# ZKTLabs/zkt-plonk

Hardware: AMD Instinct MI355X
Metric: proofs/sec (withdraw, n=2^20) (higher is better)
Workload: dtype u32 limbs (256-bit Montgomery); 1 GPU; full prove, WithdrawCircuit INPUTS=8 HEIGHT=64 Poseidon x5 (1019498 gates, 538 Poseidon gadgets), bn254, n=2^20, TABLE_SIZE=1024, 12 public inputs; parallelism=proofs sharded across 1 GPU(s), chained=True, distinct_witnesses=2, witness_on_device=True, table_cached=True, proof_bytes=802

## Files before the change

### include/zkt_plonk.h

```cpp
#ifndef ZKT_PLONK_H
#define ZKT_PLONK_H

#include <stddef.h>
#include <stdint.h>

#ifdef __cplusplus
extern "C" {
#endif

typedef struct zkt_ctx zkt_ctx;

enum {
    ZKT_CURVE_BN254 = 0,
    ZKT_CURVE_BLS12_381 = 1
};

enum {
    ZKT_OK = 0,
    ZKT_ERR_INVALID_ARGUMENT = 1,
    ZKT_ERR_INVALID_DOMAIN_SIZE = 2,
    ZKT_ERR_HIP = 3,
    ZKT_ERR_NO_DEVICE = 4,
    ZKT_ERR_TOO_MANY_COEFFICIENTS = 5,
    ZKT_ERR_ZERO_DENOMINATOR = 6,
// ... 23 lines not shown
    int (*all_gather_async)(void* user, const void* d_send, void* d_recv, size_t bytes, void* hip_stream);
} zkt_comm_vtable;
#define ZKT_QUOTIENT_CHUNKS 4
int zkt_ctx_set_comm(zkt_ctx* ctx, const zkt_comm_vtable* comm);
int zkt_shard_range(size_t total, int rank, int world, size_t* lo, size_t* hi);
int zkt_comm_stats(zkt_ctx* ctx, uint64_t* calls, uint64_t* bytes_sent);
int zkt_comm_selftest(const zkt_comm_vtable* comm, const void* send, void* recv, size_t bytes);

int zkt_dev_alloc(zkt_ctx* ctx, size_t bytes, void** dptr);
int zkt_dev_free(zkt_ctx* ctx, void* dptr);
int zkt_dev_upload(zkt_ctx* ctx, void* dptr, const void* host, size_t bytes);
int zkt_dev_download(zkt_ctx* ctx, void* host, const void* dptr, size_t bytes);

int zkt_ntt(zkt_ctx* ctx, int log_n, int inverse, int coset, const uint64_t* in, size_t in_len, uint64_t* out);
int zkt_ntt_dev(zkt_ctx* ctx, int log_n, int inverse, int coset, const void* d_in, size_t in_len, void* d_out);
int zkt_ntt_class(zkt_ctx* ctx, int log_n, int log_big, int cls, const uint64_t* in, size_t in_len, uint64_t* out);
int zkt_domain_group_gen(zkt_ctx* ctx, int log_n, uint64_t* out4);

int zkt_srs_load(zkt_ctx* ctx, const uint64_t* g1_xy_mont, size_t count);
int zkt_srs_load_dev(zkt_ctx* ctx, const void* d_g1_xy_mont, size_t count);
int zkt_srs_generate(zkt_ctx* ctx, const uint64_t* tau_canonical4, size_t count);
int zkt_srs_download(zkt_ctx* ctx, size_t offset, size_t count, uint64_t* out_xy_mont);
int zkt_srs_generate_g2(int curve_id, const uint64_t* tau_canonical4, uint64_t* out_h, uint64_t* out_beta_h);
int zkt_srs_load_slice(zkt_ctx* ctx, const uint64_t* g1_xy_mont_slice, size_t offset, size_t count, size_t total);
int zkt_srs_generate_slice(zkt_ctx* ctx, const uint64_t* tau_canonical4, size_t offset, size_t count, size_t total);
int zkt_msm_g1(zkt_ctx* ctx, const uint64_t* scalars, size_t len, size_t base_offset, int scalars_montgomery,
               uint64_t* out_xy_mont, int* out_is_infinity);
int zkt_msm_g1_dev(zkt_ctx* ctx, const void* d_scalars, size_t len, size_t base_offset, int scalars_montgomery,
                   void* out_xy_mont_host);
int zkt_msm_enqueue_dev(zkt_ctx* ctx, const void* d_scalars, size_t len, size_t base_offset, int scalars_montgomery);
int zkt_msm_info(zkt_ctx* ctx, int* window_bits, int* windows, size_t* srs_count);

#define ZKT_MSM_BASES_MAX ((size_t)1 << 22)
int zkt_msm_g1_bases(zkt_ctx* ctx, const uint64_t* bases_xy_mont, const uint64_t* scalars, size_t n,
                     int scalars_montgomery, uint64_t* out_xy_mont, int* out_is_infinity);
int zkt_msm_g1_bases_dev(zkt_ctx* ctx, const void* d_bases_xy_mont, const void* d_scalars, size_t n,
                         int scalars_montgomery, uint64_t* out_xy_mont_host, int* out_is_infinity);
int zkt_msm_bases_info(zkt_ctx* ctx, size_t n, int scalars_montgomery, int* window_bits, int* windows);

#define ZKT_KZG_BATCH_MAX 32
int zkt_kzg_commit_batch(zkt_ctx* ctx, const uint64_t* const* coeffs, const size_t* lens, int k,
                         int scalars_montgomery, uint64_t* out_xy_mont, int* out_is_infinity);
int zkt_kzg_commit_batch_dev(zkt_ctx* ctx, const void* const* d_coeffs, const size_t* lens, int k,
                             int scalars_montgomery, uint64_t* out_xy_mont, int* out_is_infinity);
int zkt_kzg_open(zkt_ctx* ctx, const uint64_t* const* coeffs, const size_t* lens, int k,
                 const uint64_t* challenges_mont, const uint64_t* point_mont,
                 uint64_t* out_w_xy_mont, int* out_w_is_infinity, uint64_t* out_evals_mont);
int zkt_kzg_open_dev(zkt_ctx* ctx, const void* const* d_coeffs, const size_t* lens, int k,
                     const uint64_t* challenges_mont, const uint64_t* point_mont,
                     uint64_t* out_w_xy_mont, int* out_w_is_infinity, uint64_t* out_evals_mont);

int zkt_ctx_set_lagrange(zkt_ctx* ctx, int on);
int zkt_ctx_set_wire_elimination(zkt_ctx* ctx, int mode);
int zkt_lagrange_info(zkt_ctx* ctx, int* log_n, size_t* bases);
int zkt_commit_evals_dev(zkt_ctx* ctx, const void* d_evals, const uint64_t* blinders, int k, int path, uint64_t* out_xy_mont,
                         int* out_is_infinity);

enum {
    ZKT_TRANSCRIPT_MERLIN = 0,
    ZKT_TRANSCRIPT_ETHEREUM = 1
};
typedef struct zkt_transcript zkt_transcript;
zkt_transcript* zkt_transcript_new(int kind, const char* label);
void zkt_transcript_free(zkt_transcript* t);
void zkt_transcript_append_u64(zkt_transcript* t, const char* label, uint64_t v);
void zkt_transcript_append_scalars(zkt_transcript* t, const char* label, const uint8_t* le32, size_t count, int single);
void zkt_transcript_append_commitment(zkt_transcript* t, const char* label, const uint8_t* x_le, const uint8_t* y_le,
                                      size_t fq_bytes, int is_infinity);
void zkt_transcript_challenge_scalar(zkt_transcript* t, const char* label, int fr_bits, uint8_t out_le32[32]);
void zkt_transcript_seed(zkt_transcript* t, uint64_t circuit_size, const uint8_t* xy_le, const uint8_t* is_infinity,
                         size_t fq_bytes);
int zkt_transcript_append_message(zkt_transcript* t, const char* label, const uint8_t* msg, size_t len);
int zkt_transcript_challenge_bytes(zkt_transcript* t, const char* label, uint8_t* out, size_t len);

typedef struct {
    void* user;
    void (*append_u64)(void* user, const char* label, uint64_t v);
    void (*append_scalars)(void* user, const char* label, const uint64_t* fr_mont, size_t count, int single);
    void (*append_commitment)(void* user, const char* label, const uint64_t* g1_xy_mont, int is_infinity);
    void (*challenge_scalar)(void* user, const char* label, uint64_t* fr_mont_out4);
} zkt_transcript_vtable;

int zkt_circuit_load(zkt_ctx* ctx, int log_n, const uint64_t* const* pk_polys, const size_t* pk_lens);

int zkt_circuit_setup(zkt_ctx* ctx, int log_n, const uint64_t* const* evals, const size_t* eval_lens, int evals_on_device,
                      uint64_t* out_commitments, int* out_is_infinity);

int zkt_circuit_sigma_dev(zkt_ctx* ctx, int log_n, const uint32_t* d_w_l, const uint32_t* d_w_r, const uint32_t* d_w_o,
                          size_t n_rows, size_t n_vars, void* const* d_sigma);
int zkt_circuit_setup_wiring(zkt_ctx* ctx, int log_n, const uint64_t* const* evals, const size_t* eval_lens,
                             int evals_on_device, const uint32_t* w_l, const uint32_t* w_r, const uint32_t* w_o,
                             size_t n_rows, size_t n_vars, int wiring_on_device,
                             uint64_t* out_commitments, int* out_is_infinity);

typedef struct {
    const uint64_t* a_evals;
    const uint64_t* b_evals;
    const uint64_t* c_evals;
    size_t n_rows;
    const uint64_t* table;
    size_t table_len;
    const size_t* pi_pos;
    const uint64_t* pi_vals;
    size_t n_pi;
    const uint64_t* blinders;
    int wires_on_device;
// ... 107 lines not shown
int zkt_verify_prepare(int curve_id, const zkt_verify_inputs* in, zkt_transcript* transcript, uint64_t* out_pairs,
                       int* out_is_infinity);

int zkt_pairing_product_is_one(int curve_id, const uint64_t* g1_xy_mont, const uint64_t* g2_xy_mont, size_t n, int* is_one);
int zkt_verify(int curve_id, const zkt_verify_inputs* in, zkt_transcript* transcript, const uint64_t* h_g2_mont,
               const uint64_t* beta_h_g2_mont, int* accepted);

int zkt_verify_batch(int curve_id, const zkt_verify_inputs* ins, zkt_transcript* const* transcripts, size_t count,
                     const uint64_t* h_g2_mont, const uint64_t* beta_h_g2_mont, int* accepted);

#define ZKT_G1_DECOMPRESS_MAX ((size_t)1 << 22)
enum {
    ZKT_G1_VALID = 0,
    ZKT_G1_IDENTITY = 1,
    ZKT_G1_NOT_CANONICAL = 2,
    ZKT_G1_BOTH_FLAGS = 3,
    ZKT_G1_NOT_ON_CURVE = 4,
    ZKT_G1_NOT_IN_SUBGROUP = 5
};
int zkt_g1_decompress(zkt_ctx* ctx, const uint8_t* compressed, size_t n, uint64_t* out_xy_mont, uint8_t* out_status);
int zkt_g1_decompress_dev(zkt_ctx* ctx, const void* d_compressed, size_t n, void* d_out_xy_mont, void* d_out_status);

#define ZKT_VERIFY_BATCH_DEV_MAX (ZKT_MSM_BASES_MAX / 24)
int zkt_verify_batch_prepare_dev(zkt_ctx* ctx, const zkt_verify_inputs* ins, zkt_transcript* const* transcripts, size_t count,
                                 const uint64_t* h_g2_mont, const uint64_t* beta_h_g2_mont, uint64_t* out_ab,
                                 int* out_ab_is_infinity, uint64_t* out_rho);
int zkt_verify_batch_dev(zkt_ctx* ctx, const zkt_verify_inputs* ins, zkt_transcript* const* transcripts, size_t count,
                         const uint64_t* h_g2_mont, const uint64_t* beta_h_g2_mont, int* accepted);

int zkt_g1_msm_host(int curve_id, const uint64_t* points_xy_mont, const uint64_t* scalars, size_t n, int scalars_montgomery,
                    uint64_t* out_xy_mont, int* out_is_infinity);

int zkt_keyfile_committer_key(const char* path, int curve_id, size_t max_powers, uint64_t* out_xy_mont, size_t* n_powers);
int zkt_keyfile_prover_key(const char* path, int curve_id, uint64_t* const* out_polys, size_t* lens10);
int zkt_keyfile_verifier_key(const char* path, int curve_id, uint64_t* n, uint64_t* pi_roots_mont, size_t pi_cap, size_t* n_pi,
                             uint64_t* commitments_xy_mont, int* is_infinity10);
#define ZKT_EPK_VECTORS 17
int zkt_keyfile_extended_prover_key(const char* path, int curve_id, int which, uint64_t* out_mont, size_t cap, size_t* lens17);
int zkt_circuit_check_epk_file(zkt_ctx* ctx, const char* epk_path, int* first_mismatch_vector, size_t* mismatch_at);
int zkt_srs_load_file(zkt_ctx* ctx, const char* ck_path, size_t max_powers);
int zkt_circuit_load_file(zkt_ctx* ctx, const char* pk_path, int log_n);

int zkt_debug_params(zkt_ctx* ctx, int which, uint32_t* out, size_t out_words);
int zkt_host_field_op(int curve_id, int which, int op, const uint32_t* a, const uint32_t* b, uint32_t* out);
int zkt_g1_sum_host(int curve_id, const uint64_t* points_xy_mont, size_t count, uint64_t* out_xy_mont, int* out_is_infinity);
int zkt_debug_fr_mul(zkt_ctx* ctx, const uint64_t* a, const uint64_t* b, size_t n, uint64_t* out);
int zkt_debug_ntt_batch(zkt_ctx* ctx, int log_n, int inverse, int coset, int nb, const void* const* d_in, const size_t* in_len,
                        void* const* d_out);
int zkt_debug_ntt_split(zkt_ctx* ctx, int npass, const int* log_r);
int zkt_debug_merkle_tree_split(zkt_merkle_tree* tree, int wide_min_parents);
int zkt_debug_pairing_selftest(int curve_id);
int zkt_debug_quotient(zkt_ctx* ctx, const uint64_t* challenges, const uint64_t* const* wit, const uint64_t* pi_pos,
                       const uint64_t* pi_vals, size_t n_pi, uint64_t* out);
int zkt_debug_grand_products(zkt_ctx* ctx, const uint64_t* challenges, const uint64_t* const* vectors, uint64_t* out_z1,
                             uint64_t* out_z2);
int zkt_debug_combine_split(zkt_ctx* ctx, const uint64_t* table, size_t table_len, const uint64_t* f, int fresh,
                            uint64_t* h1_out, uint64_t* h2_out);
int zkt_debug_commit_wires_dev(zkt_ctx* ctx, const void* d_variables, size_t n_vars, const uint32_t* d_w_l, const uint32_t* d_w_r,
                               const uint32_t* d_w_o, size_t n_rows, const uint64_t* blinders, int route, uint64_t* out_xy_mont,
                               int* out_is_infinity, int* out_route);
int zkt_debug_commit_wires_pi_dev(zkt_ctx* ctx, const void* d_variables, size_t n_vars, const uint32_t* d_w_l, const uint32_t* d_w_r,
                                  const uint32_t* d_w_o, size_t n_rows, const uint64_t* blinders, int route, const size_t* pi_pos,
                                  size_t n_pi, uint64_t* out_xy_mont, int* out_is_infinity, int* out_route);
int zkt_debug_wire_elimination(int curve, const uint64_t* const* selectors, const uint32_t* w_l, const uint32_t* w_r, const uint32_t* w_o,
                               size_t n_rows, size_t n_vars, const size_t* pi_pos, size_t n_pi, int K, uint8_t* out_kind,
                               uint32_t* out_free, size_t* out_n_free, uint32_t* out_term_v, uint32_t* out_term_f,
                               uint64_t* out_term_coef, size_t* out_n_terms, uint64_t* out_kappa);
int zkt_debug_open_witness(zkt_ctx* ctx, const uint64_t* coeffs, size_t len, const uint64_t* z4, uint64_t* out);
int zkt_debug_eval_lincomb(zkt_ctx* ctx, const uint64_t* const* polys, const size_t* lens, int k, const uint64_t* points,
                           const uint64_t* scalars, uint64_t* out_evals, uint64_t* out_lincomb, size_t out_len);

enum zkt_fx_op {
    ZKT_FX_UNPACK = 0, ZKT_FX_UNPACK_SHIFT = 1, ZKT_FX_PACK = 2, ZKT_FX_FROM_ARK = 3, ZKT_FX_TO_ARK = 4,
    ZKT_FX_NORMALIZE = 5, ZKT_FX_ADD = 6, ZKT_FX_DBL = 7, ZKT_FX_SUB_1 = 8, ZKT_FX_SUB_2 = 9, ZKT_FX_SUB_4 = 10,
    ZKT_FX_SUB_8 = 11, ZKT_FX_SUB2_6 = 12, ZKT_FX_ADD_LAZY = 13, ZKT_FX_SUB_LAZY_3 = 14, ZKT_FX_SUB_LAZY_4 = 15,
    ZKT_FX_SUB_LAZY_5 = 16, ZKT_FX_SUB_LAZY_9 = 17, ZKT_FX_SUB_LAZY_WIDE_8_30 = 18, ZKT_FX_MUL = 19, ZKT_FX_MUL_INL = 20,
    ZKT_FX_SQR = 21, ZKT_FX_SQR_INL = 22, ZKT_FX_MUL2_INL = 23, ZKT_FX_MUL_SHOUP = 24 ,
    ZKT_FX_MUL_LOW = 25, ZKT_FX_REDUCE_SMALL = 26, ZKT_FX_REDUCE_LAZY = 27 ,
    ZKT_FX_COND_SUB_P = 28, ZKT_FX_CANON = 29, ZKT_FX_IS_ZERO_CANON = 30, ZKT_FX_IS_ZERO_LT2P = 31, ZKT_FX_OP_COUNT = 32
};
enum zkt_xyzz_op {
    ZKT_XYZZ_ADD_MIXED = 0, ZKT_XYZZ_ADD_MIXED_INL = 1, ZKT_XYZZ_ADD = 2, ZKT_XYZZ_ADD_INL = 3, ZKT_XYZZ_DOUBLE = 4,
    ZKT_XYZZ_DOUBLE_AFFINE = 5, ZKT_XYZZ_OP_COUNT = 6
};
int zkt_debug_fx_layout(int curve_id, int which, int* limbs, int* limb_bits, int* sh);
int zkt_host_fx_op(int curve_id, int which, int op, const uint32_t* in, size_t n, uint32_t* out);
int zkt_debug_fx_op(zkt_ctx* ctx, int which, int op, const uint32_t* in, size_t n, uint32_t* out);
int zkt_host_xyzz_op(int curve_id, int op, const uint32_t* in, size_t n, uint32_t* out);
int zkt_debug_xyzz_op(zkt_ctx* ctx, int op, const uint32_t* in, size_t n, uint32_t* out);

#ifdef __cplusplus
}
#endif
#endif
```

### shim/src/ffi.rs

```rust
use std::os::raw::{c_char, c_int, c_void};

#[repr(C)]
pub struct ZktCtx {
    _private: [u8; 0],
}

#[repr(C)]
pub struct ZktTranscriptVtable {
    pub user: *mut c_void,
    pub append_u64: extern "C" fn(*mut c_void, *const c_char, u64),
    pub append_scalars: extern "C" fn(*mut c_void, *const c_char, *const u64, usize, c_int),
    pub append_commitment: extern "C" fn(*mut c_void, *const c_char, *const u64, c_int),
    pub challenge_scalar: extern "C" fn(*mut c_void, *const c_char, *mut u64),
}

#[repr(C)]
pub struct ZktCommVtable {
    pub user: *mut c_void,
    pub rank: c_int,
    pub world: c_int,
    pub device_buffers: c_int,
    pub all_gather: extern "C" fn(*mut c_void, *const c_void, *mut c_void, usize, c_int, *mut c_void) -> c_int,
    pub all_gather_async: Option<extern "C" fn(*mut c_void, *const c_void, *mut c_void, usize, *mut c_void) -> c_int>,
}
// ... 17 lines not shown
    pub w_r: *const u32,
    pub w_o: *const u32,
}

#[repr(C)]
pub struct ZktWitnessReport {
    pub satisfied: c_int,
    pub checked: c_int,
    pub n_arithmetic: u64,
    pub first_arithmetic: u64,
    pub residual: [u64; 4],
    pub n_lookup: u64,
    pub first_lookup: u64,
    pub n_wiring: u64,
    pub first_wiring_row: u64,
    pub first_wiring_column: c_int,
}

pub const ZKT_CHECK_WIRING: c_int = 1;
pub const ZKT_CHECK_NONE: u64 = u64::MAX;
pub const ZKT_VARIABLE_ZERO: u32 = 0xFFFF_FFFF;
pub const ZKT_CURVE_BN254: c_int = 0;
pub const ZKT_CURVE_BLS12_381: c_int = 1;
pub const ZKT_KZG_BATCH_MAX: usize = 32;

extern "C" {
    pub fn zkt_ctx_create(curve_id: c_int, device_id: c_int, out: *mut *mut ZktCtx) -> c_int;
    pub fn zkt_ctx_destroy(ctx: *mut ZktCtx);
    pub fn zkt_last_error(ctx: *const ZktCtx) -> *const c_char;
    pub fn zkt_ctx_set_comm(ctx: *mut ZktCtx, comm: *const ZktCommVtable) -> c_int;
    pub fn zkt_shard_range(total: usize, rank: c_int, world: c_int, lo: *mut usize, hi: *mut usize) -> c_int;
    pub fn zkt_ntt(ctx: *mut ZktCtx, log_n: c_int, inverse: c_int, coset: c_int, input: *const u64, in_len: usize,
                   out: *mut u64) -> c_int;
    pub fn zkt_srs_load(ctx: *mut ZktCtx, g1_xy_mont: *const u64, count: usize) -> c_int;
    pub fn zkt_srs_load_slice(ctx: *mut ZktCtx, g1_xy_mont: *const u64, offset: usize, count: usize, total: usize) -> c_int;
    pub fn zkt_srs_load_file(ctx: *mut ZktCtx, ck_path: *const c_char, max_powers: usize) -> c_int;
    pub fn zkt_msm_g1(ctx: *mut ZktCtx, scalars: *const u64, len: usize, base_offset: usize, scalars_montgomery: c_int,
                      out_xy_mont: *mut u64, out_is_infinity: *mut c_int) -> c_int;
    pub fn zkt_ctx_fork(ctx: *mut ZktCtx, out: *mut *mut ZktCtx) -> c_int;
    pub fn zkt_kzg_commit_batch(ctx: *mut ZktCtx, coeffs: *const *const u64, lens: *const usize, k: c_int,
                                scalars_montgomery: c_int, out_xy_mont: *mut u64, out_is_infinity: *mut c_int) -> c_int;
    pub fn zkt_kzg_commit_batch_dev(ctx: *mut ZktCtx, d_coeffs: *const *const c_void, lens: *const usize, k: c_int,
                                    scalars_montgomery: c_int, out_xy_mont: *mut u64, out_is_infinity: *mut c_int) -> c_int;
    pub fn zkt_kzg_open(ctx: *mut ZktCtx, coeffs: *const *const u64, lens: *const usize, k: c_int, challenges_mont: *const u64,
                        point_mont: *const u64, out_w_xy_mont: *mut u64, out_w_is_infinity: *mut c_int,
                        out_evals_mont: *mut u64) -> c_int;
    pub fn zkt_kzg_open_dev(ctx: *mut ZktCtx, d_coeffs: *const *const c_void, lens: *const usize, k: c_int,
                            challenges_mont: *const u64, point_mont: *const u64, out_w_xy_mont: *mut u64,
                            out_w_is_infinity: *mut c_int, out_evals_mont: *mut u64) -> c_int;
    pub fn zkt_commit_evals_dev(ctx: *mut ZktCtx, d_evals: *const c_void, blinders: *const u64, k: c_int, path: c_int,
                                out_xy_mont: *mut u64, out_is_infinity: *mut c_int) -> c_int;
    pub fn zkt_ctx_set_lagrange(ctx: *mut ZktCtx, on: c_int) -> c_int;
    pub fn zkt_ctx_set_wire_elimination(ctx: *mut ZktCtx, mode: c_int) -> c_int;
    pub fn zkt_lagrange_info(ctx: *mut ZktCtx, log_n: *mut c_int, bases: *mut usize) -> c_int;
    pub fn zkt_circuit_load(ctx: *mut ZktCtx, log_n: c_int, pk_polys: *const *const u64, pk_lens: *const usize) -> c_int;
    pub fn zkt_circuit_load_file(ctx: *mut ZktCtx, pk_path: *const c_char, log_n: c_int) -> c_int;
    pub fn zkt_keyfile_extended_prover_key(path: *const c_char, curve_id: c_int, which: c_int, out_mont: *mut u64, cap: usize,
                                           lens17: *mut usize) -> c_int;
    pub fn zkt_circuit_check_epk_file(ctx: *mut ZktCtx, epk_path: *const c_char, first_mismatch_vector: *mut c_int,
                                      mismatch_at: *mut usize) -> c_int;
    pub fn zkt_circuit_setup(ctx: *mut ZktCtx, log_n: c_int, evals: *const *const u64, eval_lens: *const usize,
                             evals_on_device: c_int, out_commitments: *mut u64, out_is_infinity: *mut c_int) -> c_int;
    pub fn zkt_circuit_sigma_dev(ctx: *mut ZktCtx, log_n: c_int, d_w_l: *const u32, d_w_r: *const u32, d_w_o: *const u32,
                                 n_rows: usize, n_vars: usize, d_sigma: *const *mut c_void) -> c_int;
    pub fn zkt_circuit_setup_wiring(ctx: *mut ZktCtx, log_n: c_int, evals: *const *const u64, eval_lens: *const usize,
                                    evals_on_device: c_int, w_l: *const u32, w_r: *const u32, w_o: *const u32, n_rows: usize,
                                    n_vars: usize, wiring_on_device: c_int, out_commitments: *mut u64,
                                    out_is_infinity: *mut c_int) -> c_int;
    pub fn zkt_prove_with(ctx: *mut ZktCtx, inputs: *const ZktProveInputs, transcript: *const ZktTranscriptVtable,
                          proof_out: *mut u8, proof_cap: usize, proof_len: *mut usize) -> c_int;
    pub fn zkt_prove_set_next(ctx: *mut ZktCtx, next: *const ZktProveInputs) -> c_int;
    pub fn zkt_circuit_check_witness(ctx: *mut ZktCtx, inputs: *const ZktProveInputs, flags: c_int,
                                     out: *mut ZktWitnessReport) -> c_int;
    pub fn zkt_g1_msm_host(curve_id: c_int, points_xy_mont: *const u64, scalars: *const u64, n: usize, scalars_montgomery: c_int,
                           out_xy_mont: *mut u64, out_is_infinity: *mut c_int) -> c_int;
    pub fn zkt_msm_g1_bases(ctx: *mut ZktCtx, bases_xy_mont: *const u64, scalars: *const u64, n: usize,
                            scalars_montgomery: c_int, out_xy_mont: *mut u64, out_is_infinity: *mut c_int) -> c_int;
    pub fn zkt_msm_g1_bases_dev(ctx: *mut ZktCtx, d_bases_xy_mont: *const c_void, d_scalars: *const c_void, n: usize,
                                scalars_montgomery: c_int, out_xy_mont_host: *mut u64, out_is_infinity: *mut c_int) -> c_int;
    pub fn zkt_verify(curve_id: c_int, inputs: *const ZktVerifyInputs, transcript: *mut c_void, h_g2_mont: *const u64,
                      beta_h_g2_mont: *const u64, accepted: *mut c_int) -> c_int;
    pub fn zkt_verify_batch(curve_id: c_int, inputs: *const ZktVerifyInputs, transcripts: *const *mut c_void, count: usize,
                            h_g2_mont: *const u64, beta_h_g2_mont: *const u64, accepted: *mut c_int) -> c_int;
    pub fn zkt_verify_batch_prepare_dev(ctx: *mut ZktCtx, inputs: *const ZktVerifyInputs, transcripts: *const *mut c_void, count: usize,
                                        h_g2_mont: *const u64, beta_h_g2_mont: *const u64, out_ab: *mut u64,
                                        out_ab_is_infinity: *mut c_int, out_rho: *mut u64) -> c_int;
    pub fn zkt_verify_batch_dev(ctx: *mut ZktCtx, inputs: *const ZktVerifyInputs, transcripts: *const *mut c_void, count: usize,
                                h_g2_mont: *const u64, beta_h_g2_mont: *const u64, accepted: *mut c_int) -> c_int;
    pub fn zkt_g1_decompress(ctx: *mut ZktCtx, compressed: *const u8, n: usize, out_xy_mont: *mut u64, out_status: *mut u8) -> c_int;
    pub fn zkt_g1_decompress_dev(ctx: *mut ZktCtx, d_compressed: *const c_void, n: usize, d_out_xy_mont: *mut c_void,
                                 d_out_status: *mut c_void) -> c_int;
    pub fn zkt_poseidon_load(ctx: *mut ZktCtx, params: *const ZktPoseidonParams, out: *mut *mut c_void) -> c_int;
    pub fn zkt_poseidon_free(ctx: *mut ZktCtx, params: *mut c_void);
    pub fn zkt_poseidon_hash_batch_dev(ctx: *mut ZktCtx, params: *const c_void, d_inputs: *const c_void, batch: usize,
                                       arity: c_int, d_out_hashes: *mut c_void, d_out_states: *mut c_void) -> c_int;
    pub fn zkt_poseidon_gadget_vars_per_hash(params: *const c_void) -> usize;
    pub fn zkt_poseidon_gadget_witness_dev(ctx: *mut ZktCtx, params: *const c_void, args: *const ZktPoseidonGadgetArgs) -> c_int;
    pub fn zkt_poseidon_gadget_check(ctx: *mut ZktCtx, params: *const c_void) -> c_int;
    pub fn zkt_merkle_path_vars_per_level(params: *const c_void) -> usize;
    pub fn zkt_poseidon_merkle_path_witness_dev(ctx: *mut ZktCtx, params: *const c_void, args: *const ZktMerklePathArgs) -> c_int;
    pub fn zkt_poseidon_merkle_path_validate(ctx: *mut ZktCtx, params: *const c_void, args: *const ZktMerklePathArgs) -> c_int;
    pub fn zkt_merkle_tree_create(ctx: *mut ZktCtx, params: *const c_void, height: c_int, capacity: usize, out: *mut *mut c_void) -> c_int;
    pub fn zkt_merkle_tree_free(ctx: *mut ZktCtx, tree: *mut c_void);
    pub fn zkt_merkle_tree_append_dev(ctx: *mut ZktCtx, tree: *mut c_void, d_leaves: *const c_void, m: usize, first_index: *mut u64) -> c_int;
    pub fn zkt_merkle_tree_append(ctx: *mut ZktCtx, tree: *mut c_void, leaves: *const u64, m: usize, first_index: *mut u64) -> c_int;
    pub fn zkt_merkle_tree_root(ctx: *mut ZktCtx, tree: *mut c_void, out4: *mut u64) -> c_int;
// ... 73 lines not shown
```

### zkt-plonk_amd/_lib.py

```python
from __future__ import annotations

import ctypes
import os
import re
from typing import Optional

import numpy as np

_HERE = os.path.dirname(os.path.abspath(__file__))
_LIB = os.environ.get("ZKT_LIB_PATH") or os.path.join(_HERE, "libzkt_plonk_hip.so")
_HEADER = os.path.join(_HERE, "..", "include", "zkt_plonk.h")

MSM_BASES_MAX = 1 << 22
G1_DECOMPRESS_MAX = 1 << 22
VERIFY_BATCH_DEV_MAX = MSM_BASES_MAX // 24
KZG_BATCH_MAX = 32
CURVE_BN254 = 0
CURVE_BLS12_381 = 1
_CURVES = {"bn254": 0, "bls12_381": 1, "bls12-381": 1, 0: 0, 1: 1}

_lib = None


class ZktError(RuntimeError):
# ... 462 lines not shown
def host_fx_op(curve, which: int, op: int, records) -> np.ndarray:
    L_ = fx_layout(curve, which)[0]
    rec = _records(records, 4 * L_)
    out = np.zeros_like(rec)
    rc = lib().zkt_host_fx_op(curve_id(curve), which, op, _u32p(rec), rec.shape[0], _u32p(out))
    if rc:
        raise ZktError(rc, "zkt_host_fx_op")
    return out


def host_xyzz_op(curve, op: int, records) -> np.ndarray:
    w = 4 * fx_layout(curve, 1)[0] + 1
    rec = _records(records, 2 * w)
    out = np.zeros((rec.shape[0], w), dtype=np.uint32)
    rc = lib().zkt_host_xyzz_op(curve_id(curve), op, _u32p(rec), rec.shape[0], _u32p(out))
    if rc:
        raise ZktError(rc, "zkt_host_xyzz_op")
    return out


def srs_generate_g2(curve, tau: int):
    L = lib()
    cid = curve_id(curve)
    words = 8 if cid == CURVE_BN254 else 12
    t = np.array([(int(tau) >> (64 * i)) & 0xFFFFFFFFFFFFFFFF for i in range(4)], dtype=np.uint64)
    h = np.zeros(2 * words, dtype=np.uint64)
    bh = np.zeros(2 * words, dtype=np.uint64)
    P64 = ctypes.POINTER(ctypes.c_uint64)
    L.zkt_srs_generate_g2.argtypes = [ctypes.c_int, P64, P64, P64]
    rc = L.zkt_srs_generate_g2(cid, u64p(t), u64p(h), u64p(bh))
    if rc:
        raise ZktError(rc, "zkt_srs_generate_g2")
    return h, bh


def g1_msm_host(curve, points, scalars, montgomery: bool = True) -> tuple:
    L = lib()
    cid = curve_id(curve)
    words = 8 if cid == CURVE_BN254 else 12
    pts = np.ascontiguousarray(points, dtype=np.uint64).reshape(-1, words)
    sc = np.ascontiguousarray(scalars, dtype=np.uint64).reshape(-1, 4)
    assert pts.shape[0] == sc.shape[0]
    out = np.zeros(words, dtype=np.uint64)
    inf = ctypes.c_int(0)
    P64 = ctypes.POINTER(ctypes.c_uint64)
    L.zkt_g1_msm_host.argtypes = [ctypes.c_int, P64, P64, ctypes.c_size_t, ctypes.c_int, P64, ctypes.POINTER(ctypes.c_int)]
    rc = L.zkt_g1_msm_host(cid, u64p(pts) if pts.size else None, u64p(sc) if sc.size else None, pts.shape[0], int(montgomery),
                           u64p(out), ctypes.byref(inf))
    if rc:
        raise ZktError(rc, "zkt_g1_msm_host")
    return out, bool(inf.value)


def wire_elimination(curve, selectors, w_l, w_r, w_o, n_vars: int, pi_pos=(), K: int = 16):
    L = lib()
    sel = [np.ascontiguousarray(q, dtype=np.uint64).reshape(-1, 4) for q in selectors]
    w = [np.ascontiguousarray(x, dtype=np.uint32) for x in (w_l, w_r, w_o)]
    n_rows = len(w[0])
    assert len(sel) == 5 and all(q.shape[0] == n_rows for q in sel) and all(len(x) == n_rows for x in w)
    pi = (ctypes.c_size_t * max(len(pi_pos), 1))(*[int(x) for x in pi_pos])
    cap = max(K * n_vars, 1)
    kind = np.zeros(max(n_vars, 1), dtype=np.uint8)
    free = np.zeros(max(n_vars, 1), dtype=np.uint32)
    tv, tf = np.zeros(cap, dtype=np.uint32), np.zeros(cap, dtype=np.uint32)
    tc = np.zeros((cap, 4), dtype=np.uint64)
    kappa = np.zeros((max(n_vars, 1), 4), dtype=np.uint64)
    n_free, n_terms = ctypes.c_size_t(0), ctypes.c_size_t(0)
    P64, P32 = ctypes.POINTER(ctypes.c_uint64), ctypes.POINTER(ctypes.c_uint32)
    sp = (P64 * 5)(*[u64p(q) for q in sel])
    L.zkt_debug_wire_elimination.argtypes = [ctypes.c_int, ctypes.POINTER(P64), P32, P32, P32, ctypes.c_size_t, ctypes.c_size_t,
                                             ctypes.POINTER(ctypes.c_size_t), ctypes.c_size_t, ctypes.c_int,
                                             ctypes.POINTER(ctypes.c_uint8), P32, ctypes.POINTER(ctypes.c_size_t), P32, P32, P64,
                                             ctypes.POINTER(ctypes.c_size_t), P64]
    rc = L.zkt_debug_wire_elimination(curve_id(curve), sp, _u32p(w[0]), _u32p(w[1]), _u32p(w[2]), n_rows, n_vars, pi, len(pi_pos),
                                      int(K), kind.ctypes.data_as(ctypes.POINTER(ctypes.c_uint8)), _u32p(free), ctypes.byref(n_free),
                                      _u32p(tv), _u32p(tf), u64p(tc), ctypes.byref(n_terms), u64p(kappa))
    if rc:
        raise ZktError(rc, "zkt_debug_wire_elimination")
    nt = n_terms.value
    return kind[:n_vars], free[:n_free.value].copy(), tv[:nt].copy(), tf[:nt].copy(), tc[:nt].copy(), kappa[:n_vars]


class Transcript:

    def __init__(self, kind: str = "merlin", label: str = "ZKT Plonk", fr_bits: int = 254, fq_bytes: int = 32):
        self._L = lib()
        self._h = ctypes.c_void_p(self._L.zkt_transcript_new(0 if kind == "merlin" else 1, label.encode()))
        self.fr_bits = fr_bits
        self.fq_bytes = fq_bytes

    def __del__(self):
        if getattr(self, "_h", None):
            self._L.zkt_transcript_free(self._h)
            self._h = None

    @property
    def handle(self):
        return self._h

    def append_u64(self, label: str, v: int):
        self._L.zkt_transcript_append_u64(self._h, label.encode(), v)

    def append_scalar(self, label: str, v: int):
        self._L.zkt_transcript_append_scalars(self._h, label.encode(), int(v).to_bytes(32, "little"), 1, 1)

    def append_scalars(self, label: str, vals):
# ... 702 lines not shown
            self._L.zkt_debug_commit_wires_pi_dev.argtypes = [ctypes.c_void_p, ctypes.c_void_p, ctypes.c_size_t, ctypes.c_void_p,
                                                              ctypes.c_void_p, ctypes.c_void_p, ctypes.c_size_t,
                                                              ctypes.POINTER(ctypes.c_uint64), ctypes.c_int,
                                                              ctypes.POINTER(ctypes.c_size_t), ctypes.c_size_t,
                                                              ctypes.POINTER(ctypes.c_uint64), ctypes.POINTER(ctypes.c_int),
                                                              ctypes.POINTER(ctypes.c_int)]
            self.check(self._L.zkt_debug_commit_wires_pi_dev(self._h, ctypes.c_void_p(d_variables), n_vars, ctypes.c_void_p(d_w_l),
                                                             ctypes.c_void_p(d_w_r), ctypes.c_void_p(d_w_o), n_rows, u64p(bl),
                                                             int(route), pi, len(pos), u64p(out), inf, took))
            return out, [bool(x) for x in inf], [int(x) for x in took]
        self._L.zkt_debug_commit_wires_dev.argtypes = [ctypes.c_void_p, ctypes.c_void_p, ctypes.c_size_t, ctypes.c_void_p,
                                                       ctypes.c_void_p, ctypes.c_void_p, ctypes.c_size_t,
                                                       ctypes.POINTER(ctypes.c_uint64), ctypes.c_int,
                                                       ctypes.POINTER(ctypes.c_uint64), ctypes.POINTER(ctypes.c_int),
                                                       ctypes.POINTER(ctypes.c_int)]
        self.check(self._L.zkt_debug_commit_wires_dev(self._h, ctypes.c_void_p(d_variables), n_vars, ctypes.c_void_p(d_w_l),
                                                      ctypes.c_void_p(d_w_r), ctypes.c_void_p(d_w_o), n_rows, u64p(bl), int(route),
                                                      u64p(out), inf, took))
        return out, [bool(x) for x in inf], [int(x) for x in took]

    def check_epk_file(self, path: str):
        self._L.zkt_circuit_check_epk_file.argtypes = [ctypes.c_void_p, ctypes.c_char_p, ctypes.POINTER(ctypes.c_int),
                                                       ctypes.POINTER(ctypes.c_size_t)]
        vec, at = ctypes.c_int(0), ctypes.c_size_t(0)
        self.check(self._L.zkt_circuit_check_epk_file(self._h, path.encode(), ctypes.byref(vec), ctypes.byref(at)))
        if vec.value < 0:
            return None
        return vec.value, (-1 if at.value == ctypes.c_size_t(-1).value else at.value)

    def debug_eval_lincomb(self, polys, points, scalars, out_len: int):
        keep = [np.ascontiguousarray(p_, dtype=np.uint64).reshape(-1, 4) for p_ in polys]
        k = len(keep)
        P64 = ctypes.POINTER(ctypes.c_uint64)
        ptrs = (P64 * k)(*[u64p(a) for a in keep])
        lens = (ctypes.c_size_t * k)(*[a.shape[0] for a in keep])
        pts = np.ascontiguousarray(points, dtype=np.uint64).reshape(k, 4)
        scs = np.ascontiguousarray(scalars, dtype=np.uint64).reshape(k, 4)
        ev = np.empty((k, 4), dtype=np.uint64)
        lc = np.empty((out_len, 4), dtype=np.uint64)
        self._L.zkt_debug_eval_lincomb.argtypes = [ctypes.c_void_p, ctypes.POINTER(P64), ctypes.POINTER(ctypes.c_size_t), ctypes.c_int,
                                                   P64, P64, P64, P64, ctypes.c_size_t]
        self.check(self._L.zkt_debug_eval_lincomb(self._h, ptrs, lens, k, u64p(pts), u64p(scs), u64p(ev), u64p(lc), out_len))
        return ev, lc

    def debug_open_witness(self, coeffs, z) -> np.ndarray:
        p_ = np.ascontiguousarray(coeffs, dtype=np.uint64).reshape(-1, 4)
        zz = np.ascontiguousarray(z, dtype=np.uint64).reshape(4)
        out = np.empty((p_.shape[0] - 1, 4), dtype=np.uint64)
        self._L.zkt_debug_open_witness.argtypes = [ctypes.c_void_p, ctypes.POINTER(ctypes.c_uint64), ctypes.c_size_t,
                                                   ctypes.POINTER(ctypes.c_uint64), ctypes.POINTER(ctypes.c_uint64)]
        self.check(self._L.zkt_debug_open_witness(self._h, u64p(p_), p_.shape[0], u64p(zz), u64p(out)))
        return out

    def debug_quotient(self, n: int, challenges, wit, pi_pos=(), pi_vals=None) -> np.ndarray:
        ch = np.ascontiguousarray(challenges, dtype=np.uint64).reshape(5, 4)
        keep = [None if w is None else np.ascontiguousarray(w, dtype=np.uint64).reshape(4 * n, 4) for w in wit]
        assert len(keep) == 9
        ptrs = (ctypes.c_void_p * 9)(*[None if w is None else w.ctypes.data for w in keep])
        pos = np.ascontiguousarray(list(pi_pos), dtype=np.uint64)
        vals = np.ascontiguousarray(pi_vals if len(pos) else np.zeros((0, 4)), dtype=np.uint64).reshape(-1, 4)
        out = np.empty((4 * n, 4), dtype=np.uint64)
        self.check(self._L.zkt_debug_quotient(self._h, u64p(ch), ptrs, u64p(pos) if len(pos) else None,
                                              u64p(vals) if len(pos) else None, len(pos), u64p(out)))
        return out
```

### zkt-plonk_amd/csrc/capi.hip

```cpp
#include "ctx.hpp"

#include <cstdlib>
#include "hostinv.hpp"
#include "ec.hpp"
#include "hostec.hpp"
#include "fx_test.hpp"
#include "msm.hpp"

#include <cstring>

namespace zkt {

const char* exp_env(const char* name) {
#ifdef ZKT_EXPERIMENTS
    return getenv(name);
#else
    (void)name;
    return nullptr;
#endif
}

int set_err(zkt_ctx* c, int code, const std::string& msg) {
    if (c) c->err = msg;
    return code;
// ... 150 lines not shown
template <class P>
static int dump_params(uint32_t* out, size_t words) {
    const int N = P::N;
    if (words < (size_t)(3 * N + 1)) return -1;
    for (int i = 0; i < N; ++i) out[i] = P::mod(i);
    out[N] = P::INV;
    for (int i = 0; i < N; ++i) out[N + 1 + i] = P::one(i);
    for (int i = 0; i < N; ++i) out[2 * N + 1 + i] = P::r2(i);
    return N;
}

}

using namespace zkt;

extern "C" {

const char* zkt_version(void) { return "zkt-plonk_amd 0.1 (gfx950)"; }

int zkt_ctx_create(int curve_id, int device_id, zkt_ctx** out) {
    if (!out) return ZKT_ERR_INVALID_ARGUMENT;
    *out = nullptr;
    if (curve_id != ZKT_CURVE_BN254 && curve_id != ZKT_CURVE_BLS12_381) return ZKT_ERR_INVALID_ARGUMENT;
    int count = 0;
    if (hipGetDeviceCount(&count) != hipSuccess || count <= 0 || device_id < 0 || device_id >= count)
        return ZKT_ERR_NO_DEVICE;
    if (hipSetDevice(device_id) != hipSuccess) return ZKT_ERR_NO_DEVICE;
    zkt_ctx* c = new zkt_ctx();
    c->batch_off = exp_env("ZKT_MSM_NO_BATCH") != nullptr;
    c->aux_off = exp_env("ZKT_NO_AUX") != nullptr;
    c->curve = curve_id;
    c->device = device_id;
    if (hipStreamCreateWithFlags(&c->stream, hipStreamNonBlocking) != hipSuccess) {
        delete c;
        return ZKT_ERR_HIP;
    }
    c->own_stream = true;
    *out = c;
    return ZKT_OK;
}

int zkt_ctx_fork(zkt_ctx* parent, zkt_ctx** out) {
    if (!parent || !out) return ZKT_ERR_INVALID_ARGUMENT;
    *out = nullptr;
    if (parent->sharded()) return set_err(parent, ZKT_ERR_INVALID_ARGUMENT, "zkt_ctx_fork: not for a context with a communicator");
    if (parent->zombie) return set_err(parent, ZKT_ERR_INVALID_ARGUMENT, "zkt_ctx_fork: the context has been destroyed");
    zkt_ctx* root = parent->parent ? parent->parent : parent;
    zkt_ctx* c = nullptr;
    int rc = zkt_ctx_create(parent->curve, parent->device, &c);
    if (rc) return rc;
    (void)hipStreamSynchronize(parent->stream);
    c->lagrange_off = parent->lagrange_off;
    c->wire_elim_mode = parent->wire_elim_mode;
    c->batch_off = parent->batch_off;
    c->aux_off = parent->aux_off;
    c->ntt_plans = parent->ntt_plans;
    c->parent = root;
    root->forks.fetch_add(1);
    if ((rc = msm_fork(c, parent)) || (rc = circuit_fork(c, parent))) {
        parent->err = c->err;
        zkt_ctx_destroy(c);
        return rc;
    }
    *out = c;
    return ZKT_OK;
}

void zkt_ctx_destroy(zkt_ctx* c) {
    if (!c) return;
    (void)hipSetDevice(c->device);
    (void)hipStreamSynchronize(c->stream);
    if (c->forks.load() > 0) {
        c->zombie = true;
        return;
    }
    zkt_ctx* const owner = c->parent;
    circuit_release(c);
    msm_release(c);
    prof_resolve(c);
    for (hipEvent_t e : c->event_pool) (void)hipEventDestroy(e);
    c->event_pool.clear();
    c->ntt_plans.clear();
    c->msm.reset();
    c->msmb.reset();
    c->kzg.reset();
    c->circuit.reset();
    if (c->comm.pinned) (void)hipHostFree(c->comm.pinned);
    for (void* p : c->owned) (void)hipFree(p);
    c->owned.clear();
    if (c->own_stream && c->stream) (void)hipStreamDestroy(c->stream);
    delete c;
    if (owner && owner->forks.fetch_sub(1) == 1 && owner->zombie) {
        owner->zombie = false;
        zkt_ctx_destroy(owner);
    }
}

int zkt_ctx_set_comm(zkt_ctx* c, const zkt_comm_vtable* comm) {
    if (!c) return ZKT_ERR_INVALID_ARGUMENT;
    if (int rf = refuse_if_forked(c, "zkt_ctx_set_comm")) return rf;
    if (c->parent && comm && comm->world > 1) return set_err(c, ZKT_ERR_INVALID_ARGUMENT, "a forked context cannot take a communicator");
    if (comm && comm->world > 1) {
        const int w = comm->world;
        if ((w != 2 && w != 4 && w != 8) || comm->rank < 0 || comm->rank >= w || !comm->all_gather)
            return set_err(c, ZKT_ERR_INVALID_ARGUMENT, "communicator: world must be 1, 2, 4 or 8 with a valid rank and callback");
    }
// ... 372 lines not shown
```

### zkt-plonk_amd/csrc/ctx.hpp

```cpp
#pragma once
#include <hip/hip_runtime.h>
#include <stdint.h>
#include <stddef.h>
#include <map>
#include <string>
#include <tuple>
#include <vector>
#include <memory>
#include <atomic>

#include "../../include/zkt_plonk.h"
#include "fp.hpp"
#include "fx.hpp"
#include "ntt.hpp"

namespace zkt {

struct MsmState;
struct MsmBasesState;
struct KzgState;
struct CircuitState;

}

struct zkt_ctx {
    int curve = 0;
    int device = 0;
    hipStream_t stream = nullptr;
    bool own_stream = false;
    std::string err;

    std::map<std::tuple<int, int, int, int>, std::shared_ptr<void>> ntt_plans;
    int ntt_split_npass = 0;
    int ntt_split_log_r[3] = {0, 0, 0};
    void* ntt_scratch = nullptr;
    size_t ntt_scratch_bytes = 0;
    void* io_a = nullptr;
    size_t io_a_bytes = 0;
    void* io_b = nullptr;
    size_t io_b_bytes = 0;
    void* check_scratch = nullptr;
    size_t check_scratch_bytes = 0;
    void* verify_scratch = nullptr;
    size_t verify_scratch_bytes = 0;

    int prof_on = 0;
    struct ProfSlot {
        std::vector<std::pair<hipEvent_t, hipEvent_t>> pending;
        double total_ms = 0.0;
        uint64_t calls = 0;
        uint64_t launches = 0;
    };
    std::map<std::string, ProfSlot> prof;
    std::vector<hipEvent_t> event_pool;

    struct Comm {
        zkt_comm_vtable vt{};
        void* pinned = nullptr;
        size_t pinned_bytes = 0;
        uint64_t calls = 0, bytes = 0;
    } comm;
    bool sharded() const { return comm.vt.world > 1; }

    std::shared_ptr<zkt::MsmState> msm;
    std::shared_ptr<zkt::MsmBasesState> msmb;
    std::shared_ptr<zkt::KzgState> kzg;
    uint64_t msm_epoch = 0;
    uint64_t srs_generation = 0;
    zkt_ctx* parent = nullptr;
    std::atomic<int> forks{0};
    bool zombie = false;
    bool aux_off = false;
    bool batch_off = false;
    bool lagrange_off = false;
    int wire_elim_mode = 1;
    std::shared_ptr<zkt::CircuitState> circuit;
    std::vector<void*> owned;
};

namespace zkt {

const char* exp_env(const char* name);

int set_err(zkt_ctx* c, int code, const std::string& msg);
int refuse_if_forked(zkt_ctx* c, const char* what);
int hip_fail(zkt_ctx* c, hipError_t e, const char* what);

#define ZKT_HIP(c, call)                                        \
    do {                                                        \
        hipError_t _e = (call);                                 \
        if (_e != hipSuccess) return zkt::hip_fail((c), _e, #call); \
    } while (0)

struct ProfScope {
    zkt_ctx* c;
    zkt_ctx::ProfSlot* slot = nullptr;
    hipEvent_t e0 = nullptr, e1 = nullptr;
    hipStream_t stream = nullptr;
    uint64_t count = 1;
    ProfScope(zkt_ctx* ctx, const char* name, hipStream_t on_stream = nullptr, uint64_t units = 1);
    ~ProfScope();
};

int comm_all_gather_host(zkt_ctx* c, const void* send, void* recv, size_t bytes);
int comm_all_gather_dev(zkt_ctx* c, const void* d_send, void* d_recv, size_t bytes);
bool comm_async_available(const zkt_ctx* c);
int comm_all_gather_async(zkt_ctx* c, const void* d_send, void* d_recv, size_t bytes, hipStream_t st);

int ensure_buffer(zkt_ctx* c, void** p, size_t* cur, size_t bytes);
struct DevBuf {
    void* p = nullptr;
    size_t bytes = 0;
};
inline int grow(zkt_ctx* c, DevBuf& b, size_t bytes) { return ensure_buffer(c, &b.p, &b.bytes, bytes); }
int dev_alloc(zkt_ctx* c, void** p, size_t bytes);
void dev_free(zkt_ctx* c, void* p);

template <class P>
Fe<P> root_of_unity(int log_n);
int ntt_run(zkt_ctx* c, int log_n, int inverse, int coset, const void* d_in, size_t in_len, void* d_out);
int ntt_run_batch(zkt_ctx* c, int log_n, int inverse, int coset, int nb, const void* const* d_in, const size_t* in_len,
                  void* const* d_out);
int ntt_class_code(int log_big, int cls);
int ntt_force_split(zkt_ctx* c, int npass, const int* log_r);
int ntt_run_class(zkt_ctx* c, int log_n, int log_big, int cls, const void* d_in, size_t in_len, void* d_out, void* d_fold);

void circuit_release(zkt_ctx* c);
int circuit_fork(zkt_ctx* child, const zkt_ctx* parent);

}
```

### zkt-plonk_amd/csrc/ntt.hip

```cpp
#include "ctx.hpp"
#include "hostinv.hpp"
#include <cstdlib>

namespace zkt {

constexpr int TILE_LOG = 10;
constexpr int TILE = 1 << TILE_LOG;
constexpr int NTT_THREADS = 256;
constexpr int EPT = TILE / NTT_THREADS;

template <class P>
ZKT_D Fx<P> tile_get(const uint4* lo, const uint4* hi, const uint32_t* top, int64_t idx) {
    static_assert(FxP<P>::L == 9, "scalar fields use nine limbs");
    const uint4 a = lo[idx], b = hi[idx];
    Fx<P> r;
    r.l[0] = a.x; r.l[1] = a.y; r.l[2] = a.z; r.l[3] = a.w;
    r.l[4] = b.x; r.l[5] = b.y; r.l[6] = b.z; r.l[7] = b.w;
    r.l[8] = top[idx];
    return r;
}
template <class P>
ZKT_D void tile_put(uint4* lo, uint4* hi, uint32_t* top, int64_t idx, const Fx<P>& x) {
    lo[idx] = make_uint4(x.l[0], x.l[1], x.l[2], x.l[3]);
    hi[idx] = make_uint4(x.l[4], x.l[5], x.l[6], x.l[7]);
    top[idx] = x.l[8];
}

ZKT_D uint32_t bitrev32(uint32_t x, int bits) { return __brev(x) >> (32 - bits); }

constexpr int NTT_W_PACKED = 0, NTT_W_LIMBS = 1, NTT_W_SHOUP = 2;
template <class P, int MODE>
struct WTile {
    const uint4* lo;
    const uint4* hi;
    const uint32_t* top;
    const uint4* qlo;
    const uint4* qhi;
    const uint32_t* qtop;
    ZKT_D Fx<P> mul(int e, const Fx<P>& d) const {
        if constexpr (MODE == NTT_W_SHOUP) {
            return fx_mul_shoup<P>(d, tile_get<P>(lo, hi, top, e), tile_get<P>(qlo, qhi, qtop, e));
        } else if constexpr (MODE == NTT_W_LIMBS) {
            return fx_mul_inl<P>(tile_get<P>(lo, hi, top, e), d);
        } else {
            Fe<P> w;
            const uint4 a = lo[e], b = hi[e];
            w.v[0] = a.x; w.v[1] = a.y; w.v[2] = a.z; w.v[3] = a.w;
            w.v[4] = b.x; w.v[5] = b.y; w.v[6] = b.z; w.v[7] = b.w;
            return fx_mul_inl<P>(fx_unpack<P>(w), d);
        }
    }
};

template <class P, int G, bool LASTSTEP, class W>
ZKT_D void dif_group(Fx<P>* x, const W& w, int off, int sub, int L) {
// ... 116 lines not shown
        } else {
            const Fe<P> w = fe_load<P>(w_inner + i);
            lds_w_lo[i] = make_uint4(w.v[0], w.v[1], w.v[2], w.v[3]);
            lds_w_hi[i] = make_uint4(w.v[4], w.v[5], w.v[6], w.v[7]);
        }
    }
    const uint4* gq = reinterpret_cast<const uint4*>(reinterpret_cast<const char*>(a.w_inner_s) + (R / 2) * 36 + ((R / 2) * 36 % 16 ? 16 - (R / 2) * 36 % 16 : 0));
    const WT lds_w{lds_w_lo, lds_w_hi, lds_w_top, gq, gq + R / 2, reinterpret_cast<const uint32_t*>(gq + R)};

    const uint64_t tile = blockIdx.x;
    uint64_t in_base, out_base, tw_base;
    uint64_t ld_r, ld_c, st_k;
    if constexpr (!LAST) {
        const uint32_t log_s = a.log_s;
        const uint64_t tiles_per_hi = (uint64_t)1 << (log_s - LOG_T);
        const uint64_t hi = tile >> (log_s - LOG_T);
        const uint64_t lo0 = (tile & (tiles_per_hi - 1)) << LOG_T;
        in_base = (hi << (LOG_R + log_s)) + lo0;
        out_base = in_base;
        ld_r = (uint64_t)1 << log_s;
        ld_c = 1;
        st_k = ld_r;
        tw_base = hi << LOG_R;
    } else {
        const uint32_t log_r1 = a.log_r1, log_mid = a.log_mid;
        const uint64_t k1_tiles = (uint64_t)1 << (log_r1 - LOG_T);
        const uint64_t mid = tile >> (log_r1 - LOG_T);
        const uint64_t k10 = (tile & (k1_tiles - 1)) << LOG_T;
        in_base = (k10 << (log_mid + LOG_R)) + (mid << LOG_R);
        ld_r = 1;
        ld_c = (uint64_t)1 << (log_mid + LOG_R);
        out_base = k10 + (mid << log_r1);
        st_k = (uint64_t)1 << (a.log_n - LOG_R);
        tw_base = (k10 + (mid << log_r1)) << LOG_R;
    }

#pragma unroll 2
    for (int e = 0; e < EPT; ++e) {
        int flat = e * NTT_THREADS + tid;
        int r, c;
        if constexpr (!LAST) {
            c = flat & (T - 1);
            r = flat >> LOG_T;
        } else {
            r = flat & (R - 1);
            c = flat >> LOG_R;
        }
        uint64_t g = in_base + (uint64_t)r * ld_r + (uint64_t)c * ld_c;
        Fx<P> x;
        if (a.in_raw) {
            const uint4* rlo = reinterpret_cast<const uint4*>(in_p);
            x = tile_get<P>(rlo, rlo + a.raw_n, reinterpret_cast<const uint32_t*>(rlo + 2 * a.raw_n), (int64_t)g);
        } else {
            x = (g < in_len) ? fx_unpack<P>(fe_load<P>(in + g)) : fx_zero<P>();
        }
        if (in_row && (a.in_raw || g < in_len)) x = fx_mul<P>(x, fx_unpack<P>(fe_load<P>(in_row + r)));
        if (tw) {
            uint64_t ti = LAST ? (tw_base + ((uint64_t)c << LOG_R) + r) : (tw_base + r);
            x = fx_mul<P>(x, fx_unpack<P>(fe_load<P>(tw + ti)));
        }
        tile_put<P>(lds_lo, lds_hi, lds_top, r * T + c, x);
    }
    __syncthreads();

    dif_all<P, LOG_R>(lds_lo, lds_hi, lds_top, lds_w, tid);
    __syncthreads();

#pragma unroll 2
    for (int e = 0; e < EPT; ++e) {
        int flat = e * NTT_THREADS + tid;
        int c = flat & (T - 1);
        int k = flat >> LOG_T;
        int rho = (int)bitrev32((uint32_t)k, LOG_R);
        Fx<P> x = tile_get<P>(lds_lo, lds_hi, lds_top, rho * T + c);
        if (out_row) x = fx_mul<P>(x, fx_unpack<P>(fe_load<P>(out_row + k)));
        else if (!a.out_raw) x = fx_cond_sub_p<P>(x);
        const uint64_t at = out_base + (uint64_t)k * st_k + c;
        if (a.out_raw) {
            uint4* rlo = reinterpret_cast<uint4*>(out_p);
            tile_put<P>(rlo, rlo + a.raw_n, reinterpret_cast<uint32_t*>(rlo + 2 * a.raw_n), (int64_t)at, x);
        } else {
            fe_store<P>(out + at, fx_pack<P>(fx_cond_sub_p<P>(x)));
        }
    }
}

template <class P>
__global__ void k_table_to_fx(Fe<P>* t, uint64_t n) {
    uint64_t i = (uint64_t)blockIdx.x * blockDim.x + threadIdx.x;
    if (i >= n) return;
    fe_store<P>(t + i, fx_pack<P>(fx_cond_sub_p<P>(fx_from_ark<P>(fe_load<P>(t + i)))));
}

template <class P>
__global__ void k_table_to_shoup(const Fe<P>* t, void* out, uint64_t n, Fx<P> npinv) {
    uint64_t i = (uint64_t)blockIdx.x * blockDim.x + threadIdx.x;
    if (i >= n) return;
    const Fe<P> x = fe_load<P>(t + i);
    const Fx<P> w = fx_unpack<P>(fe_from_mont<P>(x));
    const Fx<P> what = fx_cond_sub_p<P>(fx_from_ark<P>(x));
    const Fx<P> wq = fx_mul_low<P>(what, npinv);
    const uint64_t plane = n * 36, second = (plane + 15) & ~(uint64_t)15;
    uint4* wl = reinterpret_cast<uint4*>(out);
    tile_put<P>(wl, wl + n, reinterpret_cast<uint32_t*>(wl + 2 * n), (int64_t)i, w);
    uint4* ql = reinterpret_cast<uint4*>(reinterpret_cast<char*>(out) + second);
    tile_put<P>(ql, ql + n, reinterpret_cast<uint32_t*>(ql + 2 * n), (int64_t)i, wq);
}

template <class P>
__global__ __launch_bounds__(NTT_THREADS) void k_ntt_small(const Fe<P>* in, uint64_t in_len, Fe<P>* out, int log_n,
                                                           const Fe<P>* w, const Fe<P>* in_scale,
                                                           const Fe<P>* out_scale) {
    __shared__ Fe<P> buf[TILE];
    const int n = 1 << log_n;
    const int tid = threadIdx.x;
    for (int i = tid; i < n; i += NTT_THREADS) {
        Fe<P> x = ((uint64_t)i < in_len) ? fe_load<P>(in + i) : fe_zero<P>();
        if (in_scale) x = fe_mul<P>(x, fe_load<P>(in_scale + i));
        buf[i] = x;
    }
    __syncthreads();
    for (int s = 0; s < log_n; ++s) {
        const int m = n >> s, half = m >> 1;
        for (int idx = tid; idx < n / 2; idx += NTT_THREADS) {
            int blk = idx / half, j = idx % half;
            int i0 = blk * m + j, i1 = i0 + half;
            Fe<P> u = buf[i0], v = buf[i1];
            buf[i0] = fe_add<P>(u, v);
            buf[i1] = fe_mul<P>(fe_sub<P>(u, v), fe_load<P>(w + ((size_t)j << s)));
        }
        __syncthreads();
    }
    for (int k = tid; k < n; k += NTT_THREADS) {
        Fe<P> x = buf[log_n ? bitrev32((uint32_t)k, log_n) : 0];
        if (out_scale) x = fe_mul<P>(x, fe_load<P>(out_scale + k));
        fe_store<P>(out + k, x);
    }
}

template <class P>
__global__ void k_gen_pow(Fe<P>* out, uint64_t n, Fe<P> base, Fe<P> scale) {
    uint64_t i = (uint64_t)blockIdx.x * blockDim.x + threadIdx.x;
    if (i >= n) return;
    fe_store<P>(out + i, fe_mul<P>(scale, fe_pow_u64<P>(base, i)));
}
template <class P>
__global__ void k_gen_tw2d(Fe<P>* out, uint64_t rows, uint32_t log_cols, Fe<P> w, Fe<P> row_base, Fe<P> col_base,
                           Fe<P> scale, int use_row, int use_col) {
    uint64_t i = (uint64_t)blockIdx.x * blockDim.x + threadIdx.x;
    if (i >= (rows << log_cols)) return;
    uint64_t K = i >> log_cols, m = i & (((uint64_t)1 << log_cols) - 1);
    Fe<P> x = fe_mul<P>(scale, fe_pow_u64<P>(w, m * K));
    if (use_row) x = fe_mul<P>(x, fe_pow_u64<P>(row_base, K));
    if (use_col) x = fe_mul<P>(x, fe_pow_u64<P>(col_base, m));
    fe_store<P>(out + i, x);
}

template <class P>
static Fe<P> host_pow_limbs(const Fe<P>& a, const uint32_t* e, int nlimbs) {
    Fe<P> r = fe_one<P>();
    bool started = false;
    for (int i = nlimbs * 32 - 1; i >= 0; --i) {
        if (started) r = fe_sqr<P>(r);
        if ((e[i / 32] >> (i % 32)) & 1u) {
            r = fe_mul<P>(r, a);
            started = true;
        }
    }
    return r;
}
// ... 209 lines not shown
                               (const Fe<P>*)pl.w_inner[i], pl.w_inner_s[i], cnt, npinv);
            ZKT_HIP(c, hipGetLastError());
        }
    }
    for (int i = 0; i < p; ++i)
        if ((rc = table_to_fx<P>(c, pl.w_inner[i], (uint64_t)1 << (pl.log_r[i] - 1)))) return rc;
    if ((rc = table_to_fx<P>(c, pl.in_row, (uint64_t)1 << pl.log_r[0]))) return rc;
    {
        int acc2 = 0;
        for (int i = 1; i < p; ++i) {
            acc2 += pl.log_r[i - 1];
            if ((rc = table_to_fx<P>(c, pl.tw[i], (uint64_t)1 << (acc2 + pl.log_r[i])))) return rc;
        }
    }
    if ((rc = table_to_fx<P>(c, pl.out_row, (uint64_t)1 << pl.log_r[p - 1]))) return rc;
    return 0;
}

static int ntt_mode_for(int log_r) {
    int mont_from = 10;
    if (const char* e = exp_env("ZKT_NTT_MONT_FROM")) mont_from = atoi(e);
    if (log_r < mont_from) return NTT_W_SHOUP;
    return log_r <= 7 ? NTT_W_LIMBS : NTT_W_PACKED;
}

template <class P, bool LAST, int LOG_R>
static void launch_pass_r(zkt_ctx* c, const dim3& grid, const NttPassArgs& a) {
    const int mode = ntt_mode_for(LOG_R);
    if (mode == NTT_W_SHOUP) {
        hipLaunchKernelGGL((k_ntt_pass<P, LOG_R, LAST, NTT_W_SHOUP>), grid, dim3(NTT_THREADS), 0, c->stream, a);
        return;
    }
#if defined(ZKT_EXPERIMENTS)
    hipLaunchKernelGGL((k_ntt_pass<P, LOG_R, LAST, (LOG_R <= 7 ? NTT_W_LIMBS : NTT_W_PACKED)>), grid, dim3(NTT_THREADS), 0, c->stream, a);
#else
    hipLaunchKernelGGL((k_ntt_pass<P, LOG_R, LAST, NTT_W_SHOUP>), grid, dim3(NTT_THREADS), 0, c->stream, a);
#endif
}

template <class P, bool LAST>
static void launch_pass(zkt_ctx* c, int log_r, unsigned blocks, unsigned nb, const NttPassArgs& a) {
    const dim3 grid(blocks, nb);
    switch (log_r) {
        case 5: launch_pass_r<P, LAST, 5>(c, grid, a); break;
        case 6: launch_pass_r<P, LAST, 6>(c, grid, a); break;
        case 7: launch_pass_r<P, LAST, 7>(c, grid, a); break;
        case 8: launch_pass_r<P, LAST, 8>(c, grid, a); break;
        default: launch_pass_r<P, LAST, 9>(c, grid, a); break;
    }
}

template <class P>
static int ntt_run_batch_t(zkt_ctx* c, int log_n, int inverse, int coset, int nb, const void* const* d_in, const size_t* in_len,
                           void* const* d_out) {
    if (nb < 1 || nb > NTT_MAX_BATCH) return set_err(c, ZKT_ERR_INVALID_ARGUMENT, "transform batch out of range");
    if (log_n < 0 || log_n > P::TWO_ADICITY)
        return set_err(c, ZKT_ERR_INVALID_DOMAIN_SIZE,
                       "InvalidEvalDomainSize: log_size_of_group " + std::to_string(log_n) + " exceeds adicity " +
                           std::to_string(P::TWO_ADICITY));
    if (log_n > 27) return set_err(c, ZKT_ERR_INVALID_DOMAIN_SIZE, "domains above 2^27 are not supported");
    const uint64_t N = (uint64_t)1 << log_n;
    for (int y = 0; y < nb; ++y)
        if (in_len[y] > N) return set_err(c, ZKT_ERR_INVALID_DOMAIN_SIZE, "more coefficients than the domain size");
    const bool forced = c->ntt_split_npass && log_n > TILE_LOG;
    if (forced && c->ntt_split_log_r[0] + c->ntt_split_log_r[1] + c->ntt_split_log_r[2] != log_n)
        return set_err(c, ZKT_ERR_INVALID_ARGUMENT, "the forced split (zkt_debug_ntt_split) does not multiply to this domain size");
    auto key = std::make_tuple(log_n, inverse ? 1 : 0, coset, forced ? ntt_split_code(c) : 0);
    auto it = c->ntt_plans.find(key);
    if (it == c->ntt_plans.end()) {
        auto holder = std::make_shared<NttPlan<P>>();
        int rc = build_plan<P>(c, log_n, inverse ? 1 : 0, coset, forced, *holder);
        if (rc) return rc;
        it = c->ntt_plans.emplace(key, std::static_pointer_cast<void>(holder)).first;
    }
    const NttPlan<P>& pl = *static_cast<const NttPlan<P>*>(it->second.get());
    const std::string prof_name = "ntt_" + std::to_string(log_n);
    ProfScope prof_all(c, prof_name.c_str(), nullptr, nb);
    if (pl.npass == 0) {
        for (int y = 0; y < nb; ++y)
            hipLaunchKernelGGL(k_ntt_small<P>, dim3(1), dim3(NTT_THREADS), 0, c->stream, (const Fe<P>*)d_in[y],
                               (uint64_t)in_len[y], (Fe<P>*)d_out[y], log_n, (const Fe<P>*)pl.small_w,
                               (const Fe<P>*)pl.small_in, (const Fe<P>*)pl.small_out);
        ZKT_HIP(c, hipGetLastError());
        return 0;
    }
    int rc = ensure_buffer(c, &c->ntt_scratch, &c->ntt_scratch_bytes, N * 36 * (size_t)nb);
    if (rc) return rc;
    const int p = pl.npass;
    const unsigned blocks = (unsigned)(N >> TILE_LOG);
    int acc = 0;
    for (int i = 0; i < p; ++i) {
        NttPassArgs a{};
        const bool last = (i == p - 1);
        for (int y = 0; y < NTT_MAX_BATCH; ++y) {
            const int yy = y < nb ? y : 0;
            a.in[y] = (i == 0) ? d_in[yy] : c->ntt_scratch;
            a.out[y] = last ? d_out[yy] : c->ntt_scratch;
            a.in_len[y] = (i == 0) ? (uint64_t)in_len[yy] : N;
        }
        a.w_inner = pl.w_inner[i];
        a.w_inner_s = pl.w_inner_s[i];
        a.in_row = (i == 0) ? pl.in_row : nullptr;
        a.tw = pl.tw[i];
        a.out_row = last ? pl.out_row : nullptr;
        a.log_n = (uint32_t)log_n;
        a.in_raw = (i == 0) ? 0u : 1u;
        a.out_raw = last ? 0u : 1u;
        a.raw_n = N;
        acc += pl.log_r[i];
        if (!last) {
            a.log_s = (uint32_t)(log_n - acc);
            launch_pass<P, false>(c, pl.log_r[i], blocks, (unsigned)nb, a);
        } else {
            a.log_r1 = (uint32_t)pl.log_r[0];
            a.log_mid = (uint32_t)(log_n - pl.log_r[0] - pl.log_r[i]);
            launch_pass<P, true>(c, pl.log_r[i], blocks, (unsigned)nb, a);
        }
        ZKT_HIP(c, hipGetLastError());
    }
    return 0;
}

template <class P>
static int ntt_run_t(zkt_ctx* c, int log_n, int inverse, int coset, const void* d_in, size_t in_len, void* d_out) {
    return ntt_run_batch_t<P>(c, log_n, inverse, coset, 1, &d_in, &in_len, &d_out);
}

int ntt_run_batch(zkt_ctx* c, int log_n, int inverse, int coset, int nb, const void* const* d_in, const size_t* in_len,
                  void* const* d_out) {
    if (c->curve == ZKT_CURVE_BN254) return ntt_run_batch_t<Bn254Fr>(c, log_n, inverse, coset, nb, d_in, in_len, d_out);
    return ntt_run_batch_t<Bls381Fr>(c, log_n, inverse, coset, nb, d_in, in_len, d_out);
}

int ntt_run(zkt_ctx* c, int log_n, int inverse, int coset, const void* d_in, size_t in_len, void* d_out) {
    if (c->curve == ZKT_CURVE_BN254) return ntt_run_t<Bn254Fr>(c, log_n, inverse, coset, d_in, in_len, d_out);
    return ntt_run_t<Bls381Fr>(c, log_n, inverse, coset, d_in, in_len, d_out);
}

template <class P>
__global__ void k_fold(const Fe<P>* in, uint64_t in_len, Fe<P>* out, uint64_t N, Fe<P> cN) {
    uint64_t i = (uint64_t)blockIdx.x * blockDim.x + threadIdx.x;
    if (i >= N) return;
    Fe<P> acc = (i < in_len) ? fe_load<P>(in + i) : fe_zero<P>();
    Fe<P> pw = cN;
    for (uint64_t at = i + N; at < in_len; at += N) {
        acc = fe_add<P>(acc, fe_mul<P>(pw, fe_load<P>(in + at)));
        pw = fe_mul<P>(pw, cN);
    }
    fe_store<P>(out + i, acc);
}

template <class P>
static int ntt_run_class_t(zkt_ctx* c, int log_n, int log_big, int cls, const void* d_in, size_t in_len, void* d_out,
                           void* d_fold) {
    const uint64_t N = (uint64_t)1 << log_n;
    if (log_big < log_n || log_big > P::TWO_ADICITY || cls < 0 || cls >= (1 << (log_big - log_n)) || cls > 255)
        return set_err(c, ZKT_ERR_INVALID_DOMAIN_SIZE, "class transform: bad (log_n, log_big, class)");
    const int code = (log_big == log_n) ? 1 : ntt_class_code(log_big, cls);
    if (in_len > N) {
        if (!d_fold) return set_err(c, ZKT_ERR_INVALID_ARGUMENT, "class transform: fold scratch missing");
        const Fe<P> cN = fe_pow_u64<P>(coset_shift<P>(code), N);
        hipLaunchKernelGGL(k_fold<P>, dim3((unsigned)((N + 255) / 256)), dim3(256), 0, c->stream, (const Fe<P>*)d_in,
                           (uint64_t)in_len, (Fe<P>*)d_fold, N, cN);
        ZKT_HIP(c, hipGetLastError());
        d_in = d_fold;
        in_len = N;
    }
    return ntt_run_t<P>(c, log_n, 0, code, d_in, in_len, d_out);
}

int ntt_run_class(zkt_ctx* c, int log_n, int log_big, int cls, const void* d_in, size_t in_len, void* d_out, void* d_fold) {
    if (c->curve == ZKT_CURVE_BN254) return ntt_run_class_t<Bn254Fr>(c, log_n, log_big, cls, d_in, in_len, d_out, d_fold);
    return ntt_run_class_t<Bls381Fr>(c, log_n, log_big, cls, d_in, in_len, d_out, d_fold);
}

}
```

### zkt-plonk_amd/csrc/ntt.hpp

```cpp
#pragma once
#include <hip/hip_runtime.h>
#include <stdint.h>
#include <stddef.h>

namespace zkt {

constexpr int NTT_MAX_BATCH = 4;

struct NttPassArgs {
    const void* in[NTT_MAX_BATCH];
    void* out[NTT_MAX_BATCH];
    const void* w_inner;
    const void* w_inner_s;
    const void* in_row;
    const void* tw;
    const void* out_row;
    uint64_t in_len[NTT_MAX_BATCH];
    uint32_t log_n;
    uint32_t log_s;
    uint32_t log_r1;
    uint32_t log_mid;
    uint32_t in_raw, out_raw;
    uint64_t raw_n;
};

template <class P>
struct NttPlan {
    int log_n = -1;
    int inverse = 0, coset = 0;
    int npass = 0;
    int log_r[3] = {0, 0, 0};
    void* w_inner[3] = {nullptr, nullptr, nullptr};
    void* w_inner_s[3] = {nullptr, nullptr, nullptr};
    void* in_row = nullptr;
    void* tw[3] = {nullptr, nullptr, nullptr};
    void* out_row = nullptr;
    void* small_w = nullptr;
    void* small_in = nullptr;
    void* small_out = nullptr;
    size_t table_bytes = 0;
};

}
```

### zkt-plonk_amd/csrc/poly.hip

```cpp
#include "poly.hpp"
#include "hostinv.hpp"

namespace zkt {

template <class P>
ZKT_D Fe<P> arg_fe(const uint32_t* w) {
    Fe<P> r;
#pragma unroll
    for (int i = 0; i < 8; ++i) r.v[i] = w[i];
    return r;
}

template <class P>
__global__ void k_mul_vec(const Fe<P>* a, const Fe<P>* b, Fe<P>* o, size_t n) {
    size_t i = (size_t)blockIdx.x * blockDim.x + threadIdx.x;
    if (i < n) fe_store<P>(o + i, fe_mul<P>(fe_load<P>(a + i), fe_load<P>(b + i)));
}

template <class P>
__global__ void k_trim_len(const Fe<P>* p, size_t lo, size_t n, uint32_t* len, int skip_if_set, Fe<P>* zero_at,
                           int zero_count) {
    if (zero_at && blockIdx.x == 0 && (int)threadIdx.x < zero_count) fe_store<P>(zero_at + threadIdx.x, fe_zero<P>());
    if (skip_if_set && *len != 0) return;
    size_t i = lo + (size_t)blockIdx.x * blockDim.x + threadIdx.x;
// ... 813 lines not shown
    const uint64_t j = i / piece, o = i - j * piece;
    fe_store<P>(out + t, fe_load<P>(in + ((j << log_g) + cls) * piece + o));
}
template <class P> static int interleave_t(zkt_ctx* c, const void* in, void* out, size_t n4, uint32_t G, uint32_t chunks) {
    uint32_t lg = 0;
    while ((1u << lg) < G) ++lg;
    const uint64_t m = n4 >> lg;
    if (chunks == 0 || m % chunks) return set_err(c, ZKT_ERR_INVALID_ARGUMENT, "interleave: pieces must divide the class");
    hipLaunchKernelGGL(k_interleave<P>, dim3(nblocks(n4)), dim3(256), 0, c->stream, (const Fe<P>*)in, (Fe<P>*)out, (uint64_t)n4, lg,
                       m / chunks);
    ZKT_HIP(c, hipGetLastError());
    return ZKT_OK;
}
int quotient_interleave(zkt_ctx* c, const void* in, void* out, size_t n4, uint32_t G, uint32_t chunks) {
    ZKT_DISPATCH(c, interleave_t, in, out, n4, G, chunks);
}

template <class P>
__global__ void k_quot_split(const Fe<P>* q, size_t chunk, size_t cap, Fe<P>* lo, Fe<P>* mid, Fe<P>* hi) {
    const size_t i = (size_t)blockIdx.x * blockDim.x + threadIdx.x;
    if (i >= cap) return;
    const bool in = i < chunk;
    const Fe<P> z = fe_zero<P>();
    fe_store<P>(lo + i, in ? fe_load<P>(q + i) : z);
    fe_store<P>(mid + i, in ? fe_load<P>(q + chunk + i) : z);
    fe_store<P>(hi + i, in ? fe_load<P>(q + 2 * chunk + i) : z);
}

template <class P> static int quot_split_t(zkt_ctx* c, const void* q, size_t n, const void* b0b1, void* lo, void* mid, void* hi, uint32_t* d_status) {
    const Fe<P>* Q = (const Fe<P>*)q;
    const size_t cap = n + 8, chunk = n + 2;
    hipLaunchKernelGGL(k_quot_split<P>, dim3(nblocks(cap)), dim3(256), 0, c->stream, Q, chunk, cap, (Fe<P>*)lo, (Fe<P>*)mid,
                       (Fe<P>*)hi);
    ZKT_HIP(c, hipGetLastError());
    uint32_t* lens = d_status + 4;
    int rc;
    if ((rc = trim_len_t<P>(c, lo, chunk, lens + 0))) return rc;
    if ((rc = trim_len_t<P>(c, mid, chunk, lens + 1))) return rc;
    if ((rc = trim_len_t<P>(c, hi, chunk, lens + 2))) return rc;
    {
        const size_t lo = 3 * chunk, hi = 4 * n;
        hipLaunchKernelGGL(k_trim_len<P>, dim3(nblocks(hi - lo)), dim3(256), 0, c->stream, (const Fe<P>*)q, lo, hi, lens + 3, 0,
                           (Fe<P>*)nullptr, 0);
        ZKT_HIP(c, hipGetLastError());
    }
    hipLaunchKernelGGL(k_quot_blind<P>, dim3(1), dim3(64), 0, c->stream, (Fe<P>*)lo, (Fe<P>*)mid, (Fe<P>*)hi, lens, (const Fe<P>*)b0b1, (uint32_t)n, d_status);
    ZKT_HIP(c, hipGetLastError());
    return ZKT_OK;
}
int quotient_split_blind(zkt_ctx* c, const void* q, size_t n, const void* d_b0b1, void* q_lo, void* q_mid, void* q_hi, uint32_t* d_status) {
    ZKT_DISPATCH(c, quot_split_t, q, n, d_b0b1, q_lo, q_mid, q_hi, d_status);
}

int open_elems(size_t len) { return ow_elems(len); }
size_t open_blocks(size_t len) { return ow_blocks(len); }
template <class P> static int open_pow_tables_t(zkt_ctx* c, const uint32_t* z, const uint32_t* zinv, void* d_powers, size_t len) {
    hipLaunchKernelGGL(k_pow_tables<P>, dim3(1), dim3(OW_THREADS), 0, c->stream, host_fe<P>(z), host_fe<P>(zinv), (Fe<P>*)d_powers,
                       (int)ow_blocks(len), ow_elems(len));
    ZKT_HIP(c, hipGetLastError());
    return ZKT_OK;
}
int open_pow_tables(zkt_ctx* c, const uint32_t z[8], const uint32_t z_inv[8], void* d_powers, size_t len) {
    ZKT_DISPATCH(c, open_pow_tables_t, z, z_inv, d_powers, len);
}
template <class P> static int open_divide_t(zkt_ctx* c, const void* t, size_t len, void* tb, void* scan_tmp, void* out, const void* d_powers) {
    if (len == 0) return ZKT_OK;
    const Fe<P>* pw = (const Fe<P>*)d_powers;
    const int E = ow_elems(len);
    const unsigned blocks = (unsigned)ow_blocks(len);
    int rc = scan_t<P, OpAdd>(c, (const Fe<P>*)t, (Fe<P>*)tb, len, true, (Fe<P>*)scan_tmp);
    if (rc) return rc;
    hipLaunchKernelGGL(k_mul_pow<P>, dim3(blocks), dim3(256), 0, c->stream, (const Fe<P>*)tb + 1, (Fe<P>*)out, len - 1, len,
                       pw + EV_PW, pw + 2 * EV_PW + blocks, E, 1);
    ZKT_HIP(c, hipGetLastError());
    return ZKT_OK;
}
int open_divide(zkt_ctx* c, const void* t, size_t len, void* d_tmp, void* d_scan_tmp, void* out, const void* d_powers) {
    ZKT_DISPATCH(c, open_divide_t, t, len, d_tmp, d_scan_tmp, out, d_powers);
}

template <class P> static int open_witness_t(zkt_ctx* c, const void* p, size_t len, const uint32_t* z, const uint32_t* zinv, void* ta, void* tb, void* scan_tmp, void* out, void* d_powers) {
    if (len == 0) return ZKT_OK;
    Fe<P>* pw = (Fe<P>*)d_powers;
    const int E = ow_elems(len);
    const unsigned blocks = (unsigned)ow_blocks(len);
    int rc = open_pow_tables_t<P>(c, z, zinv, d_powers, len);
    if (rc) return rc;
    hipLaunchKernelGGL(k_mul_pow<P>, dim3(blocks), dim3(256), 0, c->stream, (const Fe<P>*)p, (Fe<P>*)ta, len, len,
                       (const Fe<P>*)pw, (const Fe<P>*)pw + 2 * EV_PW, E, 0);
    ZKT_HIP(c, hipGetLastError());
    return open_divide_t<P>(c, ta, len, tb, scan_tmp, out, d_powers);
}
int open_witness(zkt_ctx* c, const void* p, size_t len, const uint32_t z[8], const uint32_t z_inv[8], void* d_tmp_a, void* d_tmp_b, void* d_scan_tmp, void* out, void* d_powers) {
    ZKT_DISPATCH(c, open_witness_t, p, len, z, z_inv, d_tmp_a, d_tmp_b, d_scan_tmp, out, d_powers);
}

template <class P> static int sum_rows_t(zkt_ctx* c, const void* partials, int nblk, int rows, void* out) {
    hipLaunchKernelGGL(k_eval_final<P>, dim3(rows), dim3(256), 0, c->stream, (const Fe<P>*)partials, nblk, (Fe<P>*)out);
    ZKT_HIP(c, hipGetLastError());
    return ZKT_OK;
}
int poly_sum_rows(zkt_ctx* c, const void* d_partials, int nblk, int rows, void* d_out) {
    ZKT_DISPATCH(c, sum_rows_t, d_partials, nblk, rows, d_out);
}

template <class P> static int gen_powers_t(zkt_ctx* c, void* out, size_t n, const uint32_t* base, const uint32_t* scale) {
// ... 35 lines not shown
```

### zkt-plonk_amd/csrc/poly.hpp

```cpp
#pragma once
#include "ctx.hpp"

namespace zkt {

constexpr int LC_MAX_TERMS = 16;
struct LinCombArgs {
    const void* poly[LC_MAX_TERMS];
    uint64_t len[LC_MAX_TERMS];
    uint32_t scalar[LC_MAX_TERMS][8];
    int nterms;
};

constexpr int EVAL_MAX = 16;
struct EvalArgs {
    const void* poly[EVAL_MAX];
    uint64_t len[EVAL_MAX];
    uint32_t point[EVAL_MAX][8];
    int count;
};

struct QuotientArgs {
    const void *a, *b, *c, *pi, *z1, *z2, *t, *h1, *h2;
    const void *q_m, *q_l, *q_r, *q_o, *q_c, *q_lookup, *q_table, *sigma1, *sigma2, *sigma3, *x, *l1;
    void* out;
    uint32_t alpha[8], beta[8], gamma[8], delta[8], epsilon[8];
    uint32_t zh_inv[4][8];
    uint64_t n4;
    const uint32_t* pi_tab;
    uint32_t n_pi_direct;
    uint32_t G, cls, next_off;
    const void *z1_next, *z2_next, *t_next, *h1_next;
    uint64_t first, count;
};
constexpr int QUOTIENT_PI_DIRECT_MAX = 16;

struct ZTermsArgs {
    const void *a, *b, *c, *s1, *s2, *s3, *roots;
    const void *f, *t, *h1, *h2;
    void *num, *den;
    uint32_t beta[8], gamma[8], delta[8], epsilon[8];
    uint64_t n;
};

int poly_mul_vec(zkt_ctx* c, const void* a, const void* b, void* out, size_t n);
int poly_set_zero(zkt_ctx* c, void* p, size_t n_elems);
int poly_trim_len(zkt_ctx* c, const void* p, size_t n, uint32_t* d_len, void* zero_at = nullptr, int zero_count = 0);
int poly_copy_pad(zkt_ctx* c, const void* d_in, size_t len, void* out, size_t n);
int poly_gather_pad(zkt_ctx* c, const void* d_values, size_t n_vars, const uint32_t* d_idx, size_t rows, void* out, size_t n,
                    uint32_t* d_status);
int poly_add_blinders(zkt_ctx* c, void* p, const uint32_t* d_len, const void* d_blinders, int k, size_t cap);
int poly_lincomb(zkt_ctx* c, const LinCombArgs& a, void* out, size_t n);
int lagrange_scalars(zkt_ctx* c, const void* ev, size_t n, const uint32_t* d_len, const void* d_blinders, int k, const void* d_roots,
                     void* out);
int poly_eval_many(zkt_ctx* c, const EvalArgs& a, void* d_partials, void* d_results, void* d_powers);
int z1_terms(zkt_ctx* c, const ZTermsArgs& a);
int z2_terms(zkt_ctx* c, const ZTermsArgs& a);
int scan_mul(zkt_ctx* c, const void* in, void* out, size_t n, bool reverse, void* d_tmp );
int scan_add(zkt_ctx* c, const void* in, void* out, size_t n, bool reverse, void* d_tmp);
int z_combine(zkt_ctx* c, const void* pn, const void* sd, const uint32_t inv_total[8], void* out, size_t n);
int quotient_pointwise(zkt_ctx* c, const QuotientArgs& a);
int to_hat_form(zkt_ctx* c, void* v, size_t n, int k32);
int quotient_interleave(zkt_ctx* c, const void* in, void* out, size_t n4, uint32_t G, uint32_t chunks = 1);
int quotient_split_blind(zkt_ctx* c, const void* q, size_t n, const void* d_b0b1, void* q_lo, void* q_mid, void* q_hi,
                         uint32_t* d_status);
int open_witness(zkt_ctx* c, const void* p, size_t len, const uint32_t z[8], const uint32_t z_inv[8], void* d_tmp_a, void* d_tmp_b,
                 void* d_scan_tmp, void* out, void* d_powers );
size_t open_witness_powers(size_t maxlen);
constexpr int OPEN_PW_ROW = 257;
int open_elems(size_t len);
size_t open_blocks(size_t len);
int open_pow_tables(zkt_ctx* c, const uint32_t z[8], const uint32_t z_inv[8], void* d_powers, size_t len);
int open_divide(zkt_ctx* c, const void* t, size_t len, void* d_tmp, void* d_scan_tmp, void* out, const void* d_powers);
int poly_sum_rows(zkt_ctx* c, const void* d_partials, int nblk, int rows, void* d_out);
int sigma_build(zkt_ctx* c, int log_n, const uint32_t* d_w_l, const uint32_t* d_w_r, const uint32_t* d_w_o, size_t n_rows, size_t n_vars,
                void* const* d_sigma);
size_t sigma_scratch_bytes(int log_n, size_t n_rows);
int sigma_enqueue(zkt_ctx* c, int log_n, const uint32_t* d_w_l, const uint32_t* d_w_r, const uint32_t* d_w_o, size_t n_rows, size_t n_vars,
                  void* const* d_sigma, void* d_scratch, uint32_t* d_flag);
struct WitnessCheckKeys {
    int log_n;
    const void* pk[5];
    const void* q_lookup_ev;
    const void* sigma_ev[3];
};
int selector_evals_enqueue(zkt_ctx* c, int log_n, const void* const* pk, void* const* outs);
int witness_check(zkt_ctx* c, const WitnessCheckKeys& keys, const zkt_prove_inputs& in, int flags, zkt_witness_report* out);
int gen_powers(zkt_ctx* c, void* out, size_t n, const uint32_t base[8], const uint32_t scale[8]);
int lookup_count(zkt_ctx* c, const void* f, size_t n, const void* d_sorted_keys, const uint32_t* d_perm, uint32_t nkeys,
                 uint32_t* d_counts, uint32_t* d_status);
int lookup_starts(zkt_ctx* c, const uint32_t* d_base_counts, uint32_t* d_hits, uint32_t nkeys, size_t n, uint32_t* d_even,
                  uint32_t* d_odd, uint32_t* d_status);
int lookup_expand(zkt_ctx* c, const void* d_keys_insertion, const uint32_t* d_starts, uint32_t nkeys, void* out, size_t n);

}
```

### zkt-plonk_amd/csrc/prover.hip

```cpp
#include "ctx.hpp"
#include "hostinv.hpp"
#include <chrono>
#include <cstdio>
#include <cstdlib>
#include "ec.hpp"
#include "keyfile.hpp"
#include "msm.hpp"
#include "poly.hpp"
#include "transcript.hpp"

#include <algorithm>
#include <functional>
#include <cstring>
#include <memory>
#include <optional>
#include <vector>

namespace zkt {

enum { PK_QM = 0, PK_QL, PK_QR, PK_QO, PK_QC, PK_S1, PK_S2, PK_S3, PK_QLOOKUP, PK_QTABLE, PK_COUNT };
enum { CS_QM = 0, CS_QL, CS_QR, CS_QO, CS_QC, CS_QLOOKUP, CS_QTABLE, CS_S1, CS_S2, CS_S3, CS_X, CS_L1, CS_COUNT };
enum { W_A = 0, W_B, W_C, W_PI, W_Z1, W_Z2, W_T, W_H1, W_H2, W_COUNT };

struct CircuitState {
    int log_n = 0;
    size_t n = 0;
    int G = 1, cls = 0, log_m = 0;
    size_t m = 0;
    void* wnext[4] = {};
    void* fold = nullptr;
    void* qgather = nullptr;
    bool have[16] = {};
    void* pk[PK_COUNT] = {};
    size_t pk_len[PK_COUNT] = {};
    void* coset[CS_COUNT] = {};
    void* sigma_ev[3] = {};
    void* q_lookup_ev = nullptr;
    void* roots = nullptr;
    uint32_t zh_inv[4][8] = {};
    void* ev[8] = {};
    void* sc[4] = {};
    void* scan_tmp = nullptr;
    void* poly[13] = {};
    void* wcos[W_COUNT] = {};
    void* qev = nullptr;
    void* lag_scalars = nullptr;
    void* lag_scalars_q[3] = {};
    void* small = nullptr;
    uint32_t* status = nullptr;
    uint32_t* lk_u32 = nullptr;
    uint32_t lk_nkeys = 0;
    std::vector<uint32_t> lk_host_keys, lk_host_sorted, lk_host_counts, lk_host_order;
    bool has_next = false, prefetch_same_table = false;
    int prefetch_stage = 0;
    uint64_t prefetch_epoch = 0;
    zkt_prove_inputs next_in{}, prefetch_in{};
    void* poly_alt[3] = {};
    uint32_t* status_alt = nullptr;
    void* lk_keys = nullptr;
    size_t lk_cap = 0;
    void* pinned = nullptr;
    hipStream_t comm_stream = nullptr;
    hipEvent_t ev_piece[ZKT_QUOTIENT_CHUNKS] = {}, ev_gathered = nullptr;
    hipStream_t aux_stream = nullptr;
    hipEvent_t ev_aux_go = nullptr, ev_aux_done = nullptr;
    void* aux_scan_tmp = nullptr;
    void* aux_pw = nullptr;
    hipStream_t copy_stream = nullptr;
    hipEvent_t ev_copy[4] = {};
    void* pinned_pi = nullptr;
    uint32_t* pi_tab = nullptr;
    void* eval_pw = nullptr;
    std::vector<uint64_t> cached_table;
    bool t_cached = false, t_coset_valid = false;
    uint64_t t_srs_generation = 0;
    uint64_t t_commit_xy[12] = {};
    bool keys_borrowed = false;
    bool wire_route[3] = {};
    bool wire_dense_only = false;
    int wire_elim_force = -1;
};

template <class P>
struct HostF {
    using F = Fe<P>;
    static F from_words(const uint64_t* w) {
        F r;
        memcpy(r.v, w, 32);
        return r;
    }
    static void to_le_bytes(const F& mont, uint8_t out[32]) {
        F c = fe_from_mont<P>(mont);
        memcpy(out, c.v, 32);
    }
    static F from_le_bytes(const uint8_t in[32]) {
        F c;
        memcpy(c.v, in, 32);
        return fe_to_mont<P>(c);
    }
    static F pow_u64(F a, uint64_t e) { return fe_pow_u64<P>(a, e); }
};

template <class Q>
static void fq_to_le(const Fe<Q>& mont, uint8_t* out) {
    Fe<Q> c = fe_from_mont<Q>(mont);
    memcpy(out, c.v, Q::N * 4);
}

template <class Q>
static void serialize_point(const Affine<Q>& p, std::vector<uint8_t>& out) {
    const size_t nb = Q::N * 4;
    std::vector<uint8_t> b(nb, 0);
    if (aff_is_inf<Q>(p)) {
        b[nb - 1] |= 0x40;
    } else {
        fq_to_le<Q>(p.x, b.data());
        Fe<Q> y = fe_from_mont<Q>(p.y);
        Fe<Q> ny = fe_from_mont<Q>(fe_neg<Q>(p.y));
        bool greater = false;
        for (int i = Q::N - 1; i >= 0; --i) {
            if (y.v[i] != ny.v[i]) {
                greater = y.v[i] > ny.v[i];
                break;
            }
        }
        if (greater) b[nb - 1] |= 0x80;
    }
    out.insert(out.end(), b.begin(), b.end());
}

constexpr int WIRE_ELIM_MIN_LOG_N = 17;

template <class C>
struct Prover {
    using R = typename C::Fr;
    using Q = typename C::Fq;
    using F = Fe<R>;
    using H = HostF<R>;

    zkt_ctx* c;
    CircuitState& S;
    HostTranscript& tr;
    Prover(zkt_ctx* ctx, CircuitState& st, HostTranscript& t) : c(ctx), S(st), tr(t) {
        trace_on = exp_env("ZKT_HOST_TRACE") != nullptr;
    }
    bool copy_fenced = false;
    bool trace_on = false;
    std::vector<std::pair<const char*, std::chrono::steady_clock::time_point>> marks;
    void mark(const char* what) {
        if (trace_on) marks.emplace_back(what, std::chrono::steady_clock::now());
    }
    void dump_marks() {
        if (!trace_on || marks.empty()) return;
        for (size_t i = 1; i < marks.size(); ++i)
            fprintf(stderr, "[zkt host] %-28s %8.1f us\n", marks[i].first,
                    std::chrono::duration<double, std::micro>(marks[i].second - marks[i - 1].second).count());
        marks.clear();
    }

    void tr_commit(const char* label, const Affine<Q>& p) {
        uint8_t x[64], y[64];
        bool inf = aff_is_inf<Q>(p);
        if (!inf) {
            fq_to_le<Q>(p.x, x);
            fq_to_le<Q>(p.y, y);
        }
        tr.append_commitment(label, x, y, Q::N * 4, inf);
    }
    void tr_scalar(const char* label, const F& v) {
        uint8_t b[32];
        H::to_le_bytes(v, b);
        tr.append_scalars(label, b, 1, 32, true);
    }
    F tr_challenge(const char* label) {
        uint8_t b[32];
        tr.challenge_scalar(label, R::BITS, b);
        return H::from_le_bytes(b);
    }
    static void put(uint32_t dst[8], const F& v) { memcpy(dst, v.v, 32); }

    std::optional<ProfScope> idle;
    void wait_begin() {
        if (c->prof_on && !idle) idle.emplace(c, "host_wait");
    }
// ... 179 lines not shown
            size_t zero_idx = table_len;
            for (size_t i = 0; i < table_len; ++i)
                if (fe_is_zero<R>(keys[i])) {
                    zero_idx = i;
                    break;
                }
            if (n > table_len) {
                if (zero_idx == table_len) {
                    keys.push_back(fe_zero<R>());
                    counts.push_back(0);
                }
                counts[zero_idx] += (uint32_t)(n - table_len);
            }
            const uint32_t nk = (uint32_t)keys.size();
            if (nk + 2 > S.lk_cap) return set_err(c, ZKT_ERR_INVALID_ARGUMENT, "lookup table larger than the circuit bound");
            order.resize(nk);
            for (uint32_t i = 0; i < nk; ++i) order[i] = i;
            auto less = [&](uint32_t a, uint32_t b) {
                for (int i = R::N - 1; i >= 0; --i) {
                    if (keys[a].v[i] != keys[b].v[i]) return keys[a].v[i] < keys[b].v[i];
                }
                return false;
            };
            std::sort(order.begin(), order.end(), less);
            for (uint32_t i = 1; i < nk; ++i)
                if (!less(order[i - 1], order[i]))
                    return set_err(c, ZKT_ERR_INVALID_ARGUMENT, "lookup table holds a repeated value");
            sorted.resize(nk);
            for (uint32_t i = 0; i < nk; ++i) sorted[i] = keys[order[i]];
            ZKT_HIP(c, hipMemcpyAsync(d_keys, keys.data(), nk * 32, hipMemcpyHostToDevice, c->stream));
            ZKT_HIP(c, hipMemcpyAsync(d_sorted, sorted.data(), nk * 32, hipMemcpyHostToDevice, c->stream));
            ZKT_HIP(c, hipMemcpyAsync(d_perm, order.data(), nk * 4, hipMemcpyHostToDevice, c->stream));
            ZKT_HIP(c, hipMemcpyAsync(d_base, counts.data(), nk * 4, hipMemcpyHostToDevice, c->stream));
            ZKT_HIP(c, hipMemsetAsync(d_hits, 0, (size_t)nk * 4, c->stream));
            S.lk_nkeys = nk;
        }
        const uint32_t nk = S.lk_nkeys;
        int rc;
        if ((rc = lookup_count(c, S.ev[4], n, d_sorted, d_perm, nk, d_hits, S.status))) return rc;
        if ((rc = lookup_starts(c, d_base, d_hits, nk, n, d_even, d_odd, S.status))) return rc;
        if ((rc = lookup_expand(c, d_keys, d_even, nk, S.ev[5], n))) return rc;
        if ((rc = lookup_expand(c, d_keys, d_odd, nk, S.ev[6], n))) return rc;
        return ZKT_OK;
    }

    static bool same_inputs(const zkt_prove_inputs& a, const zkt_prove_inputs& b) {
        return a.a_evals == b.a_evals && a.b_evals == b.b_evals && a.c_evals == b.c_evals && a.n_rows == b.n_rows &&
               a.table == b.table && a.table_len == b.table_len && a.pi_pos == b.pi_pos && a.pi_vals == b.pi_vals &&
               a.n_pi == b.n_pi && a.blinders == b.blinders && a.wires_on_device == b.wires_on_device &&
               a.variables == b.variables && a.n_vars == b.n_vars && a.w_l == b.w_l && a.w_r == b.w_r && a.w_o == b.w_o;
    }
    int to_coset(int k) {
        static const int coset_src[W_COUNT] = {0, 1, 2, 8, 6, 7, 3, 4, 5};
        if (S.G == 1) return ntt_run(c, S.log_n + 2, 0, 1, S.poly[coset_src[k]], S.n + 8, S.wcos[k]);
        int rc = ntt_run_class(c, S.log_m, S.log_n + 2, S.cls, S.poly[coset_src[k]], S.n + 8, S.wcos[k], S.fold);
        if (rc || S.G < 8) return rc;
        static const int next_of[W_COUNT] = {-1, -1, -1, -1, 0, 1, 2, 3, -1};
        if (next_of[k] < 0) return ZKT_OK;
        return ntt_run_class(c, S.log_m, S.log_n + 2, (S.cls + 4) & 7, S.poly[coset_src[k]], S.n + 8, S.wnext[next_of[k]], S.fold);
    }

    int to_coset_many(std::initializer_list<int> ks) {
        static const int coset_src[W_COUNT] = {0, 1, 2, 8, 6, 7, 3, 4, 5};
        int rc;
        if (S.G != 1 || ks.size() > (size_t)NTT_MAX_BATCH) {
            for (int k : ks) if ((rc = to_coset(k))) return rc;
            return ZKT_OK;
        }
        const void* ins[NTT_MAX_BATCH];
        void* outs[NTT_MAX_BATCH];
        size_t lens[NTT_MAX_BATCH];
        int nb = 0;
        for (int k : ks) {
            ins[nb] = S.poly[coset_src[k]];
            outs[nb] = S.wcos[k];
            lens[nb] = S.n + 8;
            ++nb;
        }
        return nb ? ntt_run_batch(c, S.log_n + 2, 0, 1, nb, ins, lens, outs) : ZKT_OK;
    }

    void swap_work_sets() {
        for (int k = 0; k < 3; ++k) std::swap(S.poly[k], S.poly_alt[k]);
        std::swap(S.status, S.status_alt);
    }

    int enqueue_round_1(const zkt_prove_inputs& in) {
        const size_t n = S.n;
        int rc;
        ProfScope prof_round(c, "round1");
        if (in.n_rows > n) return set_err(c, ZKT_ERR_INVALID_ARGUMENT, "more rows than the circuit bound");
        if (in.table_len >= n) return set_err(c, ZKT_ERR_INVALID_ARGUMENT, "max table size is equal or larger than n");
        if (n < 8) return set_err(c, ZKT_ERR_INVALID_ARGUMENT, "circuit bound below 8");
        if (!in.blinders) return set_err(c, ZKT_ERR_INVALID_ARGUMENT, "null blinders");
        ZKT_HIP(c, hipMemsetAsync(S.status, 0, 64 * 4, c->stream));
        ZKT_HIP(c, hipMemcpyAsync(S.small, in.blinders, 19 * 32, hipMemcpyHostToDevice, c->stream));

        const uint64_t* wires[3] = {in.a_evals, in.b_evals, in.c_evals};
        const bool from_vars = in.a_evals == nullptr && in.variables != nullptr;
        const void* d_vars = in.variables;
        const uint32_t* d_idx[3] = {in.w_l, in.w_r, in.w_o};
        if (from_vars) {
            if (in.n_rows && (!in.w_l || !in.w_r || !in.w_o)) return set_err(c, ZKT_ERR_INVALID_ARGUMENT, "null wire index vector");
            if (in.n_vars > 0xFFFFFFFEull) return set_err(c, ZKT_ERR_INVALID_ARGUMENT, "too many variables");
            if (!in.wires_on_device) {
                if (in.n_vars > 4 * n || 3 * in.n_rows * 4 > (n + 8) * 32)
                    return set_err(c, ZKT_ERR_INVALID_ARGUMENT, "witness larger than the staging buffers");
                if (in.n_vars)
                    ZKT_HIP(c, hipMemcpyAsync(S.qev, in.variables, in.n_vars * 32, hipMemcpyHostToDevice, c->stream));
                d_vars = S.qev;
                for (int k = 0; k < 3; ++k) {
                    uint32_t* dst = (uint32_t*)S.poly[12] + (size_t)k * in.n_rows;
                    if (in.n_rows)
                        ZKT_HIP(c, hipMemcpyAsync(dst, d_idx[k], in.n_rows * 4, hipMemcpyHostToDevice, c->stream));
                    d_idx[k] = dst;
                }
            }
        }
        const bool host_wires = !from_vars && !in.wires_on_device;
        for (bool& r : S.wire_route) r = false;
        bool wire_tables = from_vars && in.wires_on_device && !c->sharded() && !c->lagrange_off && !S.wire_dense_only &&
                           lagrange_ready(c, S.log_n) && in.n_rows > 0;
        if (wire_tables) {
            const bool eliminate = S.wire_elim_force >= 0 ? S.wire_elim_force != 0
                                                          : c->wire_elim_mode == 2 || (c->wire_elim_mode == 1 && S.log_n >= WIRE_ELIM_MIN_LOG_N);
            WireElimKeys ek{};
            for (int k = 0; k < 5; ++k) ek.pk[k] = S.pk[PK_QM + k];
            ek.pi_pos = in.pi_pos;
            ek.n_pi = in.pi_pos ? in.n_pi : 0;
            if ((rc = wire_bases_prepare(c, S.log_n, d_idx, in.n_rows, in.n_vars, eliminate ? &ek : nullptr))) return rc;
            wire_tables = wire_bases_use(c, 0) || wire_bases_use(c, 1) || wire_bases_use(c, 2);
            if (wire_tables && (rc = wire_bases_digest(c, d_idx, in.n_rows))) return rc;
// ... 35 lines not shown
                    S.wire_route[k] = true;
                }
                rc = queueing() ? commit_push(sc, len, k, tbl) : tbl ? msm_begin(c, sc, len, 0, 1, k, tbl) : commit_begin(sc, len, k);
                if (rc) return rc;
            }
        }
        if ((rc = commit_flush())) return rc;
        return to_coset_many({W_A, W_B, W_C});
    }

    bool table_is_cached(const zkt_prove_inputs& in) const {
        return S.t_cached && S.t_srs_generation == c->srs_generation && S.cached_table.size() == 4 * in.table_len &&
               (in.table_len == 0 || memcmp(S.cached_table.data(), in.table, in.table_len * 32) == 0);
    }
    int enqueue_table(const zkt_prove_inputs& in, bool with_coset) {
        const size_t n = S.n;
        int rc;
        if (in.table_len >= n) return set_err(c, ZKT_ERR_INVALID_ARGUMENT, "max table size is equal or larger than n");
        S.t_cached = false;
        S.t_coset_valid = false;
        ZKT_HIP(c, hipMemsetAsync(S.ev[3], 0, n * 32, c->stream));
        if (in.table_len) ZKT_HIP(c, hipMemcpyAsync(S.ev[3], in.table, in.table_len * 32, hipMemcpyHostToDevice, c->stream));
        if ((rc = evals_to_blinded_poly(S.ev[3], S.poly[3], 0, 0, 3))) return rc;
        if ((rc = commit_evals_begin(S.ev[3], S.poly[3], 0, 0, 3, 3))) return rc;
        if (with_coset && (rc = to_coset(W_T))) return rc;
        return ZKT_OK;
    }

    int enqueue_round_2(const zkt_prove_inputs& in, bool* same_table_out, bool table_done = false) {
        const size_t n = S.n;
        int rc;
        ProfScope prof_round(c, "round2");
        const bool same_table = !table_done && table_is_cached(in);
        *same_table_out = same_table;
        if (!same_table && !table_done && (rc = enqueue_table(in, false))) return rc;
        if ((rc = poly_mul_vec(c, S.q_lookup_ev, S.ev[2], S.ev[4], n))) return rc;
        if ((rc = combine_split(in.table, in.table_len, !same_table))) return rc;
        {
            const PolyJob jobs[2] = {{S.ev[5], S.poly[4], 6, 3, 4}, {S.ev[6], S.poly[5], 9, 2, 5}};
            if ((rc = evals_to_blinded_polys(jobs, 2))) return rc;
        }
        if ((rc = commit_evals_begin(S.ev[5], S.poly[4], 6, 3, 4, 4))) return rc;
        if ((rc = commit_evals_begin(S.ev[6], S.poly[5], 9, 2, 5, 5))) return rc;
        if ((rc = commit_flush())) return rc;
        if (!S.t_coset_valid && !table_done) return to_coset_many({W_T, W_H1, W_H2});
        return to_coset_many({W_H1, W_H2});
    }

    int run(const zkt_prove_inputs& in, std::vector<uint8_t>& proof) {
        const size_t n = S.n;
        const int log_n = S.log_n;
        int rc;
        mark("start");
        bool same_table = false;
        if (S.prefetch_stage == 2 && S.prefetch_epoch == c->msm_epoch && same_inputs(S.prefetch_in, in)) {
            same_table = S.prefetch_same_table;
            swap_work_sets();
            S.prefetch_stage = 0;
        } else {
            S.prefetch_stage = 0;
            const bool table_first = !table_is_cached(in);
            if (table_first && in.a_evals && !in.wires_on_device) {
                ZKT_HIP(c, hipEventRecord(S.ev_copy[3], c->stream));
                ZKT_HIP(c, hipStreamWaitEvent(S.copy_stream, S.ev_copy[3], 0));
                copy_fenced = true;
            }
            if (table_first && (rc = enqueue_table(in, true))) return rc;
            if ((rc = enqueue_round_1(in))) return rc;
            if ((rc = enqueue_round_2(in, &same_table, table_first))) return rc;
        }

        {
            std::vector<uint8_t> b(in.n_pi * 32);
            for (size_t i = 0; i < in.n_pi; ++i) H::to_le_bytes(H::from_words(in.pi_vals + 4 * i), b.data() + 32 * i);
            tr.append_scalars("pi", b.data(), in.n_pi, 32, false);
        }
        Affine<Q> cm[11];
        mark("enqueue rounds 1+2");
        {
            static const int slots[6] = {0, 1, 2, 3, 4, 5};
            const bool skip[6] = {false, false, false, same_table, false, false};
            if ((rc = commit_collect(slots, skip, 6, cm))) return rc;
            if ((rc = collect_wires(cm))) return rc;
        }
        mark("wait commits of rounds 1+2");
        if (!same_table) {
            memcpy(S.t_commit_xy, cm[3].x.v, Q::N * 4);
            memcpy(S.t_commit_xy + Q::N / 2, cm[3].y.v, Q::N * 4);
            S.cached_table.assign(in.table, in.table + 4 * in.table_len);
            S.t_cached = true;
            S.t_srs_generation = c->srs_generation;
        } else {
            memcpy(cm[3].x.v, S.t_commit_xy, Q::N * 4);
            memcpy(cm[3].y.v, S.t_commit_xy + Q::N / 2, Q::N * 4);
        }
        static const char* L12[6] = {"a_commit", "b_commit", "c_commit", "t_commit", "h1_commit", "h2_commit"};
        for (int k = 0; k < 6; ++k) tr_commit(L12[k], cm[k]);
        mark("transcript rounds 1+2");

        const F beta = tr_challenge("beta"), gamma = tr_challenge("gamma"), delta = tr_challenge("delta"),
                epsilon = tr_challenge("epsilon");
        if (fe_eq<R>(beta, gamma) || fe_eq<R>(beta, delta) || fe_eq<R>(beta, epsilon) || fe_eq<R>(gamma, delta) ||
            fe_eq<R>(gamma, epsilon) || fe_eq<R>(delta, epsilon))
            return set_err(c, ZKT_ERR_EQUAL_CHALLENGES, "challenges must be different (prove.rs:202-207)");
        ZTermsArgs za{};
        za.a = S.ev[0]; za.b = S.ev[1]; za.c = S.ev[2];
        za.s1 = S.sigma_ev[0]; za.s2 = S.sigma_ev[1]; za.s3 = S.sigma_ev[2]; za.roots = S.roots;
        za.f = S.ev[4]; za.t = S.ev[3]; za.h1 = S.ev[5]; za.h2 = S.ev[6];
        za.num = S.sc[0]; za.den = S.sc[1]; za.n = n;
        put(za.beta, beta); put(za.gamma, gamma); put(za.delta, delta); put(za.epsilon, epsilon);
        F* pin = (F*)S.pinned;
        void* pn2 = S.wcos[W_Z1];
        void* sd2 = (char*)S.wcos[W_Z1] + n * 32;
        mark("challenges round 3");
        std::optional<ProfScope> prof_round;
        wait_end();
        prof_round.emplace(c, "round3");
        if ((rc = z1_terms(c, za))) return rc;
        if ((rc = scan_mul(c, S.sc[0], S.sc[2], n, false, S.scan_tmp))) return rc;
        if ((rc = scan_mul(c, S.sc[1], S.sc[3], n, true, S.scan_tmp))) return rc;
        if ((rc = z2_terms(c, za))) return rc;
        if ((rc = scan_mul(c, S.sc[0], pn2, n, false, S.scan_tmp))) return rc;
        if ((rc = scan_mul(c, S.sc[1], sd2, n, true, S.scan_tmp))) return rc;
        ZKT_HIP(c, hipMemcpyAsync(pin, S.sc[3], 32, hipMemcpyDeviceToHost, c->stream));
        ZKT_HIP(c, hipMemcpyAsync(pin + 1, sd2, 32, hipMemcpyDeviceToHost, c->stream));
        mark("enqueue grand products");
        if ((rc = check_status())) return rc;
        mark("wait grand products");
        if (fe_is_zero<R>(pin[0])) return set_err(c, ZKT_ERR_ZERO_DENOMINATOR, "zero denominator in the permutation grand product");
        if (fe_is_zero<R>(pin[1])) return set_err(c, ZKT_ERR_ZERO_DENOMINATOR, "zero denominator in the lookup grand product");
        {
            const F d1 = pin[0], d2 = pin[1];
            const F inv12 = fe_inv_host<R>(fe_mul<R>(d1, d2));
            const F inv1 = fe_mul<R>(inv12, d2), inv2 = fe_mul<R>(inv12, d1);
            wait_end();
            if ((rc = z_combine(c, S.sc[2], S.sc[3], inv1.v, S.ev[7], n))) return rc;
            if ((rc = z_combine(c, pn2, sd2, inv2.v, S.sc[0], n))) return rc;
            const PolyJob jobs[2] = {{S.ev[7], S.poly[6], 11, 3, 6}, {S.sc[0], S.poly[7], 14, 3, 7}};
            if ((rc = evals_to_blinded_polys(jobs, 2))) return rc;
        }
        {
            void* const z1p[1] = {S.poly[6]};
            const size_t z1l[1] = {n + 3};
            static const int z1s[1] = {0};
            if ((rc = commit_begin_many(z1p, z1l, z1s, 1))) return rc;
        }
        if ((rc = commit_evals_begin(S.sc[0], S.poly[7], 14, 3, 7, 1))) return rc;
        if ((rc = commit_flush())) return rc;
        if ((rc = to_coset_many({W_Z1, W_Z2}))) return rc;
        for (size_t i = 0; i < in.n_pi; ++i)
            if (in.pi_pos[i] >= n) return set_err(c, ZKT_ERR_INVALID_ARGUMENT, "public input position out of range");
        const bool pi_direct = in.n_pi <= (size_t)QUOTIENT_PI_DIRECT_MAX && S.G <= 4;
        if (pi_direct) {
            uint32_t* tab = (uint32_t*)S.pinned_pi;
            for (size_t i = 0; i < in.n_pi; ++i) {
                tab[10 * i] = (uint32_t)(4 * in.pi_pos[i] / (size_t)S.G);
                const Fx<R> v = fx_unpack<R>(H::from_words(in.pi_vals + 4 * i));
                for (int w = 0; w < 9; ++w) tab[10 * i + 1 + w] = v.l[w];
            }
            if (in.n_pi)
                ZKT_HIP(c, hipMemcpyAsync(S.pi_tab, tab, in.n_pi * 40, hipMemcpyHostToDevice, c->stream));
        } else {
            ZKT_HIP(c, hipMemsetAsync(S.ev[7], 0, n * 32, c->stream));
            for (size_t i = 0; i < in.n_pi; ++i)
                ZKT_HIP(c, hipMemcpyAsync((char*)S.ev[7] + in.pi_pos[i] * 32, in.pi_vals + 4 * i, 32, hipMemcpyHostToDevice, c->stream));
            if ((rc = evals_to_blinded_poly(S.ev[7], S.poly[8], 0, 0, 8))) return rc;
            if ((rc = to_coset(W_PI))) return rc;
        }
        {
            static const int slots[2] = {0, 1};
            if ((rc = commit_collect(slots, nullptr, 2, cm + 6))) return rc;
        }
        prof_round.reset();
        tr_commit("z1_commit", cm[6]);
        tr_commit("z2_commit", cm[7]);
        mark("round 3 finish + commits");

        const F alpha = tr_challenge("alpha");
        wait_end();
        prof_round.emplace(c, "round4");
        {
            S.t_coset_valid = S.t_cached;
            QuotientArgs q{};
            q.a = S.wcos[W_A]; q.b = S.wcos[W_B]; q.c = S.wcos[W_C]; q.pi = S.wcos[W_PI];
            q.z1 = S.wcos[W_Z1]; q.z2 = S.wcos[W_Z2]; q.t = S.wcos[W_T]; q.h1 = S.wcos[W_H1]; q.h2 = S.wcos[W_H2];
            q.q_m = S.coset[CS_QM]; q.q_l = S.coset[CS_QL]; q.q_r = S.coset[CS_QR]; q.q_o = S.coset[CS_QO];
            q.q_c = S.coset[CS_QC]; q.q_lookup = S.coset[CS_QLOOKUP]; q.q_table = S.coset[CS_QTABLE];
            q.sigma1 = S.coset[CS_S1]; q.sigma2 = S.coset[CS_S2]; q.sigma3 = S.coset[CS_S3];
            q.x = S.coset[CS_X]; q.l1 = S.coset[CS_L1];
            q.out = S.qev;
            put(q.alpha, alpha); put(q.beta, beta); put(q.gamma, gamma); put(q.delta, delta); put(q.epsilon, epsilon);
            memcpy(q.zh_inv, S.zh_inv, sizeof(q.zh_inv));
            q.n4 = S.m;
            q.pi_tab = pi_direct ? S.pi_tab : nullptr;
            q.n_pi_direct = pi_direct ? (uint32_t)in.n_pi : 0;
            if (S.G > 1) {
                q.G = (uint32_t)S.G;
                q.cls = (uint32_t)S.cls;
                q.next_off = S.G <= 4 ? 4u / (uint32_t)S.G : (uint32_t)((S.cls + 4) >> 3);
                q.z1_next = S.G == 8 ? S.wnext[0] : q.z1;
                q.z2_next = S.G == 8 ? S.wnext[1] : q.z2;
                q.t_next = S.G == 8 ? S.wnext[2] : q.t;
                q.h1_next = S.G == 8 ? S.wnext[3] : q.h1;
                const size_t pieces = ZKT_QUOTIENT_CHUNKS;
                if (comm_async_available(c) && S.comm_stream && S.m % pieces == 0 && S.m / pieces >= 1024) {
                    const size_t mp = S.m / pieces;
                    for (size_t j = 0; j < pieces; ++j) {
                        char* recv = (char*)S.qgather + j * (size_t)S.G * mp * 32;
                        char* mine = recv + (size_t)S.cls * mp * 32;
                        q.first = j * mp;
                        q.count = mp;
                        q.out = mine - q.first * 32;
                        if ((rc = quotient_pointwise(c, q))) return rc;
                        ZKT_HIP(c, hipEventRecord(S.ev_piece[j], c->stream));
                        ZKT_HIP(c, hipStreamWaitEvent(S.comm_stream, S.ev_piece[j], 0));
                        if ((rc = comm_all_gather_async(c, mine, recv, mp * 32, S.comm_stream))) return rc;
                    }
                    ZKT_HIP(c, hipEventRecord(S.ev_gathered, S.comm_stream));
                    ZKT_HIP(c, hipStreamWaitEvent(c->stream, S.ev_gathered, 0));
                    if ((rc = quotient_interleave(c, S.qgather, S.qev, 4 * n, (uint32_t)S.G, (uint32_t)pieces))) return rc;
                } else {
                    q.out = (char*)S.qgather + (size_t)S.cls * S.m * 32;
                    if ((rc = quotient_pointwise(c, q))) return rc;
                    if ((rc = comm_all_gather_dev(c, q.out, S.qgather, S.m * 32))) return rc;
                    if ((rc = quotient_interleave(c, S.qgather, S.qev, 4 * n, (uint32_t)S.G))) return rc;
                }
            } else if ((rc = quotient_pointwise(c, q))) {
                return rc;
            }
            if ((rc = ntt_run(c, log_n + 2, 1, 1, S.qev, 4 * n, S.qev))) return rc;
            if ((rc = quotient_split_blind(c, S.qev, n, (const char*)S.small + 17 * 32, S.poly[9], S.poly[10], S.poly[11], S.status)))
                return rc;
        }
        {
            void* const polys[3] = {S.poly[9], S.poly[10], S.poly[11]};
            const size_t lens[3] = {n + 3, n + 3, n + 3};
            static const int slots[3] = {8, 9, 10};
            if ((rc = commit_begin_many(polys, lens, slots, 3))) return rc;
            if ((rc = commit_flush())) return rc;
        }
        if (S.has_next) {
            S.has_next = false;
            swap_work_sets();
            const int r1 = enqueue_round_1(S.next_in);
            swap_work_sets();
            S.prefetch_stage = (r1 == ZKT_OK) ? 1 : 0;
        }
        {
            static const int slots[3] = {8, 9, 10};
            if ((rc = commit_collect(slots, nullptr, 3, cm + 8))) return rc;
        }
        prof_round.reset();
        tr_commit("q_lo_commit", cm[8]);
        tr_commit("q_mid_commit", cm[9]);
        tr_commit("q_hi_commit", cm[10]);
        mark("round 4");

        const F xi = tr_challenge("xi");
        wait_end();
        prof_round.emplace(c, "round5");
        F w;
        {
            Fe<R> g = root_of_unity<R>(log_n);
            w = g;
        }
        const F shifted = fe_mul<R>(xi, w);
        const size_t cap = n + 8;
        EvalArgs ea{};
        const void* ep[12] = {S.poly[0], S.poly[1], S.poly[2], S.pk[PK_S1], S.pk[PK_S2], S.poly[6],
                              S.pk[PK_QLOOKUP], S.poly[3], S.poly[3], S.poly[7], S.poly[4], S.poly[5]};
        const size_t el[12] = {cap, cap, cap, S.pk_len[PK_S1], S.pk_len[PK_S2], cap, S.pk_len[PK_QLOOKUP], cap, cap, cap, cap, cap};
        const bool sh[12] = {false, false, false, false, false, true, false, false, true, true, true, false};
        ea.count = 12;
        for (int k = 0; k < 12; ++k) {
            ea.poly[k] = ep[k];
            ea.len[k] = el[k];
            put(ea.point[k], sh[k] ? shifted : xi);
        }
        void* d_partials = (char*)S.small + 64 * 32;
        void* d_results = (char*)S.small + 32 * 32;
        if ((rc = poly_eval_many(c, ea, d_partials, d_results, S.eval_pw))) return rc;
        ZKT_HIP(c, hipMemcpyAsync(pin, d_results, 12 * 32, hipMemcpyDeviceToHost, c->stream));
        mark("enqueue evaluations");
// ... 11 lines not shown
        nn.v[1] = (uint32_t)((uint64_t)n >> 32);
        nn = fe_to_mont<R>(nn);
        const F l1den = fe_mul<R>(nn, fe_sub<R>(xi, one));
        if (fe_is_zero<R>(l1den)) return set_err(c, ZKT_ERR_ZERO_DENOMINATOR, "xi = 1");
        const F l1 = fe_mul<R>(zh, fe_inv_host<R>(l1den));
        const F a2 = fe_sqr<R>(alpha), a3 = fe_mul<R>(a2, alpha), a4 = fe_mul<R>(a3, alpha), a5 = fe_mul<R>(a4, alpha);
        const F k1 = fe_from_u32<R>(7), k2 = fe_from_u32<R>(13);
        const F bxi = fe_mul<R>(beta, xi);
        F s_z1 = fe_mul<R>(alpha, fe_add<R>(fe_add<R>(bxi, e_a), gamma));
        s_z1 = fe_mul<R>(s_z1, fe_add<R>(fe_add<R>(fe_mul<R>(bxi, k1), e_b), gamma));
        s_z1 = fe_mul<R>(s_z1, fe_add<R>(fe_add<R>(fe_mul<R>(bxi, k2), e_c), gamma));
        s_z1 = fe_add<R>(s_z1, fe_mul<R>(l1, a2));
        F s_s3 = fe_mul<R>(fe_neg<R>(alpha), beta);
        s_s3 = fe_mul<R>(s_s3, e_z1n);
        s_s3 = fe_mul<R>(s_s3, fe_add<R>(fe_add<R>(fe_mul<R>(beta, e_s1), e_a), gamma));
        s_s3 = fe_mul<R>(s_s3, fe_add<R>(fe_add<R>(fe_mul<R>(beta, e_s2), e_b), gamma));
        const F opd = fe_add<R>(delta, one), eopd = fe_mul<R>(epsilon, opd);
        F s_z2 = fe_mul<R>(a3, opd);
        s_z2 = fe_mul<R>(s_z2, fe_add<R>(epsilon, fe_mul<R>(e_ql, e_c)));
        s_z2 = fe_mul<R>(s_z2, fe_add<R>(fe_add<R>(eopd, e_t), fe_mul<R>(delta, e_tn)));
        s_z2 = fe_add<R>(s_z2, fe_mul<R>(a4, l1));
        F s_h1 = fe_mul<R>(fe_neg<R>(a3), e_z2n);
        s_h1 = fe_mul<R>(s_h1, fe_add<R>(fe_add<R>(eopd, e_h2), fe_mul<R>(delta, e_h1n)));
        const F s_qt = fe_mul<R>(a5, e_t);
        const F xn2 = fe_mul<R>(fe_mul<R>(fe_add<R>(zh, one), xi), xi);
        const F nzh = fe_neg<R>(zh);
        LinCombArgs lr{};
        auto term = [&](LinCombArgs& L, const void* p, size_t len, const F& s) {
            L.poly[L.nterms] = p;
            L.len[L.nterms] = len;
            put(L.scalar[L.nterms], s);
            ++L.nterms;
        };
        term(lr, S.pk[PK_QM], S.pk_len[PK_QM], fe_mul<R>(e_a, e_b));
        term(lr, S.pk[PK_QL], S.pk_len[PK_QL], e_a);
        term(lr, S.pk[PK_QR], S.pk_len[PK_QR], e_b);
        term(lr, S.pk[PK_QO], S.pk_len[PK_QO], e_c);
        term(lr, S.pk[PK_QC], S.pk_len[PK_QC], one);
        term(lr, S.poly[6], cap, s_z1);
        term(lr, S.pk[PK_S3], S.pk_len[PK_S3], s_s3);
        term(lr, S.poly[7], cap, s_z2);
        term(lr, S.poly[4], cap, s_h1);
        term(lr, S.pk[PK_QTABLE], S.pk_len[PK_QTABLE], s_qt);
        term(lr, S.poly[9], cap, nzh);
        term(lr, S.poly[10], cap, fe_mul<R>(nzh, xn2));
        term(lr, S.poly[11], cap, fe_mul<R>(nzh, fe_sqr<R>(xn2)));
        static const char* EL[12] = {"a_eval", "b_eval", "c_eval", "sigma1_eval", "sigma2_eval", "z1_next_eval",
                                     "q_lookup_eval", "t_eval", "t_next_eval", "z2_next_eval", "h1_next_eval", "h2_eval"};
        for (int k = 0; k < 12; ++k) tr_scalar(EL[k], ev[k]);
        const F eta = tr_challenge("eta");
        void* work = S.poly[12];
        wait_end();
        if ((rc = poly_lincomb(c, lr, work, cap))) return rc;
        auto witness = [&](const void* comb, const F& z, void* ta, void* tb, void* scan, void* out, void* pw) -> int {
            if (fe_is_zero<R>(z)) {
                ZKT_HIP(c, hipMemcpyAsync(out, (const char*)comb + 32, (cap - 1) * 32, hipMemcpyDeviceToDevice, c->stream));
                return ZKT_OK;
            }
            const F zi = fe_inv_host<R>(z);
            return open_witness(c, comb, cap, z.v, zi.v, ta, tb, scan, out, pw);
        };
        Affine<Q> aw, saw;
        {
            LinCombArgs lo{};
            F pw = one;
            term(lo, work, cap, pw);
            const void* ps[8] = {S.poly[0], S.poly[1], S.poly[2], S.pk[PK_S1], S.pk[PK_S2], S.pk[PK_QLOOKUP], S.poly[3], S.poly[5]};
            const size_t pl[8] = {cap, cap, cap, S.pk_len[PK_S1], S.pk_len[PK_S2], S.pk_len[PK_QLOOKUP], cap, cap};
            for (int k = 0; k < 8; ++k) {
                pw = fe_mul<R>(pw, eta);
                term(lo, ps[k], pl[k], pw);
            }
            void* comb = S.sc[0];
            if ((rc = poly_lincomb(c, lo, comb, cap))) return rc;
            if ((rc = witness(comb, xi, S.sc[1], S.sc[2], S.scan_tmp, S.sc[3], S.eval_pw))) return rc;
        }
        const bool aux = S.aux_stream != nullptr && !c->aux_off;
        void* comb2 = aux ? S.wcos[W_Z1] : S.sc[0];
        void* ta2 = aux ? (void*)((char*)S.wcos[W_Z1] + cap * 32) : S.sc[1];
        void* tb2 = aux ? (void*)((char*)S.wcos[W_Z1] + 2 * cap * 32) : S.sc[2];
        void* out2 = aux ? S.wcos[W_Z2] : S.sc[3];
        auto second_opening = [&]() -> int {
            LinCombArgs lo{};
            F pw = one;
            const void* ps[4] = {S.poly[6], S.poly[7], S.poly[3], S.poly[4]};
            for (int k = 0; k < 4; ++k) {
                term(lo, ps[k], cap, pw);
                pw = fe_mul<R>(pw, eta);
            }
            int r2;
            if ((r2 = poly_lincomb(c, lo, comb2, cap))) return r2;
            return witness(comb2, shifted, ta2, tb2, aux ? S.aux_scan_tmp : S.scan_tmp, out2, aux ? S.aux_pw : S.eval_pw);
        };
        if (aux) {
            ZKT_HIP(c, hipEventRecord(S.ev_aux_go, c->stream));
            ZKT_HIP(c, hipStreamWaitEvent(S.aux_stream, S.ev_aux_go, 0));
            hipStream_t main_stream = c->stream;
            c->stream = S.aux_stream;
            const int r2 = second_opening();
            c->stream = main_stream;
            if (r2) return r2;
            ZKT_HIP(c, hipEventRecord(S.ev_aux_done, S.aux_stream));
        }
        const bool both = aux && queueing();
        if (!both && (rc = commit_begin(S.sc[3], cap - 1, 6))) return rc;
        {
            if (aux) ZKT_HIP(c, hipStreamWaitEvent(c->stream, S.ev_aux_done, 0));
            else if ((rc = second_opening())) return rc;
            if (both) {
                void* const wp[2] = {S.sc[3], out2};
                const size_t wl[2] = {cap - 1, cap - 1};
                static const int ws[2] = {6, 7};
                if ((rc = commit_begin_many(wp, wl, ws, 2))) return rc;
            } else if ((rc = commit_begin(out2, cap - 1, 7))) {
                return rc;
            }
            if ((rc = commit_flush())) return rc;
            if (S.prefetch_stage == 1) {
                bool st = false;
                swap_work_sets();
                const int r2 = enqueue_round_2(S.next_in, &st);
                swap_work_sets();
                if (r2 == ZKT_OK) {
                    S.prefetch_stage = 2;
                    S.prefetch_in = S.next_in;
                    S.prefetch_same_table = st;
                    S.prefetch_epoch = c->msm_epoch;
                } else {
                    S.prefetch_stage = 0;
                }
            }
            {
                static const int slots[2] = {6, 7};
                Affine<Q> w2[2];
                if ((rc = commit_collect(slots, nullptr, 2, w2))) return rc;
                aw = w2[0];
                saw = w2[1];
            }
        }
        wait_end();
        prof_round.reset();

        proof.clear();
        for (int k = 0; k < 11; ++k) serialize_point<Q>(cm[k], proof);
        serialize_point<Q>(aw, proof);
        proof.push_back(0);
        serialize_point<Q>(saw, proof);
        proof.push_back(0);
        for (int k = 0; k < 12; ++k) {
            uint8_t b[32];
            H::to_le_bytes(ev[k], b);
            proof.insert(proof.end(), b, b + 32);
        }
        mark("round 5 finish");
        dump_marks();
        return ZKT_OK;
    }
};

void circuit_release(zkt_ctx* c) {
    if (!c->circuit) return;
    (void)hipStreamSynchronize(c->stream);
    CircuitState& S = *c->circuit;
    if (S.copy_stream) (void)hipStreamSynchronize(S.copy_stream);
    auto fr = [&](void* p) { dev_free(c, p); };
    if (!S.keys_borrowed) {
        for (void* p : S.pk) fr(p);
        for (void* p : S.coset) fr(p);
        for (void* p : S.sigma_ev) fr(p);
        fr(S.q_lookup_ev); fr(S.roots);
    }
    for (void* p : S.ev) fr(p);
    for (void* p : S.sc) fr(p);
    fr(S.scan_tmp);
    for (void* p : S.poly) fr(p);
    for (void* p : S.wcos) fr(p);
    for (void* p : S.wnext) fr(p);
    fr(S.fold); fr(S.qgather);
    for (void* p : S.poly_alt) fr(p);
    fr(S.status_alt);
    fr(S.aux_scan_tmp); fr(S.aux_pw);
    for (void* q : S.lag_scalars_q) fr(q);
    wire_bases_drop(c);
    if (S.aux_stream) {
        (void)hipStreamSynchronize(S.aux_stream);
        (void)hipStreamDestroy(S.aux_stream);
    }
    if (S.ev_aux_go) (void)hipEventDestroy(S.ev_aux_go);
    if (S.ev_aux_done) (void)hipEventDestroy(S.ev_aux_done);
    fr(S.qev); fr(S.small); fr(S.lag_scalars); fr(S.status); fr(S.lk_u32); fr(S.lk_keys); fr(S.pi_tab); fr(S.eval_pw);
    if (S.pinned) (void)hipHostFree(S.pinned);
    if (S.pinned_pi) (void)hipHostFree(S.pinned_pi);
    if (S.copy_stream) {
        (void)hipStreamSynchronize(S.copy_stream);
        (void)hipStreamDestroy(S.copy_stream);
    }
    for (auto e : S.ev_copy) if (e) (void)hipEventDestroy(e);
    if (S.comm_stream) {
        (void)hipStreamSynchronize(S.comm_stream);
        (void)hipStreamDestroy(S.comm_stream);
    }
    for (auto e : S.ev_piece) if (e) (void)hipEventDestroy(e);
    if (S.ev_gathered) (void)hipEventDestroy(S.ev_gathered);
    c->circuit.reset();
}

static int circuit_alloc_work(zkt_ctx* c, CircuitState& S) {
    const size_t n = S.n, m = S.m;
    int rc;
    auto alloc = [&](void** p, size_t elems) { return dev_alloc(c, p, elems * 32); };
    if ((rc = alloc(&S.qev, 4 * n))) return rc;
    if (S.G > 1) {
        if ((rc = alloc(&S.fold, m))) return rc;
        if ((rc = alloc(&S.qgather, 4 * n))) return rc;
        if (S.G == 8) for (auto& p : S.wnext) if ((rc = alloc(&p, m))) return rc;
    }
    for (auto& p : S.ev) if ((rc = alloc(&p, n + 8))) return rc;
    for (auto& p : S.sc) if ((rc = alloc(&p, n + 8))) return rc;
    if ((rc = alloc(&S.scan_tmp, 2 * ((n + 8) / 1024 + 4096)))) return rc;
    for (auto& p : S.poly) if ((rc = alloc(&p, n + 8))) return rc;
    for (int k = 0; k < W_COUNT; ++k)
        if ((rc = alloc(&S.wcos[k], k == W_Z1 ? std::max(m, 2 * n) : m))) return rc;
    const size_t eval_blocks = (n + 8 + 2047) / 2048 + 1;
    if ((rc = alloc(&S.small, 64 + 16 * eval_blocks))) return rc;
    if ((rc = alloc(&S.lag_scalars, n + 16))) return rc;
    for (auto& q : S.lag_scalars_q) if ((rc = alloc(&q, n + 16))) return rc;
    if ((rc = dev_alloc(c, (void**)&S.status, 64 * 4))) return rc;
    if ((rc = dev_alloc(c, (void**)&S.status_alt, 64 * 4))) return rc;
    for (auto& p : S.poly_alt) if ((rc = alloc(&p, n + 8))) return rc;
    S.lk_cap = n + 2;
    if ((rc = dev_alloc(c, (void**)&S.lk_u32, 5 * S.lk_cap * 4 + 16))) return rc;
    if ((rc = alloc(&S.lk_keys, 2 * S.lk_cap))) return rc;
    ZKT_HIP(c, hipHostMalloc(&S.pinned, 64 * 32));
    ZKT_HIP(c, hipStreamCreateWithFlags(&S.copy_stream, hipStreamNonBlocking));
    if (S.G > 1) {
        ZKT_HIP(c, hipStreamCreateWithFlags(&S.comm_stream, hipStreamNonBlocking));
        for (auto& e : S.ev_piece) ZKT_HIP(c, hipEventCreateWithFlags(&e, hipEventDisableTiming));
        ZKT_HIP(c, hipEventCreateWithFlags(&S.ev_gathered, hipEventDisableTiming));
    }
    for (auto& e : S.ev_copy) ZKT_HIP(c, hipEventCreateWithFlags(&e, hipEventDisableTiming));
    ZKT_HIP(c, hipHostMalloc(&S.pinned_pi, QUOTIENT_PI_DIRECT_MAX * 40));
    if ((rc = dev_alloc(c, (void**)&S.pi_tab, QUOTIENT_PI_DIRECT_MAX * 40))) return rc;
    if ((rc = alloc(&S.eval_pw, std::max((size_t)EVAL_MAX * (257 + eval_blocks), open_witness_powers(n + 8))))) return rc;
    if (S.G == 1) {
        if ((rc = alloc(&S.aux_scan_tmp, 2 * ((n + 8) / 1024 + 4096)))) return rc;
        if ((rc = alloc(&S.aux_pw, open_witness_powers(n + 8)))) return rc;
        ZKT_HIP(c, hipStreamCreateWithFlags(&S.aux_stream, hipStreamNonBlocking));
        ZKT_HIP(c, hipEventCreateWithFlags(&S.ev_aux_go, hipEventDisableTiming));
        ZKT_HIP(c, hipEventCreateWithFlags(&S.ev_aux_done, hipEventDisableTiming));
    }
    return ZKT_OK;
}

int circuit_fork(zkt_ctx* child, const zkt_ctx* parent) {
    circuit_release(child);
    if (!parent->circuit) return ZKT_OK;
    const CircuitState& P0 = *parent->circuit;
    auto st = std::make_shared<CircuitState>();
    CircuitState& S = *st;
    S.log_n = P0.log_n; S.n = P0.n; S.G = P0.G; S.cls = P0.cls; S.log_m = P0.log_m; S.m = P0.m;
    for (int k = 0; k < PK_COUNT; ++k) { S.pk[k] = P0.pk[k]; S.pk_len[k] = P0.pk_len[k]; }
    for (int k = 0; k < CS_COUNT; ++k) S.coset[k] = P0.coset[k];
    for (int k = 0; k < 3; ++k) S.sigma_ev[k] = P0.sigma_ev[k];
    S.q_lookup_ev = P0.q_lookup_ev;
    S.roots = P0.roots;
    memcpy(S.zh_inv, P0.zh_inv, sizeof(S.zh_inv));
    S.keys_borrowed = true;
    child->circuit = st;
    const int rc = circuit_alloc_work(child, S);
    if (rc) circuit_release(child);
    return rc;
}

template <class C>
static int circuit_load_t(zkt_ctx* c, int log_n, const uint64_t* const* polys, const size_t* lens, bool from_evals = false,
                          unsigned evals_dev_mask = 0) {
    using R = typename C::Fr;
    using F = Fe<R>;
    if (log_n < 3 || log_n + 2 > R::TWO_ADICITY || log_n + 2 > 27)
        return set_err(c, ZKT_ERR_INVALID_DOMAIN_SIZE, "InvalidEvalDomainSize: 4n domain unsupported");
    if (int rf = refuse_if_forked(c, "loading a circuit")) return rf;
    circuit_release(c);
    auto st = std::make_shared<CircuitState>();
    CircuitState& S = *st;
    S.log_n = log_n;
    const size_t n = (size_t)1 << log_n;
    S.n = n;
    S.G = c->sharded() ? c->comm.vt.world : 1;
    S.cls = c->sharded() ? c->comm.vt.rank : 0;
    S.log_m = log_n + 2 - (S.G == 8 ? 3 : S.G == 4 ? 2 : S.G == 2 ? 1 : 0);
    S.m = (size_t)1 << S.log_m;
    const size_t m = S.m;
    int rc;
    auto alloc = [&](void** p, size_t elems) { return dev_alloc(c, p, elems * 32); };
    if ((rc = circuit_alloc_work(c, S))) return rc;
    for (int k = 0; k < PK_COUNT; ++k) {
        if (lens[k] > n) return set_err(c, ZKT_ERR_INVALID_ARGUMENT, "prover-key polynomial longer than n");
        if ((rc = alloc(&S.pk[k], n))) return rc;
        if (from_evals) {
            const void* src = polys[k];
            const bool on_device = (evals_dev_mask >> k) & 1u;
            if (!on_device) {
                ZKT_HIP(c, hipMemsetAsync(S.qev, 0, n * 32, c->stream));
                if (lens[k]) ZKT_HIP(c, hipMemcpyAsync(S.qev, polys[k], lens[k] * 32, hipMemcpyHostToDevice, c->stream));
                src = S.qev;
            }
            if ((rc = ntt_run(c, log_n, 1, 0, src, on_device ? lens[k] : n, S.pk[k]))) return rc;
            S.pk_len[k] = n;
        } else {
            ZKT_HIP(c, hipMemsetAsync(S.pk[k], 0, n * 32, c->stream));
            if (lens[k]) ZKT_HIP(c, hipMemcpyAsync(S.pk[k], polys[k], lens[k] * 32, hipMemcpyHostToDevice, c->stream));
            S.pk_len[k] = lens[k];
        }
    }
    for (int k = 0; k < CS_COUNT; ++k) if ((rc = alloc(&S.coset[k], m))) return rc;
    for (int k = 0; k < 3; ++k) if ((rc = alloc(&S.sigma_ev[k], n))) return rc;
    if ((rc = alloc(&S.q_lookup_ev, n))) return rc;
    if ((rc = alloc(&S.roots, n))) return rc;

    const int pk_of_cs[10] = {PK_QM, PK_QL, PK_QR, PK_QO, PK_QC, PK_QLOOKUP, PK_QTABLE, PK_S1, PK_S2, PK_S3};
// ... 355 lines not shown
    if (!c->circuit) return set_err(c, ZKT_ERR_NOT_LOADED, "no circuit loaded (zkt_circuit_load)");
    if (!c->msm) return set_err(c, ZKT_ERR_NOT_LOADED, "no SRS loaded (zkt_srs_load)");
    if (int rc0 = check_sharded_key(c)) return rc0;
    (void)hipSetDevice(c->device);
    if (!c->lagrange_off)
        if (int rc1 = lagrange_ensure(c, c->circuit->log_n)) return rc1;
    std::vector<uint8_t> proof;
    int rc;
    if (c->curve == ZKT_CURVE_BN254) {
        Prover<Bn254Curve> p(c, *c->circuit, tr);
        rc = p.run(*in, proof);
        if (rc) {
            (void)hipStreamSynchronize(c->circuit->copy_stream);
            if (c->circuit->comm_stream) (void)hipStreamSynchronize(c->circuit->comm_stream);
            if (c->circuit->aux_stream) (void)hipStreamSynchronize(c->circuit->aux_stream);
            (void)hipStreamSynchronize(c->stream);
        }
    } else {
        Prover<Bls381Curve> p(c, *c->circuit, tr);
        rc = p.run(*in, proof);
        if (rc) {
            (void)hipStreamSynchronize(c->circuit->copy_stream);
            if (c->circuit->comm_stream) (void)hipStreamSynchronize(c->circuit->comm_stream);
            if (c->circuit->aux_stream) (void)hipStreamSynchronize(c->circuit->aux_stream);
            (void)hipStreamSynchronize(c->stream);
        }
    }
    if (rc) {
        c->circuit->has_next = false;
        c->circuit->prefetch_stage = 0;
        return rc;
    }
    if (len) *len = proof.size();
    if (proof.size() > cap) return set_err(c, ZKT_ERR_INVALID_ARGUMENT, "proof buffer too small");
    memcpy(out, proof.data(), proof.size());
    return ZKT_OK;
}

int zkt_ctx_set_lagrange(zkt_ctx* c, int on) {
    if (!c) return ZKT_ERR_INVALID_ARGUMENT;
    c->lagrange_off = !on;
    ++c->msm_epoch;
    return ZKT_OK;
}

int zkt_ctx_set_wire_elimination(zkt_ctx* c, int mode) {
    if (!c) return ZKT_ERR_INVALID_ARGUMENT;
    if (mode < 0 || mode > 2) return set_err(c, ZKT_ERR_INVALID_ARGUMENT, "mode: 0 off, 1 automatic, 2 whenever a table can be built");
    c->wire_elim_mode = mode;
    ++c->msm_epoch;
    return ZKT_OK;
}

int zkt_lagrange_info(zkt_ctx* c, int* log_n, size_t* bases) {
    if (!c) return ZKT_ERR_INVALID_ARGUMENT;
    const bool ready = c->circuit && lagrange_ready(c, c->circuit->log_n) && !c->lagrange_off;
    if (log_n) *log_n = ready ? c->circuit->log_n : -1;
    if (bases) *bases = ready ? lagrange_bases(c) : 0;
    return ZKT_OK;
}

int zkt_commit_evals_dev(zkt_ctx* c, const void* d_evals, const uint64_t* blinders, int k, int path, uint64_t* out_xy,
                         int* out_is_infinity) {
    if (!c || !d_evals || !out_xy || (k > 0 && !blinders)) return set_err(c, ZKT_ERR_INVALID_ARGUMENT, "null pointer");
    if (k < 0 || k > 3) return set_err(c, ZKT_ERR_INVALID_ARGUMENT, "0 .. 3 blinders");
    if (!c->circuit) return set_err(c, ZKT_ERR_NOT_LOADED, "no circuit loaded (the domain comes from it)");
    if (!c->msm) return set_err(c, ZKT_ERR_NOT_LOADED, "no SRS loaded (zkt_srs_load)");
    if (c->sharded()) return set_err(c, ZKT_ERR_INVALID_ARGUMENT, "not available on a sharded key");
    (void)hipSetDevice(c->device);
    CircuitState& S = *c->circuit;
    const size_t n = S.n;
    int rc;
    if (path == 1) {
        if ((rc = lagrange_ensure(c, S.log_n))) return rc;
        if (!lagrange_ready(c, S.log_n)) return set_err(c, ZKT_ERR_NOT_LOADED, "the key is too short for the Lagrange-basis table");
    } else if (path != 0) {
        return set_err(c, ZKT_ERR_INVALID_ARGUMENT, "path: 0 coefficients, 1 Lagrange basis");
    }
    c->circuit->prefetch_stage = 0;
    uint32_t* d_len = S.status + 8 + 12;
    void* d_bl = (char*)S.lag_scalars + (n + 8) * 32;
    void* poly = S.poly[12];
    ZKT_HIP(c, hipMemsetAsync(d_len, 0, 4, c->stream));
    if (k) ZKT_HIP(c, hipMemcpyAsync(d_bl, blinders, (size_t)k * 32, hipMemcpyHostToDevice, c->stream));
    if ((rc = ntt_run(c, S.log_n, 1, 0, d_evals, n, poly))) return rc;
    if ((rc = poly_trim_len(c, poly, n, d_len, (char*)poly + n * 32, 8))) return rc;
    if (k && (rc = poly_add_blinders(c, poly, d_len, d_bl, k, n + 8))) return rc;
    if (path == 0) return msm_g1_dev(c, poly, n + (size_t)k, 0, 1, out_xy, out_is_infinity);
    if ((rc = lagrange_scalars(c, d_evals, n, d_len, d_bl, k, S.roots, S.lag_scalars))) return rc;
    if ((rc = msm_begin(c, S.lag_scalars, n + (size_t)k, 0, 1, 0, 1))) return rc;
    uint64_t xy[12] = {};
    if ((rc = msm_end(c, 0, xy))) return rc;
    const size_t words = c->curve == ZKT_CURVE_BN254 ? 8 : 12;
    memcpy(out_xy, xy, words * 8);
    if (out_is_infinity) {
        bool any = false;
        for (size_t i = 0; i < words; ++i) any = any || xy[i] != 0;
        *out_is_infinity = any ? 0 : 1;
    }
    return ZKT_OK;
}

int zkt_circuit_setup(zkt_ctx* c, int log_n, const uint64_t* const* evals, const size_t* eval_lens, int evals_on_device,
                      uint64_t* out_commitments, int* out_is_infinity) {
    if (!c || !evals || !eval_lens || !out_commitments) return set_err(c, ZKT_ERR_INVALID_ARGUMENT, "null pointer");
    if (!c->msm) return set_err(c, ZKT_ERR_NOT_LOADED, "no SRS loaded (zkt_srs_load)");
// ... 358 lines not shown
```

Before: 60.69 proofs/s.

## Compute quotient on three coset classes and recover top coefficients on host

Adds a quotient route that evaluates the constraint quotient on three of the four 4n coset classes instead of the whole extended coset. The missing information, the six top coefficients, is reconstructed on the host from small coefficient windows using low-degree product convolutions. A Vandermonde-inverse combine kernel then rebuilds the coefficient form. Folded-head inputs to the forward NTT let the three class transforms share one batch. The aim is to cut about a quarter of the extended-domain NTT and quotient-evaluation work, at the price of extra small kernels, a host round-trip for the window gather, and more complex correctness logic.

```diff
diff --git a/include/zkt_plonk.h b/include/zkt_plonk.h
--- a/include/zkt_plonk.h
+++ b/include/zkt_plonk.h
@@ -99,6 +99,7 @@
 
 int zkt_ctx_set_lagrange(zkt_ctx* ctx, int on);
 int zkt_ctx_set_wire_elimination(zkt_ctx* ctx, int mode);
+int zkt_ctx_set_quotient_route(zkt_ctx* ctx, int mode);
 int zkt_lagrange_info(zkt_ctx* ctx, int* log_n, size_t* bases);
 int zkt_commit_evals_dev(zkt_ctx* ctx, const void* d_evals, const uint64_t* blinders, int k, int path, uint64_t* out_xy_mont,
                          int* out_is_infinity);
@@ -312,6 +313,10 @@
 int zkt_debug_pairing_selftest(int curve_id);
 int zkt_debug_quotient(zkt_ctx* ctx, const uint64_t* challenges, const uint64_t* const* wit, const uint64_t* pi_pos,
                        const uint64_t* pi_vals, size_t n_pi, uint64_t* out);
+int zkt_debug_quotient_top(zkt_ctx* ctx, uint64_t* out_u, int* out_on_classes);
+int zkt_debug_quotient_coeffs(zkt_ctx* ctx, uint64_t* out, size_t count);
+int zkt_debug_quotient_classes_host(int curve, int log_n, const uint64_t* windows, const uint64_t* challenges, uint64_t* out_u,
+                                    uint64_t* out_consts);
 int zkt_debug_grand_products(zkt_ctx* ctx, const uint64_t* challenges, const uint64_t* const* vectors, uint64_t* out_z1,
                              uint64_t* out_z2);
 int zkt_debug_combine_split(zkt_ctx* ctx, const uint64_t* table, size_t table_len, const uint64_t* f, int fresh,
diff --git a/shim/src/ffi.rs b/shim/src/ffi.rs
--- a/shim/src/ffi.rs
+++ b/shim/src/ffi.rs
@@ -93,6 +93,7 @@
                                 out_xy_mont: *mut u64, out_is_infinity: *mut c_int) -> c_int;
     pub fn zkt_ctx_set_lagrange(ctx: *mut ZktCtx, on: c_int) -> c_int;
     pub fn zkt_ctx_set_wire_elimination(ctx: *mut ZktCtx, mode: c_int) -> c_int;
+    pub fn zkt_ctx_set_quotient_route(ctx: *mut ZktCtx, mode: c_int) -> c_int;
     pub fn zkt_lagrange_info(ctx: *mut ZktCtx, log_n: *mut c_int, bases: *mut usize) -> c_int;
     pub fn zkt_circuit_load(ctx: *mut ZktCtx, log_n: c_int, pk_polys: *const *const u64, pk_lens: *const usize) -> c_int;
     pub fn zkt_circuit_load_file(ctx: *mut ZktCtx, pk_path: *const c_char, log_n: c_int) -> c_int;
diff --git a/zkt-plonk_amd/_lib.py b/zkt-plonk_amd/_lib.py
--- a/zkt-plonk_amd/_lib.py
+++ b/zkt-plonk_amd/_lib.py
@@ -538,6 +538,20 @@
     return out, bool(inf.value)
 
 
+def quotient_classes_host(curve, log_n: int, windows, challenges):
+    L = lib()
+    w = np.ascontiguousarray(windows, dtype=np.uint64).reshape(10, 14, 4)
+    ch = np.ascontiguousarray(challenges, dtype=np.uint64).reshape(3, 4)
+    u = np.zeros((6, 4), dtype=np.uint64)
+    consts = np.zeros((16, 4), dtype=np.uint64)
+    P64 = ctypes.POINTER(ctypes.c_uint64)
+    L.zkt_debug_quotient_classes_host.argtypes = [ctypes.c_int, ctypes.c_int, P64, P64, P64, P64]
+    rc = L.zkt_debug_quotient_classes_host(curve_id(curve), int(log_n), u64p(w), u64p(ch), u64p(u), u64p(consts))
+    if rc:
+        raise ZktError(rc, "zkt_debug_quotient_classes_host")
+    return u, consts
+
+
 def wire_elimination(curve, selectors, w_l, w_r, w_o, n_vars: int, pi_pos=(), K: int = 16):
     L = lib()
     sel = [np.ascontiguousarray(q, dtype=np.uint64).reshape(-1, 4) for q in selectors]
@@ -1346,6 +1360,23 @@
         self.check(self._L.zkt_debug_open_witness(self._h, u64p(p_), p_.shape[0], u64p(zz), u64p(out)))
         return out
 
+    def set_quotient_route(self, mode: int = 0):
+        self._L.zkt_ctx_set_quotient_route.argtypes = [ctypes.c_void_p, ctypes.c_int]
+        self.check(self._L.zkt_ctx_set_quotient_route(self._h, int(mode)))
+
+    def debug_quotient_top(self):
+        u = np.zeros((6, 4), dtype=np.uint64)
+        on = ctypes.c_int(0)
+        self._L.zkt_debug_quotient_top.argtypes = [ctypes.c_void_p, ctypes.POINTER(ctypes.c_uint64), ctypes.POINTER(ctypes.c_int)]
+        self.check(self._L.zkt_debug_quotient_top(self._h, u64p(u), ctypes.byref(on)))
+        return u, bool(on.value)
+
+    def debug_quotient_coeffs(self, count: int) -> np.ndarray:
+        out = np.zeros((count, 4), dtype=np.uint64)
+        self._L.zkt_debug_quotient_coeffs.argtypes = [ctypes.c_void_p, ctypes.POINTER(ctypes.c_uint64), ctypes.c_size_t]
+        self.check(self._L.zkt_debug_quotient_coeffs(self._h, u64p(out), int(count)))
+        return out
+
     def debug_quotient(self, n: int, challenges, wit, pi_pos=(), pi_vals=None) -> np.ndarray:
         ch = np.ascontiguousarray(challenges, dtype=np.uint64).reshape(5, 4)
         keep = [None if w is None else np.ascontiguousarray(w, dtype=np.uint64).reshape(4 * n, 4) for w in wit]
diff --git a/zkt-plonk_amd/csrc/capi.hip b/zkt-plonk_amd/csrc/capi.hip
--- a/zkt-plonk_amd/csrc/capi.hip
+++ b/zkt-plonk_amd/csrc/capi.hip
@@ -226,6 +226,7 @@
     (void)hipStreamSynchronize(parent->stream);
     c->lagrange_off = parent->lagrange_off;
     c->wire_elim_mode = parent->wire_elim_mode;
+    c->quotient_route = parent->quotient_route;
     c->batch_off = parent->batch_off;
     c->aux_off = parent->aux_off;
     c->ntt_plans = parent->ntt_plans;
diff --git a/zkt-plonk_amd/csrc/ctx.hpp b/zkt-plonk_amd/csrc/ctx.hpp
--- a/zkt-plonk_amd/csrc/ctx.hpp
+++ b/zkt-plonk_amd/csrc/ctx.hpp
@@ -74,6 +74,7 @@
     bool batch_off = false;
     bool lagrange_off = false;
     int wire_elim_mode = 1;
+    int quotient_route = 0;
     std::shared_ptr<zkt::CircuitState> circuit;
     std::vector<void*> owned;
 };
@@ -120,7 +121,8 @@
 Fe<P> root_of_unity(int log_n);
 int ntt_run(zkt_ctx* c, int log_n, int inverse, int coset, const void* d_in, size_t in_len, void* d_out);
 int ntt_run_batch(zkt_ctx* c, int log_n, int inverse, int coset, int nb, const void* const* d_in, const size_t* in_len,
-                  void* const* d_out);
+                  void* const* d_out, const void* d_head = nullptr);
+int ntt_fold_heads(zkt_ctx* c, int nb, const void* const* d_in, size_t n, const uint32_t* gammas, void* d_out);
 int ntt_class_code(int log_big, int cls);
 int ntt_force_split(zkt_ctx* c, int npass, const int* log_r);
 int ntt_run_class(zkt_ctx* c, int log_n, int log_big, int cls, const void* d_in, size_t in_len, void* d_out, void* d_fold);
diff --git a/zkt-plonk_amd/csrc/ntt.hip b/zkt-plonk_amd/csrc/ntt.hip
--- a/zkt-plonk_amd/csrc/ntt.hip
+++ b/zkt-plonk_amd/csrc/ntt.hip
@@ -1,6 +1,7 @@
 #include "ctx.hpp"
 #include "hostinv.hpp"
 #include <cstdlib>
+#include <cstring>
 
 namespace zkt {
 
@@ -223,7 +224,9 @@
             const uint4* rlo = reinterpret_cast<const uint4*>(in_p);
             x = tile_get<P>(rlo, rlo + a.raw_n, reinterpret_cast<const uint32_t*>(rlo + 2 * a.raw_n), (int64_t)g);
         } else {
-            x = (g < in_len) ? fx_unpack<P>(fe_load<P>(in + g)) : fx_zero<P>();
+            const Fe<P>* src = in + g;
+            if (a.head && g < NTT_HEAD) src = reinterpret_cast<const Fe<P>*>(a.head) + py * NTT_HEAD + g;
+            x = (g < in_len) ? fx_unpack<P>(fe_load<P>(src)) : fx_zero<P>();
         }
         if (in_row && (a.in_raw || g < in_len)) x = fx_mul<P>(x, fx_unpack<P>(fe_load<P>(in_row + r)));
         if (tw) {
@@ -281,12 +284,12 @@
 template <class P>
 __global__ __launch_bounds__(NTT_THREADS) void k_ntt_small(const Fe<P>* in, uint64_t in_len, Fe<P>* out, int log_n,
                                                            const Fe<P>* w, const Fe<P>* in_scale,
-                                                           const Fe<P>* out_scale) {
+                                                           const Fe<P>* out_scale, const Fe<P>* head) {
     __shared__ Fe<P> buf[TILE];
     const int n = 1 << log_n;
     const int tid = threadIdx.x;
     for (int i = tid; i < n; i += NTT_THREADS) {
-        Fe<P> x = ((uint64_t)i < in_len) ? fe_load<P>(in + i) : fe_zero<P>();
+        Fe<P> x = ((uint64_t)i < in_len) ? fe_load<P>(head && i < NTT_HEAD ? head + i : in + i) : fe_zero<P>();
         if (in_scale) x = fe_mul<P>(x, fe_load<P>(in_scale + i));
         buf[i] = x;
     }
@@ -602,7 +605,7 @@
 
 template <class P>
 static int ntt_run_batch_t(zkt_ctx* c, int log_n, int inverse, int coset, int nb, const void* const* d_in, const size_t* in_len,
-                           void* const* d_out) {
+                           void* const* d_out, const void* d_head = nullptr) {
     if (nb < 1 || nb > NTT_MAX_BATCH) return set_err(c, ZKT_ERR_INVALID_ARGUMENT, "transform batch out of range");
     if (log_n < 0 || log_n > P::TWO_ADICITY)
         return set_err(c, ZKT_ERR_INVALID_DOMAIN_SIZE,
@@ -630,7 +633,8 @@
         for (int y = 0; y < nb; ++y)
             hipLaunchKernelGGL(k_ntt_small<P>, dim3(1), dim3(NTT_THREADS), 0, c->stream, (const Fe<P>*)d_in[y],
                                (uint64_t)in_len[y], (Fe<P>*)d_out[y], log_n, (const Fe<P>*)pl.small_w,
-                               (const Fe<P>*)pl.small_in, (const Fe<P>*)pl.small_out);
+                               (const Fe<P>*)pl.small_in, (const Fe<P>*)pl.small_out,
+                               d_head ? (const Fe<P>*)d_head + (size_t)y * NTT_HEAD : nullptr);
         ZKT_HIP(c, hipGetLastError());
         return 0;
     }
@@ -651,6 +655,7 @@
         a.w_inner = pl.w_inner[i];
         a.w_inner_s = pl.w_inner_s[i];
         a.in_row = (i == 0) ? pl.in_row : nullptr;
+        a.head = (i == 0) ? d_head : nullptr;
         a.tw = pl.tw[i];
         a.out_row = last ? pl.out_row : nullptr;
         a.log_n = (uint32_t)log_n;
@@ -677,9 +682,39 @@
 }
 
 int ntt_run_batch(zkt_ctx* c, int log_n, int inverse, int coset, int nb, const void* const* d_in, const size_t* in_len,
-                  void* const* d_out) {
-    if (c->curve == ZKT_CURVE_BN254) return ntt_run_batch_t<Bn254Fr>(c, log_n, inverse, coset, nb, d_in, in_len, d_out);
-    return ntt_run_batch_t<Bls381Fr>(c, log_n, inverse, coset, nb, d_in, in_len, d_out);
+                  void* const* d_out, const void* d_head) {
+    if (d_head && (inverse || log_n < 3)) return set_err(c, ZKT_ERR_INVALID_ARGUMENT, "folded heads go with forward transforms of 8 points and more");
+    if (c->curve == ZKT_CURVE_BN254) return ntt_run_batch_t<Bn254Fr>(c, log_n, inverse, coset, nb, d_in, in_len, d_out, d_head);
+    return ntt_run_batch_t<Bls381Fr>(c, log_n, inverse, coset, nb, d_in, in_len, d_out, d_head);
+}
+
+template <class P>
+struct FoldHeadsArgs {
+    const Fe<P>* in[NTT_MAX_BATCH];
+    Fe<P> gamma[3];
+};
+template <class P>
+__global__ void k_fold_heads(FoldHeadsArgs<P> a, uint64_t n, int nb, Fe<P>* out) {
+    const int t = threadIdx.x;
+    const int i = t % NTT_HEAD, y = (t / NTT_HEAD) % NTT_MAX_BATCH, j = t / (NTT_HEAD * NTT_MAX_BATCH);
+    if (j >= 3 || y >= nb) return;
+    const Fe<P>* in = y == 0 ? a.in[0] : y == 1 ? a.in[1] : y == 2 ? a.in[2] : a.in[3];
+    const Fe<P> g = j == 0 ? a.gamma[0] : j == 1 ? a.gamma[1] : a.gamma[2];
+    fe_store<P>(out + t, fe_add<P>(fe_load<P>(in + i), fe_mul<P>(g, fe_load<P>(in + n + i))));
+}
+template <class P>
+static int ntt_fold_heads_t(zkt_ctx* c, int nb, const void* const* d_in, size_t n, const uint32_t* gammas, void* d_out) {
+    FoldHeadsArgs<P> a{};
+    for (int y = 0; y < NTT_MAX_BATCH; ++y) a.in[y] = (const Fe<P>*)d_in[y < nb ? y : 0];
+    for (int j = 0; j < 3; ++j) memcpy(a.gamma[j].v, gammas + 8 * j, 32);
+    hipLaunchKernelGGL(k_fold_heads<P>, dim3(1), dim3(3 * NTT_MAX_BATCH * NTT_HEAD), 0, c->stream, a, (uint64_t)n, nb, (Fe<P>*)d_out);
+    ZKT_HIP(c, hipGetLastError());
+    return ZKT_OK;
+}
+int ntt_fold_heads(zkt_ctx* c, int nb, const void* const* d_in, size_t n, const uint32_t* gammas, void* d_out) {
+    if (nb < 1 || nb > NTT_MAX_BATCH) return set_err(c, ZKT_ERR_INVALID_ARGUMENT, "transform batch out of range");
+    if (c->curve == ZKT_CURVE_BN254) return ntt_fold_heads_t<Bn254Fr>(c, nb, d_in, n, gammas, d_out);
+    return ntt_fold_heads_t<Bls381Fr>(c, nb, d_in, n, gammas, d_out);
 }
 
 int ntt_run(zkt_ctx* c, int log_n, int inverse, int coset, const void* d_in, size_t in_len, void* d_out) {
diff --git a/zkt-plonk_amd/csrc/ntt.hpp b/zkt-plonk_amd/csrc/ntt.hpp
--- a/zkt-plonk_amd/csrc/ntt.hpp
+++ b/zkt-plonk_amd/csrc/ntt.hpp
@@ -5,6 +5,7 @@
 
 namespace zkt {
 
+constexpr int NTT_HEAD = 8;
 constexpr int NTT_MAX_BATCH = 4;
 
 struct NttPassArgs {
@@ -16,6 +17,7 @@
     const void* tw;
     const void* out_row;
     uint64_t in_len[NTT_MAX_BATCH];
+    const void* head;
     uint32_t log_n;
     uint32_t log_s;
     uint32_t log_r1;
diff --git a/zkt-plonk_amd/csrc/poly.hip b/zkt-plonk_amd/csrc/poly.hip
--- a/zkt-plonk_amd/csrc/poly.hip
+++ b/zkt-plonk_amd/csrc/poly.hip
@@ -889,6 +889,87 @@
     ZKT_DISPATCH(c, quot_split_t, q, n, d_b0b1, q_lo, q_mid, q_hi, d_status);
 }
 
+
+template <class P>
+__global__ void k_classes_of_coset(const Fe<P>* in, Fe<P>* out, uint64_t n) {
+    const uint64_t i = (uint64_t)blockIdx.x * blockDim.x + threadIdx.x;
+    if (i >= n) return;
+#pragma unroll
+    for (int j = 0; j < 3; ++j) fe_store<P>(out + (uint64_t)j * n + i, fe_load<P>(in + 4 * i + j));
+}
+template <class P> static int classes_of_coset_t(zkt_ctx* c, const void* in, void* out, size_t n) {
+    hipLaunchKernelGGL(k_classes_of_coset<P>, dim3(nblocks(n)), dim3(256), 0, c->stream, (const Fe<P>*)in, (Fe<P>*)out, (uint64_t)n);
+    ZKT_HIP(c, hipGetLastError());
+    return ZKT_OK;
+}
+int quotient_classes_of_coset(zkt_ctx* c, const void* in, void* out, size_t n) { ZKT_DISPATCH(c, classes_of_coset_t, in, out, n); }
+
+struct WindowPtrs {
+    const void* p[QC_WIN_POLYS];
+};
+template <class P>
+__global__ void k_gather_windows(WindowPtrs w, uint64_t first, Fe<P>* out) {
+    const int t = threadIdx.x;
+    if (t >= QC_WIN_POLYS * QC_WIN) return;
+    const int k = t / QC_WIN, i = t % QC_WIN;
+    const void* p = w.p[0];
+#pragma unroll
+    for (int e = 1; e < QC_WIN_POLYS; ++e) p = (k == e) ? w.p[e] : p;
+    fe_store<P>(out + t, fe_load<P>((const Fe<P>*)p + first + i));
+}
+template <class P> static int gather_windows_t(zkt_ctx* c, const void* const* polys, size_t first, void* out) {
+    WindowPtrs w{};
+    for (int k = 0; k < QC_WIN_POLYS; ++k) w.p[k] = polys[k];
+    hipLaunchKernelGGL(k_gather_windows<P>, dim3(1), dim3(128), 0, c->stream, w, (uint64_t)first, (Fe<P>*)out);
+    ZKT_HIP(c, hipGetLastError());
+    return ZKT_OK;
+}
+int quotient_gather_windows(zkt_ctx* c, const void* const* polys, size_t first, void* out) {
+    static_assert(QC_WIN_POLYS * QC_WIN <= 128, "one workgroup of 128");
+    ZKT_DISPATCH(c, gather_windows_t, polys, first, out);
+}
+
+template <class P>
+struct CombineArgs {
+    Fe<P> vinv[9];
+    Fe<P> u[6];
+    Fe<P> g3[3];
+};
+template <class P>
+__global__ __launch_bounds__(256) void k_classes_combine(Fe<P>* q, uint64_t n, CombineArgs<P> a) {
+    const uint64_t i = (uint64_t)blockIdx.x * blockDim.x + threadIdx.x;
+    if (i >= n) return;
+    const Fe<P> e0 = fe_load<P>(q + i), e1 = fe_load<P>(q + n + i), e2 = fe_load<P>(q + 2 * n + i);
+    Fe<P> t[4];
+#pragma unroll
+    for (int k = 0; k < 3; ++k)
+        t[k] = fe_add<P>(fe_add<P>(fe_mul<P>(a.vinv[3 * k], e0), fe_mul<P>(a.vinv[3 * k + 1], e1)), fe_mul<P>(a.vinv[3 * k + 2], e2));
+    t[3] = fe_zero<P>();
+    if (i < 6) {
+        Fe<P> u = a.u[0];
+#pragma unroll
+        for (int e = 1; e < 6; ++e) u = (i == (uint64_t)e) ? a.u[e] : u;
+        t[3] = u;
+        t[2] = fe_add<P>(t[2], fe_mul<P>(u, a.g3[0]));
+        t[1] = fe_add<P>(t[1], fe_mul<P>(u, a.g3[1]));
+        t[0] = fe_add<P>(t[0], fe_mul<P>(u, a.g3[2]));
+    }
+#pragma unroll
+    for (int k = 0; k < 4; ++k) fe_store<P>(q + (uint64_t)k * n + i, t[k]);
+}
+template <class P> static int classes_combine_t(zkt_ctx* c, void* q, size_t n, const uint32_t* vinv, const uint32_t* u, const uint32_t* g3) {
+    CombineArgs<P> a{};
+    for (int k = 0; k < 9; ++k) a.vinv[k] = host_fe<P>(vinv + 8 * k);
+    for (int k = 0; k < 6; ++k) a.u[k] = host_fe<P>(u + 8 * k);
+    for (int k = 0; k < 3; ++k) a.g3[k] = host_fe<P>(g3 + 8 * k);
+    hipLaunchKernelGGL(k_classes_combine<P>, dim3(nblocks(n)), dim3(256), 0, c->stream, (Fe<P>*)q, (uint64_t)n, a);
+    ZKT_HIP(c, hipGetLastError());
+    return ZKT_OK;
+}
+int quotient_classes_combine(zkt_ctx* c, void* q, size_t n, const uint32_t* vinv, const uint32_t* u, const uint32_t* g3) {
+    ZKT_DISPATCH(c, classes_combine_t, q, n, vinv, u, g3);
+}
+
 int open_elems(size_t len) { return ow_elems(len); }
 size_t open_blocks(size_t len) { return ow_blocks(len); }
 template <class P> static int open_pow_tables_t(zkt_ctx* c, const uint32_t* z, const uint32_t* zinv, void* d_powers, size_t len) {
diff --git a/zkt-plonk_amd/csrc/poly.hpp b/zkt-plonk_amd/csrc/poly.hpp
--- a/zkt-plonk_amd/csrc/poly.hpp
+++ b/zkt-plonk_amd/csrc/poly.hpp
@@ -63,6 +63,10 @@
 int quotient_interleave(zkt_ctx* c, const void* in, void* out, size_t n4, uint32_t G, uint32_t chunks = 1);
 int quotient_split_blind(zkt_ctx* c, const void* q, size_t n, const void* d_b0b1, void* q_lo, void* q_mid, void* q_hi,
                          uint32_t* d_status);
+constexpr int QC_WIN = 14, QC_WIN_POLYS = 6;
+int quotient_classes_of_coset(zkt_ctx* c, const void* in, void* out, size_t n);
+int quotient_gather_windows(zkt_ctx* c, const void* const* polys, size_t first, void* out);
+int quotient_classes_combine(zkt_ctx* c, void* q, size_t n, const uint32_t* vinv, const uint32_t* u, const uint32_t* g3);
 int open_witness(zkt_ctx* c, const void* p, size_t len, const uint32_t z[8], const uint32_t z_inv[8], void* d_tmp_a, void* d_tmp_b,
                  void* d_scan_tmp, void* out, void* d_powers );
 size_t open_witness_powers(size_t maxlen);
diff --git a/zkt-plonk_amd/csrc/prover.hip b/zkt-plonk_amd/csrc/prover.hip
--- a/zkt-plonk_amd/csrc/prover.hip
+++ b/zkt-plonk_amd/csrc/prover.hip
@@ -7,6 +7,7 @@
 #include "keyfile.hpp"
 #include "msm.hpp"
 #include "poly.hpp"
+#include "quotient_classes.hpp"
 #include "transcript.hpp"
 
 #include <algorithm>
@@ -79,6 +80,17 @@
     bool wire_route[3] = {};
     bool wire_dense_only = false;
     int wire_elim_force = -1;
+    void* ccoset[CS_COUNT] = {};
+    bool ccoset_borrowed = false, ccoset_ready = false;
+    uint32_t key_win[4][QCW][8] = {};
+    uint32_t qc_gamma[4][8] = {}, qc_vinv[9][8] = {}, qc_g3[3][8] = {};
+    bool use_classes = false;
+    void* heads = nullptr;
+    void* d_win = nullptr;
+    void* pinned_win = nullptr;
+    hipEvent_t ev_win = nullptr;
+    uint32_t last_u[6][8] = {};
+    bool last_u_valid = false;
 };
 
 template <class P>
@@ -130,6 +142,7 @@
 }
 
 constexpr int WIRE_ELIM_MIN_LOG_N = 17;
+constexpr int QUOTIENT_CLASSES_MIN_LOG_N = 20;
 
 template <class C>
 struct Prover {
@@ -415,6 +428,7 @@
     }
     int to_coset(int k) {
         static const int coset_src[W_COUNT] = {0, 1, 2, 8, 6, 7, 3, 4, 5};
+        if (S.use_classes) return to_coset_classes(&k, 1);
         if (S.G == 1) return ntt_run(c, S.log_n + 2, 0, 1, S.poly[coset_src[k]], S.n + 8, S.wcos[k]);
         int rc = ntt_run_class(c, S.log_m, S.log_n + 2, S.cls, S.poly[coset_src[k]], S.n + 8, S.wcos[k], S.fold);
         if (rc || S.G < 8) return rc;
@@ -423,9 +437,33 @@
         return ntt_run_class(c, S.log_m, S.log_n + 2, (S.cls + 4) & 7, S.poly[coset_src[k]], S.n + 8, S.wnext[next_of[k]], S.fold);
     }
 
+    int to_coset_classes(const int* ks, int nb) {
+        static const int coset_src[W_COUNT] = {0, 1, 2, 8, 6, 7, 3, 4, 5};
+        const void* ins[NTT_MAX_BATCH];
+        void* outs[NTT_MAX_BATCH];
+        size_t lens[NTT_MAX_BATCH];
+        int rc;
+        for (int y = 0; y < nb; ++y) {
+            ins[y] = S.poly[coset_src[ks[y]]];
+            lens[y] = S.n;
+        }
+        if ((rc = ntt_fold_heads(c, nb, ins, S.n, &S.qc_gamma[0][0], S.heads))) return rc;
+        for (int j = 0; j < 3; ++j) {
+            for (int y = 0; y < nb; ++y) outs[y] = (char*)S.wcos[ks[y]] + (size_t)j * S.n * 32;
+            const void* head = (const char*)S.heads + (size_t)j * NTT_MAX_BATCH * NTT_HEAD * 32;
+            if ((rc = ntt_run_batch(c, S.log_n, 0, ntt_class_code(S.log_n + 2, j), nb, ins, lens, outs, head))) return rc;
+        }
+        return ZKT_OK;
+    }
+
     int to_coset_many(std::initializer_list<int> ks) {
         static const int coset_src[W_COUNT] = {0, 1, 2, 8, 6, 7, 3, 4, 5};
         int rc;
+        if (S.use_classes && ks.size() <= (size_t)NTT_MAX_BATCH) {
+            int kk[NTT_MAX_BATCH], nb = 0;
+            for (int k : ks) kk[nb++] = k;
+            return nb ? to_coset_classes(kk, nb) : ZKT_OK;
+        }
         if (S.G != 1 || ks.size() > (size_t)NTT_MAX_BATCH) {
             for (int k : ks) if ((rc = to_coset(k))) return rc;
             return ZKT_OK;
@@ -441,6 +479,40 @@
             ++nb;
         }
         return nb ? ntt_run_batch(c, S.log_n + 2, 0, 1, nb, ins, lens, outs) : ZKT_OK;
+    }
+
+    int ensure_class_tables() {
+        if (S.ccoset_ready) return ZKT_OK;
+        const size_t n = S.n;
+        int rc;
+        for (int k = 0; k < CS_COUNT; ++k) {
+            if (!S.ccoset[k] && (rc = dev_alloc(c, &S.ccoset[k], 3 * n * 32))) return rc;
+            if ((rc = quotient_classes_of_coset(c, S.coset[k], S.ccoset[k], n))) return rc;
+        }
+        static const int key_of[4] = {PK_S1, PK_S2, PK_S3, PK_QLOOKUP};
+        memset(S.key_win, 0, sizeof(S.key_win));
+        for (int k = 0; k < 4; ++k)
+            ZKT_HIP(c, hipMemcpyAsync(S.key_win[k], (const char*)S.pk[key_of[k]] + (n - 6) * 32, 6 * 32, hipMemcpyDeviceToHost, c->stream));
+        ZKT_HIP(c, hipStreamSynchronize(c->stream));
+        const QuotientClassConsts<R> q = quotient_class_consts<R>(S.log_n);
+        for (int j = 0; j < 4; ++j) put(S.qc_gamma[j], q.gamma[j]);
+        for (int j = 0; j < 9; ++j) put(S.qc_vinv[j], q.vinv[j]);
+        for (int j = 0; j < 3; ++j) put(S.qc_g3[j], q.g3[j]);
+        S.ccoset_ready = true;
+        return ZKT_OK;
+    }
+    int choose_route() {
+        int mode = c->quotient_route;
+        if (const char* e = exp_env("ZKT_QUOTIENT_ROUTE")) mode = atoi(e);
+        const bool want = !c->sharded() && S.G == 1 && (mode == 1 || (mode == 0 && S.log_n >= QUOTIENT_CLASSES_MIN_LOG_N));
+        if (want)
+            if (int rc = ensure_class_tables()) return rc;
+        if (want != S.use_classes) {
+            S.use_classes = want;
+            S.t_coset_valid = false;
+            S.prefetch_stage = 0;
+        }
+        return ZKT_OK;
     }
 
     void swap_work_sets() {
@@ -582,6 +654,8 @@
         const int log_n = S.log_n;
         int rc;
         mark("start");
+        if ((rc = choose_route())) return rc;
+        const bool classes = S.use_classes;
         bool same_table = false;
         if (S.prefetch_stage == 2 && S.prefetch_epoch == c->msm_epoch && same_inputs(S.prefetch_in, in)) {
             same_table = S.prefetch_same_table;
@@ -669,6 +743,12 @@
             const PolyJob jobs[2] = {{S.ev[7], S.poly[6], 11, 3, 6}, {S.sc[0], S.poly[7], 14, 3, 7}};
             if ((rc = evals_to_blinded_polys(jobs, 2))) return rc;
         }
+        if (classes) {
+            const void* const wp[QC_WIN_POLYS] = {S.poly[0], S.poly[1], S.poly[2], S.poly[6], S.poly[7], S.poly[3]};
+            if ((rc = quotient_gather_windows(c, wp, n - 6, S.d_win))) return rc;
+            ZKT_HIP(c, hipMemcpyAsync(S.pinned_win, S.d_win, QC_WIN_POLYS * QC_WIN * 32, hipMemcpyDeviceToHost, c->stream));
+            ZKT_HIP(c, hipEventRecord(S.ev_win, c->stream));
+        }
         {
             void* const z1p[1] = {S.poly[6]};
             const size_t z1l[1] = {n + 3};
@@ -684,7 +764,7 @@
         if (pi_direct) {
             uint32_t* tab = (uint32_t*)S.pinned_pi;
             for (size_t i = 0; i < in.n_pi; ++i) {
-                tab[10 * i] = (uint32_t)(4 * in.pi_pos[i] / (size_t)S.G);
+                tab[10 * i] = (uint32_t)(4 * in.pi_pos[i] / (size_t)(classes ? 4 : S.G));
                 const Fx<R> v = fx_unpack<R>(H::from_words(in.pi_vals + 4 * i));
                 for (int w = 0; w < 9; ++w) tab[10 * i + 1 + w] = v.l[w];
             }
@@ -724,7 +804,41 @@
             q.n4 = S.m;
             q.pi_tab = pi_direct ? S.pi_tab : nullptr;
             q.n_pi_direct = pi_direct ? (uint32_t)in.n_pi : 0;
-            if (S.G > 1) {
+            if (classes) {
+                q.G = 4;
+                q.next_off = 1;
+                q.n4 = n;
+                const void** in_ptrs[] = {&q.a, &q.b, &q.c, &q.pi, &q.z1, &q.z2, &q.t, &q.h1, &q.h2};
+                const int cs_of[12] = {CS_QM, CS_QL, CS_QR, CS_QO, CS_QC, CS_QLOOKUP, CS_QTABLE, CS_S1, CS_S2, CS_S3, CS_X, CS_L1};
+                const void** key_ptrs[12] = {&q.q_m, &q.q_l, &q.q_r, &q.q_o, &q.q_c, &q.q_lookup, &q.q_table,
+                                             &q.sigma1, &q.sigma2, &q.sigma3, &q.x, &q.l1};
+                static const int w_of[9] = {W_A, W_B, W_C, W_PI, W_Z1, W_Z2, W_T, W_H1, W_H2};
+                for (int j = 0; j < 3; ++j) {
+                    const size_t off = (size_t)j * n * 32;
+                    for (int k = 0; k < 9; ++k) *in_ptrs[k] = (const char*)S.wcos[w_of[k]] + off;
+                    for (int k = 0; k < 12; ++k) *key_ptrs[k] = (const char*)S.ccoset[cs_of[k]] + off;
+                    q.cls = (uint32_t)j;
+                    q.z1_next = q.z1; q.z2_next = q.z2; q.t_next = q.t; q.h1_next = q.h1;
+                    q.out = (char*)S.qev + off;
+                    if ((rc = quotient_pointwise(c, q))) return rc;
+                }
+                for (int j = 0; j < 3; ++j) {
+                    void* e = (char*)S.qev + (size_t)j * n * 32;
+                    if ((rc = ntt_run(c, log_n, 1, ntt_class_code(log_n + 2, j), e, n, e))) return rc;
+                }
+                ZKT_HIP(c, hipEventSynchronize(S.ev_win));
+                const uint32_t* pw = (const uint32_t*)S.pinned_win;
+                QuotientWindows W{};
+                W.a = pw; W.b = pw + QCW * 8; W.c = pw + 2 * QCW * 8; W.z1 = pw + 3 * QCW * 8; W.z2 = pw + 4 * QCW * 8;
+                W.t = pw + 5 * QCW * 8;
+                W.sigma1 = &S.key_win[0][0][0]; W.sigma2 = &S.key_win[1][0][0]; W.sigma3 = &S.key_win[2][0][0];
+                W.q_lookup = &S.key_win[3][0][0];
+                F u[6];
+                quotient_top_coefficients<R>(log_n, W, alpha, beta, delta, u);
+                for (int e = 0; e < 6; ++e) put(S.last_u[e], u[e]);
+                S.last_u_valid = true;
+                if ((rc = quotient_classes_combine(c, S.qev, n, &S.qc_vinv[0][0], &S.last_u[0][0], &S.qc_g3[0][0]))) return rc;
+            } else if (S.G > 1) {
                 q.G = (uint32_t)S.G;
                 q.cls = (uint32_t)S.cls;
                 q.next_off = S.G <= 4 ? 4u / (uint32_t)S.G : (uint32_t)((S.cls + 4) >> 3);
@@ -758,7 +872,7 @@
             } else if ((rc = quotient_pointwise(c, q))) {
                 return rc;
             }
-            if ((rc = ntt_run(c, log_n + 2, 1, 1, S.qev, 4 * n, S.qev))) return rc;
+            if (!classes && (rc = ntt_run(c, log_n + 2, 1, 1, S.qev, 4 * n, S.qev))) return rc;
             if ((rc = quotient_split_blind(c, S.qev, n, (const char*)S.small + 17 * 32, S.poly[9], S.poly[10], S.poly[11], S.status)))
                 return rc;
         }
@@ -876,6 +990,16 @@
         void* work = S.poly[12];
         wait_end();
         if ((rc = poly_lincomb(c, lr, work, cap))) return rc;
+        if (classes) {
+            EvalArgs er{};
+            er.count = 1;
+            er.poly[0] = work;
+            er.len[0] = cap;
+            put(er.point[0], xi);
+            if ((rc = poly_eval_many(c, er, d_partials, d_results, S.eval_pw))) return rc;
+            ZKT_HIP(c, hipMemcpyAsync(pin + 16, d_results, 32, hipMemcpyDeviceToHost, c->stream));
+            ZKT_HIP(c, hipEventRecord(S.ev_win, c->stream));
+        }
         auto witness = [&](const void* comb, const F& z, void* ta, void* tb, void* scan, void* out, void* pw) -> int {
             if (fe_is_zero<R>(z)) {
                 ZKT_HIP(c, hipMemcpyAsync(out, (const char*)comb + 32, (cap - 1) * 32, hipMemcpyDeviceToDevice, c->stream));
@@ -964,6 +1088,39 @@
         }
         wait_end();
         prof_round.reset();
+        if (classes) {
+            F r0 = fe_zero<R>();
+            std::vector<F> root(in.n_pi), den(in.n_pi), before(in.n_pi);
+            F run_prod = one;
+            for (size_t i = 0; i < in.n_pi; ++i) {
+                root[i] = fe_pow_u64<R>(w, (uint64_t)in.pi_pos[i]);
+                den[i] = fe_mul<R>(nn, fe_sub<R>(xi, root[i]));
+                before[i] = run_prod;
+                if (!fe_is_zero<R>(den[i])) run_prod = fe_mul<R>(run_prod, den[i]);
+            }
+            F inv_all = in.n_pi ? fe_inv_host<R>(run_prod) : one;
+            for (size_t i = in.n_pi; i-- > 0;) {
+                const F v = H::from_words(in.pi_vals + 4 * i);
+                if (fe_is_zero<R>(den[i])) {
+                    r0 = fe_sub<R>(r0, v);
+                    continue;
+                }
+                const F di = fe_mul<R>(inv_all, before[i]);
+                inv_all = fe_mul<R>(inv_all, den[i]);
+                r0 = fe_sub<R>(r0, fe_mul<R>(fe_mul<R>(fe_mul<R>(zh, root[i]), di), v));
+            }
+            F p2 = fe_mul<R>(alpha, e_z1n);
+            p2 = fe_mul<R>(p2, fe_add<R>(fe_add<R>(e_a, fe_mul<R>(beta, e_s1)), gamma));
+            p2 = fe_mul<R>(p2, fe_add<R>(fe_add<R>(e_b, fe_mul<R>(beta, e_s2)), gamma));
+            p2 = fe_mul<R>(p2, fe_add<R>(e_c, gamma));
+            F p4 = fe_mul<R>(a3, e_z2n);
+            p4 = fe_mul<R>(p4, fe_add<R>(eopd, fe_mul<R>(delta, e_h2)));
+            p4 = fe_mul<R>(p4, fe_add<R>(fe_add<R>(eopd, e_h2), fe_mul<R>(delta, e_h1n)));
+            r0 = fe_add<R>(fe_add<R>(r0, p2), fe_add<R>(fe_mul<R>(l1, a2), fe_add<R>(p4, fe_mul<R>(l1, a4))));
+            ZKT_HIP(c, hipEventSynchronize(S.ev_win));
+            if (!fe_eq<R>(pin[16], r0))
+                return set_err(c, ZKT_ERR_QUOTIENT_TOO_SHORT, "the opening identity fails at xi: the circuit is not satisfied");
+        }
 
         proof.clear();
         for (int k = 0; k < 11; ++k) serialize_point<Q>(cm[k], proof);
@@ -999,6 +1156,10 @@
     fr(S.scan_tmp);
     for (void* p : S.poly) fr(p);
     for (void* p : S.wcos) fr(p);
+    if (!S.ccoset_borrowed) for (void* p : S.ccoset) fr(p);
+    fr(S.heads); fr(S.d_win);
+    if (S.pinned_win) (void)hipHostFree(S.pinned_win);
+    if (S.ev_win) (void)hipEventDestroy(S.ev_win);
     for (void* p : S.wnext) fr(p);
     fr(S.fold); fr(S.qgather);
     for (void* p : S.poly_alt) fr(p);
@@ -1044,11 +1205,17 @@
     if ((rc = alloc(&S.scan_tmp, 2 * ((n + 8) / 1024 + 4096)))) return rc;
     for (auto& p : S.poly) if ((rc = alloc(&p, n + 8))) return rc;
     for (int k = 0; k < W_COUNT; ++k)
-        if ((rc = alloc(&S.wcos[k], k == W_Z1 ? std::max(m, 2 * n) : m))) return rc;
+        if ((rc = alloc(&S.wcos[k], k == W_Z1 ? std::max(std::max(m, 2 * n), 3 * (n + 8)) : m))) return rc;
     const size_t eval_blocks = (n + 8 + 2047) / 2048 + 1;
     if ((rc = alloc(&S.small, 64 + 16 * eval_blocks))) return rc;
     if ((rc = alloc(&S.lag_scalars, n + 16))) return rc;
     for (auto& q : S.lag_scalars_q) if ((rc = alloc(&q, n + 16))) return rc;
+    if (S.G == 1) {
+        if ((rc = alloc(&S.heads, 3 * NTT_MAX_BATCH * NTT_HEAD))) return rc;
+        if ((rc = alloc(&S.d_win, QC_WIN_POLYS * QC_WIN))) return rc;
+        ZKT_HIP(c, hipHostMalloc(&S.pinned_win, QC_WIN_POLYS * QC_WIN * 32));
+        ZKT_HIP(c, hipEventCreateWithFlags(&S.ev_win, hipEventDisableTiming));
+    }
     if ((rc = dev_alloc(c, (void**)&S.status, 64 * 4))) return rc;
     if ((rc = dev_alloc(c, (void**)&S.status_alt, 64 * 4))) return rc;
     for (auto& p : S.poly_alt) if ((rc = alloc(&p, n + 8))) return rc;
@@ -1090,6 +1257,14 @@
     S.roots = P0.roots;
     memcpy(S.zh_inv, P0.zh_inv, sizeof(S.zh_inv));
     S.keys_borrowed = true;
+    if (P0.ccoset_ready) {
+        for (int k = 0; k < CS_COUNT; ++k) S.ccoset[k] = P0.ccoset[k];
+        memcpy(S.key_win, P0.key_win, sizeof(S.key_win));
+        memcpy(S.qc_gamma, P0.qc_gamma, sizeof(S.qc_gamma));
+        memcpy(S.qc_vinv, P0.qc_vinv, sizeof(S.qc_vinv));
+        memcpy(S.qc_g3, P0.qc_g3, sizeof(S.qc_g3));
+        S.ccoset_borrowed = S.ccoset_ready = true;
+    }
     child->circuit = st;
     const int rc = circuit_alloc_work(child, S);
     if (rc) circuit_release(child);
@@ -1551,6 +1726,68 @@
     return ZKT_OK;
 }
 
+int zkt_ctx_set_quotient_route(zkt_ctx* c, int mode) {
+    if (!c) return ZKT_ERR_INVALID_ARGUMENT;
+    if (mode < 0 || mode > 2) return set_err(c, ZKT_ERR_INVALID_ARGUMENT, "mode: 0 automatic, 1 three classes, 2 the whole coset");
+    c->quotient_route = mode;
+    return ZKT_OK;
+}
+
+int zkt_debug_quotient_top(zkt_ctx* c, uint64_t* out_u, int* out_on_classes) {
+    if (!c || !out_u) return set_err(c, ZKT_ERR_INVALID_ARGUMENT, "null pointer");
+    if (!c->circuit) return set_err(c, ZKT_ERR_NOT_LOADED, "no circuit loaded (zkt_circuit_load)");
+    const CircuitState& S = *c->circuit;
+    if (out_on_classes) *out_on_classes = S.use_classes ? 1 : 0;
+    memcpy(out_u, S.last_u, sizeof(S.last_u));
+    return ZKT_OK;
+}
+
+int zkt_debug_quotient_coeffs(zkt_ctx* c, uint64_t* out, size_t count) {
+    if (!c || !out) return set_err(c, ZKT_ERR_INVALID_ARGUMENT, "null pointer");
+    if (!c->circuit) return set_err(c, ZKT_ERR_NOT_LOADED, "no circuit loaded (zkt_circuit_load)");
+    const CircuitState& S = *c->circuit;
+    if (count > 4 * S.n) return set_err(c, ZKT_ERR_INVALID_ARGUMENT, "the quotient vector holds 4n elements");
+    (void)hipSetDevice(c->device);
+    ZKT_HIP(c, hipStreamSynchronize(c->stream));
+    ZKT_HIP(c, hipMemcpy(out, S.qev, count * 32, hipMemcpyDeviceToHost));
+    return ZKT_OK;
+}
+
+extern "C++" template <class R>
+static void debug_quotient_classes_host_t(int log_n, const uint64_t* windows, const uint64_t* challenges, uint64_t* out_u,
+                                          uint64_t* out_consts) {
+    typedef Fe<R> F;
+    const QuotientClassConsts<R> q = quotient_class_consts<R>(log_n);
+    for (int k = 0; k < 4; ++k) memcpy(out_consts + 4 * k, q.gamma[k].v, 32);
+    for (int k = 0; k < 9; ++k) memcpy(out_consts + 4 * (4 + k), q.vinv[k].v, 32);
+    for (int k = 0; k < 3; ++k) memcpy(out_consts + 4 * (13 + k), q.g3[k].v, 32);
+    const uint32_t* w = (const uint32_t*)windows;
+    QuotientWindows W{};
+    const uint32_t** slot[10] = {&W.a, &W.b, &W.c, &W.z1, &W.z2, &W.t, &W.sigma1, &W.sigma2, &W.sigma3, &W.q_lookup};
+    for (int k = 0; k < 10; ++k) *slot[k] = w + (size_t)k * QCW * 8;
+    F alpha, beta, delta, u[6];
+    memcpy(alpha.v, challenges, 32);
+    memcpy(beta.v, challenges + 4, 32);
+    memcpy(delta.v, challenges + 8, 32);
+    quotient_top_coefficients<R>(log_n, W, alpha, beta, delta, u);
+    for (int e = 0; e < 6; ++e) memcpy(out_u + 4 * e, u[e].v, 32);
+}
+
+int zkt_debug_quotient_classes_host(int curve, int log_n, const uint64_t* windows, const uint64_t* challenges, uint64_t* out_u,
+                                    uint64_t* out_consts) {
+    if (!windows || !challenges || !out_u || !out_consts) return ZKT_ERR_INVALID_ARGUMENT;
+    if (curve == ZKT_CURVE_BN254) {
+        if (log_n < 3 || log_n + 2 > Bn254Fr::TWO_ADICITY) return ZKT_ERR_INVALID_DOMAIN_SIZE;
+        debug_quotient_classes_host_t<Bn254Fr>(log_n, windows, challenges, out_u, out_consts);
+    } else if (curve == ZKT_CURVE_BLS12_381) {
+        if (log_n < 3 || log_n + 2 > Bls381Fr::TWO_ADICITY) return ZKT_ERR_INVALID_DOMAIN_SIZE;
+        debug_quotient_classes_host_t<Bls381Fr>(log_n, windows, challenges, out_u, out_consts);
+    } else {
+        return ZKT_ERR_INVALID_ARGUMENT;
+    }
+    return ZKT_OK;
+}
+
 int zkt_lagrange_info(zkt_ctx* c, int* log_n, size_t* bases) {
     if (!c) return ZKT_ERR_INVALID_ARGUMENT;
     const bool ready = c->circuit && lagrange_ready(c, c->circuit->log_n) && !c->lagrange_off;
diff --git a/zkt-plonk_amd/csrc/quotient_classes.hpp b/zkt-plonk_amd/csrc/quotient_classes.hpp
--- /dev/null
+++ b/zkt-plonk_amd/csrc/quotient_classes.hpp
@@ -0,0 +1,113 @@
+#pragma once
+#include "ctx.hpp"
+#include "hostinv.hpp"
+#include <cstring>
+
+namespace zkt {
+
+constexpr int QCW = 14;
+
+template <class R>
+struct QuotientClassConsts {
+    Fe<R> gamma[4];
+    Fe<R> vinv[9];
+    Fe<R> g3[3];
+};
+
+template <class R>
+static QuotientClassConsts<R> quotient_class_consts(int log_n) {
+    QuotientClassConsts<R> q;
+    const uint64_t n = (uint64_t)1 << log_n;
+    const Fe<R> g = fe_from_u32<R>(R::GENERATOR);
+    const Fe<R> i4 = fe_pow_u64<R>(root_of_unity<R>(log_n + 2), n);
+    q.gamma[0] = fe_pow_u64<R>(g, n);
+    for (int j = 1; j < 4; ++j) q.gamma[j] = fe_mul<R>(q.gamma[j - 1], i4);
+    for (int j = 0; j < 3; ++j) {
+        const Fe<R>&gj = q.gamma[j], &ga = q.gamma[(j + 1) % 3], &gb = q.gamma[(j + 2) % 3];
+        const Fe<R> d = fe_inv_host<R>(fe_mul<R>(fe_sub<R>(gj, ga), fe_sub<R>(gj, gb)));
+        q.vinv[0 + j] = fe_mul<R>(fe_mul<R>(ga, gb), d);
+        q.vinv[3 + j] = fe_mul<R>(fe_neg<R>(fe_add<R>(ga, gb)), d);
+        q.vinv[6 + j] = d;
+    }
+    q.g3[0] = q.gamma[3];
+    q.g3[1] = fe_sqr<R>(q.gamma[3]);
+    q.g3[2] = fe_mul<R>(q.g3[1], q.gamma[3]);
+    return q;
+}
+
+template <class R>
+static void quotient_top_of_product(const Fe<R>* const w[4], Fe<R> out[6]) {
+    int len[4];
+    for (int k = 0; k < 4; ++k) {
+        len[k] = QCW;
+        while (len[k] > 0 && fe_is_zero<R>(w[k][len[k] - 1])) --len[k];
+    }
+    for (int e = 0; e < 6; ++e) out[e] = fe_zero<R>();
+    if (!len[0] || !len[1] || !len[2] || !len[3]) return;
+    Fe<R> p01[2 * QCW - 1], p23[2 * QCW - 1];
+    auto conv = [&](const Fe<R>* x, int lx, const Fe<R>* y, int ly, Fe<R>* o) {
+        for (int i = 0; i < lx + ly - 1; ++i) o[i] = fe_zero<R>();
+        for (int i = 0; i < lx; ++i)
+            for (int j = 0; j < ly; ++j) o[i + j] = fe_add<R>(o[i + j], fe_mul<R>(x[i], y[j]));
+    };
+    conv(w[0], len[0], w[1], len[1], p01);
+    conv(w[2], len[2], w[3], len[3], p23);
+    const int l01 = len[0] + len[1] - 1, l23 = len[2] + len[3] - 1;
+    for (int e = 0; e < 6; ++e) {
+        const int s = 4 * 6 + e;
+        for (int i = 0; i < l01; ++i) {
+            const int j = s - i;
+            if (j >= 0 && j < l23) out[e] = fe_add<R>(out[e], fe_mul<R>(p01[i], p23[j]));
+        }
+    }
+}
+
+struct QuotientWindows {
+    const uint32_t *a, *b, *c, *z1, *z2, *t, *sigma1, *sigma2, *sigma3, *q_lookup;
+};
+
+template <class R>
+static void quotient_top_coefficients(int log_n, const QuotientWindows& W, const Fe<R>& alpha, const Fe<R>& beta, const Fe<R>& delta,
+                                      Fe<R> u[6]) {
+    typedef Fe<R> F;
+    auto load = [](const uint32_t* p, F* o) {
+        for (int i = 0; i < QCW; ++i)
+            for (int k = 0; k < 8; ++k) o[i].v[k] = p[8 * i + k];
+    };
+    F a[QCW], b[QCW], c[QCW], z1[QCW], z2[QCW], t[QCW], s1[QCW], s2[QCW], s3[QCW], ql[QCW];
+    load(W.a, a); load(W.b, b); load(W.c, c); load(W.z1, z1); load(W.z2, z2); load(W.t, t);
+    load(W.sigma1, s1); load(W.sigma2, s2); load(W.sigma3, s3); load(W.q_lookup, ql);
+    const F w = root_of_unity<R>(log_n);
+    F wk[QCW];
+    wk[6] = fe_one<R>();
+    const F winv = fe_inv_host<R>(w);
+    for (int i = 7; i < QCW; ++i) wk[i] = fe_mul<R>(wk[i - 1], w);
+    for (int i = 5; i >= 0; --i) wk[i] = fe_mul<R>(wk[i + 1], winv);
+    F z1w[QCW], as[QCW], bs[QCW], cs[QCW], tt[QCW];
+    for (int i = 0; i < QCW; ++i) {
+        z1w[i] = fe_mul<R>(z1[i], wk[i]);
+        as[i] = fe_add<R>(a[i], fe_mul<R>(beta, s1[i]));
+        bs[i] = fe_add<R>(b[i], fe_mul<R>(beta, s2[i]));
+        cs[i] = fe_add<R>(c[i], fe_mul<R>(beta, s3[i]));
+        tt[i] = fe_add<R>(t[i], fe_mul<R>(delta, fe_mul<R>(t[i], wk[i])));
+    }
+    F p1[6], p2[6], p3[6];
+    {
+        const F* f[4] = {z1, a, b, c};
+        quotient_top_of_product<R>(f, p1);
+    }
+    {
+        const F* f[4] = {z1w, as, bs, cs};
+        quotient_top_of_product<R>(f, p2);
+    }
+    {
+        const F* f[4] = {z2, c, ql, tt};
+        quotient_top_of_product<R>(f, p3);
+    }
+    const F a3 = fe_mul<R>(fe_sqr<R>(alpha), alpha);
+    const F k3 = fe_mul<R>(a3, fe_add<R>(delta, fe_one<R>()));
+    for (int e = 0; e < 6; ++e)
+        u[e] = fe_add<R>(fe_mul<R>(alpha, fe_sub<R>(p1[e], p2[e])), fe_mul<R>(k3, p3[e]));
+}
+
+}
```

Measured after the change: 63.19 proofs/s, median of 6. 4.1% higher.
